# srinidhiPY/SSL_CR_Histo

Measured on AMD Instinct MI355X. Metric: images/sec (ResNet18 SSL_CR step, 256x256 bf16 synthetic patches; whole job), higher is better.
Workload: dtype bf16

## Files before the change

### include/sslcr.h

```cpp
#ifndef SSLCR_H_
#define SSLCR_H_
#include <stddef.h>
#include <stdint.h>

#ifdef __cplusplus
extern "C" {
#endif
#if defined(__GNUC__) || defined(__clang__)
#pragma GCC visibility push(default)
#endif

#define SSLCR_F32 0
#define SSLCR_BF16 1
#define SSLCR_FP8 2

int sslcr_version(void);
const char* sslcr_last_error(void);

typedef struct sslcr_conv_desc {
  const void* x;
  const void* w;
  void* y;
  const float* in_scale;
  const float* in_shift;
  const float* bias;
  const void* residual;
  float* stats;
  int N, H, W, C, K, R, S, stride, pad;
  int PH, PW;
  int OH, OW, osh;
  int transposed;
  int in_relu, relu, accumulate;
  int pix_mul, pix_off_h, pix_off_w;
  unsigned tap_mask;
  const void* mask_x; const float* mask_scale; const float* mask_shift; const float* mask_mean;
  int par4;
  int seg_images, seg_stride;
  const float* out_scale;
} sslcr_conv_desc;
int sslcr_conv2d(int dtype, const sslcr_conv_desc* d, void* stream);
int sslcr_conv2d_partial_rows(const sslcr_conv_desc* d);
int sslcr_conv2d_segments_ok(int dtype, const sslcr_conv_desc* d);
const char* sslcr_conv2d_kernel_name(int dtype, const sslcr_conv_desc* d);
int sslcr_conv2d_s2_pair(int dtype, const sslcr_conv_desc* c1, const sslcr_conv_desc* ds, void* stream);
int sslcr_conv2d_s2_pair_ok(int dtype, const sslcr_conv_desc* c1, const sslcr_conv_desc* ds);

typedef struct sslcr_fp8_desc {
  const uint8_t* w8;
  const float* w_dequant;
  float x_scale;
  const float* x_scale_dev;
  float* amax_out;
} sslcr_fp8_desc;
int sslcr_conv2d_fp8(const sslcr_conv_desc* d, const sslcr_fp8_desc* q, void* stream);
int sslcr_conv2d_fp8_partial_rows(const sslcr_conv_desc* d);
typedef struct sslcr_pack_fp8_desc {
  const float* w;
  uint8_t* w8;
  float* w_dequant;
  const float* gamma; const float* beta; const float* rmean; const float* rvar; float eps; float* bias_out;
  int K, C;
} sslcr_pack_fp8_desc;
int sslcr_pack_conv_fp8(const sslcr_pack_fp8_desc* d, void* stream);

typedef struct sslcr_wgrad_desc {
  const void* x;
  const void* dy;
  float* dw;
  const float* in_scale;
  const float* in_shift;
  int in_relu;
  int N, H, W, C, K, R, S, stride, pad, OH, OW;
  int seg_images;
  int seg_stride;
} sslcr_wgrad_desc;
int sslcr_conv2d_wgrad(int dtype, const sslcr_wgrad_desc* d, void* stream);
const char* sslcr_conv2d_wgrad_kernel_name(int dtype, const sslcr_wgrad_desc* d);

int sslcr_probe_tr16(const uint16_t* in, const int* byte_addr, uint16_t* out, void* stream);

typedef struct sslcr_stem_desc {
  const void* x;
  const void* w;
  void* y;
  const float* bias;
  float* stats;
  int N, H, W, OH, OW, in_f32, relu;
  const void* x2;
  int n_split;
  const float* out_scale;
} sslcr_stem_desc;
int sslcr_stem_conv(int dtype, const sslcr_stem_desc* d, void* stream);
int sslcr_stem_partial_rows(const sslcr_stem_desc* d);
int sslcr_stem_conv_pool(int dtype, const sslcr_stem_desc* d, int POH, int POW, void* stream);
typedef struct sslcr_stem_wgrad_desc {
  const void* x; const void* dy;
  float* dw;
  int N, H, W, OH, OW, in_f32;
  const void* x2; int n_split;
} sslcr_stem_wgrad_desc;
int sslcr_stem_wgrad(int dtype, const sslcr_stem_wgrad_desc* d, void* stream);

typedef struct sslcr_bn_finalize_desc {
  const float* partials;
  int rows, C;
  double count;
  const float* gamma; const float* beta;
  float* scale; float* shift; float* mean; float* invstd;
  float* running_mean; float* running_var; int64_t* num_batches_tracked;
  float momentum, eps; int replay;
  double* sums_out;
  const double* sums_in;
  double* stage;
  int nseg, seg_stride;
  int* tickets;
} sslcr_bn_finalize_desc;
int sslcr_bn_finalize(const sslcr_bn_finalize_desc* d, void* stream);

typedef struct sslcr_bn_act_desc {
  const void* x; const float* scale; const float* shift;
  const void* res; const float* rscale; const float* rshift;
  void* y; size_t pixels; int C; int relu;
  int nseg, seg_stride;
  uint8_t* ybits;
} sslcr_bn_act_desc;
int sslcr_bn_act(int dtype, const sslcr_bn_act_desc* d, void* stream);

typedef struct sslcr_pool_fwd_desc {
  const void* x; const float* scale; const float* shift; void* y; uint8_t* argmax; int N, H, W, C, OH, OW;
} sslcr_pool_fwd_desc;
int sslcr_bn_relu_maxpool(int dtype, const sslcr_pool_fwd_desc* d, void* stream);
typedef struct sslcr_pool_bwd_desc {
  const void* dy; const uint8_t* argmax; const void* x; const float* scale; const float* shift; void* dx; int N, H, W, C, OH, OW;
} sslcr_pool_bwd_desc;
int sslcr_maxpool_relu_bwd(int dtype, const sslcr_pool_bwd_desc* d, void* stream);

int sslcr_avgpool_fwd(int dtype, const void* x, float* y, int N, int HW, int C, void* stream);
int sslcr_avgpool_bwd(int dtype, const float* dy, void* dx, int N, int HW, int C, void* stream);

typedef struct sslcr_bn_bwd_desc {
  const void* dy; const void* x; const void* yact;
  const float* scale; const float* shift; const float* mean; const float* invstd;
  double* sums;
  void* dx; void* gout;
  size_t pixels; int C; int relu_from_x; double count;
  const void* pool_dy;
  const uint8_t* pool_argmax;
  int pH, pW, pOH, pOW;
  const void* pool_y;
  int g_in_reduce;
  float* dgamma; float* dbeta;
  float pg_scale;
  int nseg, seg_stride, sums_stride;
  const uint8_t* yact_bits;
} sslcr_bn_bwd_desc;
int sslcr_bn_bwd_reduce(int dtype, const sslcr_bn_bwd_desc* d, void* stream);
int sslcr_bn_bwd_apply(int dtype, const sslcr_bn_bwd_desc* d, void* stream);
int sslcr_bn_param_grads(const double* sums, const float* invstd, float* dgamma, float* dbeta, int C, void* stream);
int sslcr_stem_wgrad_pool(int dtype, const sslcr_stem_wgrad_desc* w, const sslcr_bn_bwd_desc* bn, void* stream);

int sslcr_linear_fwd(const float* x, const float* w, const float* b, float* y, int M, int N, int K, int relu, void* stream);
int sslcr_linear_bwd(const float* x, const float* w, const float* dy, const float* yact, float* dx, float* dw, float* db,
                     int M, int N, int K, int dx_accumulate, float* scratch, void* stream);
typedef struct sslcr_loss_desc {
  int kind;
  const float* logits; const float* logits_t;
  const float* target_f; const int64_t* target_i;
  float* dlogits;
  float* out;
  int nx, nu, C; float lambda_u;
  float inv_nx_global, inv_nu_global;
} sslcr_loss_desc;
int sslcr_loss(const sslcr_loss_desc* d, void* stream);
typedef struct sslcr_loss_opts {
  const float* class_weight;
  float label_smoothing;
  int ignore_index;
  float threshold;
  float temperature;
  const float* denominator;
  float* stats;
} sslcr_loss_opts;
int sslcr_loss_ex(const sslcr_loss_desc* d, const sslcr_loss_opts* opts, void* stream);
int sslcr_ce_denominator(const int64_t* target_i, int n, int C, const float* class_weight, int ignore_index, float* out2, void* stream);
int sslcr_softmax_col(const float* logits, float* out, int n, int C, int col, void* stream);
typedef struct sslcr_predict_desc {
  const float* logits;
  int n, C;
  const int64_t* target;
  float* scores;
  int64_t* pred;
  int64_t* confusion;
  int col;
  float* map;
  const int64_t* map_index;
  int64_t map_size;
} sslcr_predict_desc;
int sslcr_predict(const sslcr_predict_desc* d, void* stream);

typedef struct sslcr_tensor_desc {
  float* p; float* g; float* s1; float* s2;
  int n;
  int K, C, RS;
  void* w_fwd;
  void* w_dgrad;
  int pack_dtype;
  int dgrad_flip;
  int group;
} sslcr_tensor_desc;
typedef struct sslcr_opt_desc {
  int kind;
  float lr, beta1, beta2, eps, wd, momentum;
  float bc1, bc2;
  int first_step;
  float grad_scale;
} sslcr_opt_desc;
int sslcr_optimizer_step(const sslcr_tensor_desc* device_descs, int ntensors, int max_n, const sslcr_opt_desc* o, void* stream);
#define SSLCR_MAX_OPT_GROUPS 8
int sslcr_optimizer_step_groups(const sslcr_tensor_desc* device_descs, int ntensors, int max_n, const sslcr_opt_desc* groups, int ngroups,
                                const float* coef_dev, void* stream);
int sslcr_grad_norm(const float* g, size_t n, float max_norm, double* partials, float* out2, void* stream);
int sslcr_grad_norm_partials(void);
int sslcr_grad_accumulate(float* dst, const float* src, size_t n, void* stream);
int sslcr_axpby(float* p, float* q, size_t n, float alpha, int copy_back, void* stream);
int sslcr_fill(float* p, size_t n, float v, void* stream);

typedef struct sslcr_pack_desc {
  const float* w; void* w_fwd; void* w_dgrad;
  const float* gamma; const float* beta; const float* rmean; const float* rvar; float eps; float* bias_out;
  int K, C, R, S;
  int dgrad_flip;
  float* scale_out;
} sslcr_pack_desc;
int sslcr_pack_conv(int dtype, const sslcr_pack_desc* d, void* stream);
int sslcr_pack_stem(int dtype, const sslcr_pack_desc* d, void* stream);

typedef struct sslcr_weak_aug_desc {
  const uint8_t* src;
  uint8_t* dst;
  const int32_t* params;
  int N, SH, SW, OH, OW, src_hwc;
} sslcr_weak_aug_desc;
int sslcr_weak_augment(const sslcr_weak_aug_desc* d, void* stream);

typedef struct sslcr_wsi_gather_desc {
  const uint8_t* src;
  const int32_t* xy;
  uint8_t* dst;
  int origin_x, origin_y;
  int N, RH, RW, S, fill;
} sslcr_wsi_gather_desc;
int sslcr_wsi_gather(const sslcr_wsi_gather_desc* d, void* stream);

typedef struct sslcr_colour_aug_desc {
  const uint8_t* src;
  uint8_t* dst;
  const double* shift;
  const uint8_t* apply;
  double hed_from_rgb[9];
  double rgb_from_hed[9];
  int N, H, W, hwc;
} sslcr_colour_aug_desc;
int sslcr_hed_colour_augment(const sslcr_colour_aug_desc* d, void* stream);
typedef struct sslcr_brightness_contrast_desc {
  const uint8_t* src; uint8_t* dst;
  const double* alpha_beta;
  const uint8_t* apply;
  unsigned long long* stats;
  int N, H, W;
} sslcr_brightness_contrast_desc;
int sslcr_brightness_contrast(const sslcr_brightness_contrast_desc* d, void* stream);

#define SSLCR_AUGV2_COPY 0
#define SSLCR_AUGV2_BRIGHTNESS 1
#define SSLCR_AUGV2_CONTRAST 2
#define SSLCR_AUGV2_COLOR 3
#define SSLCR_AUGV2_AUTOCONTRAST 4
#define SSLCR_AUGV2_EQUALIZE 5
#define SSLCR_AUGV2_SHARPNESS 6
#define SSLCR_AUGV2_NEAREST_FIXED 7
#define SSLCR_AUGV2_NEAREST_TABLE 8
#define SSLCR_AUGV2_BICUBIC 9
typedef struct sslcr_augv2_desc {
  const uint8_t* src;
  uint8_t* dst;
  const int32_t* op;
  const float* factor;
  const int32_t* fixed;
  const double* shift;
  const double* affine;
  uint32_t* hist;
  unsigned long long* lsum;
  uint8_t* lut;
  int32_t* tab;
  unsigned ops_mask;
  int N, H, W, src_hwc, dst_hwc;
} sslcr_augv2_desc;
int sslcr_randaug_v2_slot(const sslcr_augv2_desc* d, void* stream);

#define SSLCR_AUGV2C_COPY 0
#define SSLCR_AUGV2C_HED 1
#define SSLCR_AUGV2C_HSV 2
typedef struct sslcr_augv2_colour_desc {
  uint8_t* img;
  const int32_t* op;
  const double* param;
  unsigned long long* bsum;
  double cutoff_lo, cutoff_hi;
  float hed_from_rgb[9];
  float rgb_from_hed[9];
  unsigned ops_mask;
  int N, H, W, hwc;
// ... 97 lines not shown
```

### ssl_cr_histo_amd/_lib.py

```python
import ctypes as C
import os

import torch

HERE = os.path.dirname(os.path.abspath(__file__))
LIB_PATH = os.path.join(HERE, "libsslcr.so")

vp, i32, f32, f64, sz = C.c_void_p, C.c_int, C.c_float, C.c_double, C.c_size_t


class SslcrError(RuntimeError):
    pass


def _S(name, fields):
    return type(name, (C.Structure,), {"_fields_": fields})


ConvDesc = _S("ConvDesc", [("x", vp), ("w", vp), ("y", vp), ("in_scale", vp), ("in_shift", vp), ("bias", vp),
                           ("residual", vp), ("stats", vp)] +
              [(k, i32) for k in ("N", "H", "W", "C", "K", "R", "S", "stride", "pad", "PH", "PW", "OH", "OW", "osh",
                                  "transposed", "in_relu", "relu", "accumulate", "pix_mul", "pix_off_h", "pix_off_w")] +
              [("tap_mask", C.c_uint), ("mask_x", vp), ("mask_scale", vp), ("mask_shift", vp), ("mask_mean", vp),
               ("par4", i32), ("seg_images", i32), ("seg_stride", i32), ("out_scale", vp)])
WgradDesc = _S("WgradDesc", [("x", vp), ("dy", vp), ("dw", vp), ("in_scale", vp), ("in_shift", vp), ("in_relu", i32)] +
               [(k, i32) for k in ("N", "H", "W", "C", "K", "R", "S", "stride", "pad", "OH", "OW", "seg_images", "seg_stride")])
StemDesc = _S("StemDesc", [("x", vp), ("w", vp), ("y", vp), ("bias", vp), ("stats", vp)] +
              [(k, i32) for k in ("N", "H", "W", "OH", "OW", "in_f32", "relu")] + [("x2", vp), ("n_split", i32), ("out_scale", vp)])
StemWgradDesc = _S("StemWgradDesc", [("x", vp), ("dy", vp), ("dw", vp)] +
                   [(k, i32) for k in ("N", "H", "W", "OH", "OW", "in_f32")] + [("x2", vp), ("n_split", i32)])
BnFinalizeDesc = _S("BnFinalizeDesc", [("partials", vp), ("rows", i32), ("C", i32), ("count", f64), ("gamma", vp),
                                       ("beta", vp), ("scale", vp), ("shift", vp), ("mean", vp), ("invstd", vp),
                                       ("running_mean", vp), ("running_var", vp), ("num_batches_tracked", vp),
                                       ("momentum", f32), ("eps", f32), ("replay", i32), ("sums_out", vp),
                                       ("sums_in", vp), ("stage", vp), ("nseg", i32), ("seg_stride", i32), ("tickets", vp)])
BnActDesc = _S("BnActDesc", [("x", vp), ("scale", vp), ("shift", vp), ("res", vp), ("rscale", vp), ("rshift", vp),
                             ("y", vp), ("pixels", sz), ("C", i32), ("relu", i32), ("nseg", i32), ("seg_stride", i32), ("ybits", vp)])
PoolFwdDesc = _S("PoolFwdDesc", [("x", vp), ("scale", vp), ("shift", vp), ("y", vp), ("argmax", vp)] +
                 [(k, i32) for k in ("N", "H", "W", "C", "OH", "OW")])
PoolBwdDesc = _S("PoolBwdDesc", [("dy", vp), ("argmax", vp), ("x", vp), ("scale", vp), ("shift", vp), ("dx", vp)] +
                 [(k, i32) for k in ("N", "H", "W", "C", "OH", "OW")])
BnBwdDesc = _S("BnBwdDesc", [("dy", vp), ("x", vp), ("yact", vp), ("scale", vp), ("shift", vp), ("mean", vp),
                             ("invstd", vp), ("sums", vp), ("dx", vp), ("gout", vp), ("pixels", sz), ("C", i32),
                             ("relu_from_x", i32), ("count", f64), ("pool_dy", vp), ("pool_argmax", vp), ("pH", i32),
                             ("pW", i32), ("pOH", i32), ("pOW", i32), ("pool_y", vp), ("g_in_reduce", i32), ("dgamma", vp), ("dbeta", vp),
                             ("pg_scale", f32), ("nseg", i32), ("seg_stride", i32), ("sums_stride", i32), ("yact_bits", vp)])
LossDesc = _S("LossDesc", [("kind", i32), ("logits", vp), ("logits_t", vp), ("target_f", vp), ("target_i", vp),
                           ("dlogits", vp), ("out", vp), ("nx", i32), ("nu", i32), ("C", i32), ("lambda_u", f32),
                           ("inv_nx_global", f32), ("inv_nu_global", f32)])
LossOpts = _S("LossOpts", [("class_weight", vp), ("label_smoothing", f32), ("ignore_index", i32), ("threshold", f32),
                           ("temperature", f32), ("denominator", vp), ("stats", vp)])
TensorDesc = _S("TensorDesc", [("p", vp), ("g", vp), ("s1", vp), ("s2", vp), ("n", i32), ("K", i32), ("C", i32),
                               ("RS", i32), ("w_fwd", vp), ("w_dgrad", vp), ("pack_dtype", i32), ("dgrad_flip", i32),
                               ("group", i32)])
OptDesc = _S("OptDesc", [("kind", i32), ("lr", f32), ("beta1", f32), ("beta2", f32), ("eps", f32), ("wd", f32),
                         ("momentum", f32), ("bc1", f32), ("bc2", f32), ("first_step", i32), ("grad_scale", f32)])
ClipDesc = _S("ClipDesc", [("max_norm", f32), ("out2", vp)])
MAX_OPT_GROUPS = 8
WeakAugDesc = _S("WeakAugDesc", [("src", vp), ("dst", vp), ("params", vp)] +
                 [(k, i32) for k in ("N", "SH", "SW", "OH", "OW", "src_hwc")])
ColourAugDesc = _S("ColourAugDesc", [("src", vp), ("dst", vp), ("shift", vp), ("apply", vp), ("hed_from_rgb", f64 * 9),
                                     ("rgb_from_hed", f64 * 9), ("N", i32), ("H", i32), ("W", i32), ("hwc", i32)])
BrightnessContrastDesc = _S("BrightnessContrastDesc", [("src", vp), ("dst", vp), ("alpha_beta", vp), ("apply", vp), ("stats", vp),
                                                       ("N", i32), ("H", i32), ("W", i32)])
AugV2Desc = _S("AugV2Desc", [(k, vp) for k in ("src", "dst", "op", "factor", "fixed", "shift", "affine", "hist", "lsum", "lut", "tab")] +
                [("ops_mask", C.c_uint)] + [(k, i32) for k in ("N", "H", "W", "src_hwc", "dst_hwc")])
AugV2ColourDesc = _S("AugV2ColourDesc", [("img", vp), ("op", vp), ("param", vp), ("bsum", vp), ("cutoff_lo", f64), ("cutoff_hi", f64),
                                         ("hed_from_rgb", f32 * 9), ("rgb_from_hed", f32 * 9), ("ops_mask", C.c_uint)] +
                      [(k, i32) for k in ("N", "H", "W", "hwc")])
WsiGatherDesc = _S("WsiGatherDesc", [("src", vp), ("xy", vp), ("dst", vp)] +
                   [(k, i32) for k in ("origin_x", "origin_y", "N", "RH", "RW", "S", "fill")])
PredictDesc = _S("PredictDesc", [("logits", vp), ("n", i32), ("C", i32), ("target", vp), ("scores", vp), ("pred", vp), ("confusion", vp),
                                 ("col", i32), ("map", vp), ("map_index", vp), ("map_size", C.c_int64)])
PackDesc = _S("PackDesc", [("w", vp), ("w_fwd", vp), ("w_dgrad", vp), ("gamma", vp), ("beta", vp), ("rmean", vp),
                           ("rvar", vp), ("eps", f32), ("bias_out", vp)] + [(k, i32) for k in ("K", "C", "R", "S", "dgrad_flip")] + [("scale_out", vp)])

Fp8Desc = _S("Fp8Desc", [("w8", vp), ("w_dequant", vp), ("x_scale", f32), ("x_scale_dev", vp), ("amax_out", vp)])
PackFp8Desc = _S("PackFp8Desc", [("w", vp), ("w8", vp), ("w_dequant", vp), ("gamma", vp), ("beta", vp), ("rmean", vp), ("rvar", vp),
                                 ("eps", f32), ("bias_out", vp), ("K", i32), ("C", i32)])

P = C.POINTER
SIGNATURES = {
    "sslcr_version": (i32, []),
    "sslcr_last_error": (C.c_char_p, []),
    "sslcr_conv2d": (i32, [i32, P(ConvDesc), vp]),
    "sslcr_conv2d_partial_rows": (i32, [P(ConvDesc)]),
    "sslcr_conv2d_segments_ok": (i32, [i32, P(ConvDesc)]),
    "sslcr_conv2d_kernel_name": (C.c_char_p, [i32, P(ConvDesc)]),
    "sslcr_conv2d_s2_pair": (i32, [i32, P(ConvDesc), P(ConvDesc), vp]),
    "sslcr_conv2d_s2_pair_ok": (i32, [i32, P(ConvDesc), P(ConvDesc)]),
    "sslcr_conv2d_fp8": (i32, [P(ConvDesc), P(Fp8Desc), vp]),
    "sslcr_conv2d_fp8_partial_rows": (i32, [P(ConvDesc)]),
    "sslcr_pack_conv_fp8": (i32, [P(PackFp8Desc), vp]),
    "sslcr_conv2d_wgrad": (i32, [i32, P(WgradDesc), vp]),
    "sslcr_conv2d_wgrad_kernel_name": (C.c_char_p, [i32, P(WgradDesc)]),
    "sslcr_probe_tr16": (i32, [vp, vp, vp, vp]),
    "sslcr_stem_conv": (i32, [i32, P(StemDesc), vp]),
    "sslcr_stem_partial_rows": (i32, [P(StemDesc)]),
    "sslcr_stem_conv_pool": (i32, [i32, P(StemDesc), i32, i32, vp]),
    "sslcr_stem_wgrad": (i32, [i32, P(StemWgradDesc), vp]),
    "sslcr_stem_wgrad_pool": (i32, [i32, P(StemWgradDesc), P(BnBwdDesc), vp]),
    "sslcr_bn_finalize": (i32, [P(BnFinalizeDesc), vp]),
    "sslcr_bn_act": (i32, [i32, P(BnActDesc), vp]),
    "sslcr_bn_relu_maxpool": (i32, [i32, P(PoolFwdDesc), vp]),
    "sslcr_maxpool_relu_bwd": (i32, [i32, P(PoolBwdDesc), vp]),
    "sslcr_avgpool_fwd": (i32, [i32, vp, vp, i32, i32, i32, vp]),
    "sslcr_avgpool_bwd": (i32, [i32, vp, vp, i32, i32, i32, vp]),
    "sslcr_bn_bwd_reduce": (i32, [i32, P(BnBwdDesc), vp]),
    "sslcr_bn_bwd_apply": (i32, [i32, P(BnBwdDesc), vp]),
    "sslcr_bn_param_grads": (i32, [vp, vp, vp, vp, i32, vp]),
    "sslcr_linear_fwd": (i32, [vp, vp, vp, vp, i32, i32, i32, i32, vp]),
    "sslcr_linear_bwd": (i32, [vp, vp, vp, vp, vp, vp, vp, i32, i32, i32, i32, vp, vp]),
    "sslcr_loss": (i32, [P(LossDesc), vp]),
    "sslcr_loss_ex": (i32, [P(LossDesc), P(LossOpts), vp]),
    "sslcr_ce_denominator": (i32, [vp, i32, i32, vp, i32, vp, vp]),
    "sslcr_softmax_col": (i32, [vp, vp, i32, i32, i32, vp]),
    "sslcr_predict": (i32, [P(PredictDesc), vp]),
    "sslcr_wsi_gather": (i32, [P(WsiGatherDesc), vp]),
    "sslcr_optimizer_step": (i32, [vp, i32, i32, P(OptDesc), vp]),
    "sslcr_optimizer_step_groups": (i32, [vp, i32, i32, P(OptDesc), i32, vp, vp]),
    "sslcr_grad_norm": (i32, [vp, sz, f32, vp, vp, vp]),
    "sslcr_grad_norm_partials": (i32, []),
    "sslcr_grad_accumulate": (i32, [vp, vp, sz, vp]),
    "sslcr_axpby": (i32, [vp, vp, sz, f32, i32, vp]),
    "sslcr_fill": (i32, [vp, sz, f32, vp]),
    "sslcr_pack_conv": (i32, [i32, P(PackDesc), vp]),
    "sslcr_pack_stem": (i32, [i32, P(PackDesc), vp]),
    "sslcr_weak_augment": (i32, [P(WeakAugDesc), vp]),
    "sslcr_hed_colour_augment": (i32, [P(ColourAugDesc), vp]),
    "sslcr_brightness_contrast": (i32, [P(BrightnessContrastDesc), vp]),
    "sslcr_randaug_v2_slot": (i32, [P(AugV2Desc), vp]),
    "sslcr_randaug_v2_colour": (i32, [P(AugV2ColourDesc), vp]),
}

_lib = None


def lib():
    global _lib
    if _lib is None:
        if not os.path.exists(LIB_PATH):
            raise SslcrError(f"{LIB_PATH} not built: run `python -m ssl_cr_histo_amd.build` "
                             "(or __graft_entry__.build()); there is no CPU/PyTorch fallback")
        L = C.CDLL(LIB_PATH, mode=C.RTLD_GLOBAL)
        for name, (res, args) in SIGNATURES.items():
            fn = getattr(L, name)
            fn.restype = res
            fn.argtypes = args
        _lib = L
    return _lib


def check(rc):
    if rc != 0:
        raise SslcrError(lib().sslcr_last_error().decode())


def stream_ptr():
    return C.c_void_p(torch.cuda.current_stream().cuda_stream)


def ptr(t):
    return None if t is None else C.c_void_p(t.data_ptr())
```

### ssl_cr_histo_amd/csrc/capi.cpp

```cpp
#include <stdarg.h>
#include <stdio.h>
#include <string.h>

#include "kernels.hpp"

namespace sslcr {
thread_local char g_err[512] = "";
int fail(const char* fmt, ...) {
  va_list ap;
  va_start(ap, fmt);
  vsnprintf(g_err, sizeof(g_err), fmt, ap);
  va_end(ap);
  return -1;
}
int check(hipError_t e, const char* what) {
  if (e == hipSuccess) return 0;
  return fail("%s: %s", what, hipGetErrorString(e));
}
}

using namespace sslcr;

#define NEED(cond, what) \
  do {                   \
    if (!(cond)) return fail("%s: invalid argument (%s)", __func__, what); \
  } while (0)
#define DT_OK(dt) NEED((dt) == SSLCR_F32 || (dt) == SSLCR_BF16, "dtype")

extern "C" {

int sslcr_version(void) { return 12; }
const char* sslcr_last_error(void) { return g_err; }

int sslcr_conv2d(int dtype, const sslcr_conv_desc* d, void* stream) {
  DT_OK(dtype);
  NEED(d && d->x && d->w && d->y, "null tensor");
  NEED(d->N > 0 && d->C > 0 && d->K > 0 && d->R > 0 && d->S > 0 && d->stride > 0, "shape");
  NEED(d->C % (dtype == SSLCR_BF16 ? 64 : 32) == 0, "C must be a multiple of the 128-byte channel slab");
  NEED(d->K % 64 == 0, "K % 64");
  NEED(d->osh >= 1 && d->PH > 0 && d->PW > 0, "pixel space");
  const ConvPlan p = conv_plan(dtype, *d);
  NEED(p.seg_ok, "seg_images: no segment form for this shape / dtype (sslcr_conv2d_segments_ok)");
  return check(launch_conv(dtype, *d, p, (hipStream_t)stream), "conv2d");
}
int sslcr_conv2d_partial_rows(const sslcr_conv_desc* d) { return d ? conv_partials_rows(*d) : -1; }
int sslcr_conv2d_segments_ok(int dtype, const sslcr_conv_desc* d) { return (d && (dtype == DT_F32 || dtype == DT_BF16) && conv_segments_ok(dtype, *d)) ? 1 : 0; }
const char* sslcr_conv2d_kernel_name(int dtype, const sslcr_conv_desc* d) { return d ? conv_kernel_name(dtype, *d) : ""; }
int sslcr_conv2d_s2_pair_ok(int dtype, const sslcr_conv_desc* c1, const sslcr_conv_desc* ds) {
  return (c1 && ds && conv_s2_pair_ok(dtype, *c1, *ds)) ? 1 : 0;
}
int sslcr_conv2d_s2_pair(int dtype, const sslcr_conv_desc* c1, const sslcr_conv_desc* ds, void* stream) {
  DT_OK(dtype);
  NEED(c1 && ds && c1->x && c1->w && c1->y && ds->w && ds->y, "null tensor");
  NEED(conv_s2_pair_ok(dtype, *c1, *ds), "pair not served (sslcr_conv2d_s2_pair_ok)");
  return check(launch_conv_s2(*c1, ds, (hipStream_t)stream), "conv2d_s2_pair");
}

int sslcr_conv2d_fp8(const sslcr_conv_desc* d, const sslcr_fp8_desc* q, void* stream) {
  NEED(d && q && d->x && d->y && q->w8 && q->w_dequant, "null tensor");
  NEED(q->x_scale > 0.f, "x_scale must be positive");
  NEED(conv_fp8_mode(*d) != 0, "shape not served by the fp8 kernel (3x3/1, C % 128, K % 128, 16x16-tileable or 8x8 with N % 4)");
  return check(launch_conv_fp8(*d, *q, (hipStream_t)stream), "conv2d_fp8");
}
int sslcr_conv2d_fp8_partial_rows(const sslcr_conv_desc* d) { return (d && conv_fp8_mode(*d)) ? conv_fp8_rows(*d) : 0; }
int sslcr_pack_conv_fp8(const sslcr_pack_fp8_desc* d, void* stream) {
  NEED(d && d->w && d->w8 && d->w_dequant && d->K > 0 && d->C > 0, "args");
  NEED(!d->gamma || (d->beta && d->rmean && d->rvar), "BatchNorm fold needs gamma, beta, running mean and var");
  return check(launch_pack_fp8(*d, (hipStream_t)stream), "pack_conv_fp8");
}

const char* sslcr_conv2d_wgrad_kernel_name(int dtype, const sslcr_wgrad_desc* d) { return d ? wgrad_kernel_name(dtype, *d) : ""; }
int sslcr_conv2d_wgrad(int dtype, const sslcr_wgrad_desc* d, void* stream) {
  DT_OK(dtype);
  NEED(d && d->x && d->dy && d->dw, "null tensor");
  NEED(d->C % 64 == 0 && d->K % 64 == 0, "C,K % 64");
  NEED((d->R == 3 && d->S == 3) || (d->R == 1 && d->S == 1), "3x3 or 1x1");
  return check(launch_wgrad(dtype, *d, (hipStream_t)stream), "conv2d_wgrad");
}

int sslcr_probe_tr16(const uint16_t* in, const int* byte_addr, uint16_t* out, void* stream) {
  NEED(in && byte_addr && out, "null");
  return check(launch_probe_tr16(in, byte_addr, out, (hipStream_t)stream), "probe_tr16");
}

int sslcr_stem_conv(int dtype, const sslcr_stem_desc* d, void* stream) {
  DT_OK(dtype);
  NEED(d && d->x && d->w && d->y, "null tensor");
  NEED(d->OH == (d->H + 6 - 7) / 2 + 1 && d->OW == (d->W + 6 - 7) / 2 + 1, "7x7/2 pad 3 output dims");
  NEED(!d->x2 || (d->n_split >= 0 && d->n_split <= d->N), "n_split outside the batch");
  return check(launch_stem(dtype, *d, (hipStream_t)stream), "stem_conv");
}
int sslcr_stem_conv_pool(int dtype, const sslcr_stem_desc* d, int POH, int POW, void* stream) {
  DT_OK(dtype);
  NEED(d && d->x && d->w && d->y, "null");
  NEED(stem_pool_ok(dtype, *d, POH, POW), "shape / mode not served by the fused stem + max-pool kernel");
  return check(launch_stem_pool(dtype, *d, POH, POW, (hipStream_t)stream), "stem_conv_pool");
}
int sslcr_stem_partial_rows(const sslcr_stem_desc* d) { return d ? stem_partials_rows(*d) : -1; }
int sslcr_stem_wgrad(int dtype, const sslcr_stem_wgrad_desc* d, void* stream) {
  DT_OK(dtype);
  NEED(d && d->x && d->dy && d->dw, "null tensor");
  NEED(!d->x2 || (d->n_split >= 0 && d->n_split <= d->N), "n_split outside the batch");
  return check(launch_stem_wgrad(dtype, *d, (hipStream_t)stream), "stem_wgrad");
}
int sslcr_stem_wgrad_pool(int dtype, const sslcr_stem_wgrad_desc* w, const sslcr_bn_bwd_desc* bn, void* stream) {
  DT_OK(dtype);
  NEED(w && w->x && w->dw && bn && bn->pool_dy && bn->pool_argmax && bn->x && bn->sums && bn->mean && bn->invstd && bn->scale && bn->shift, "null tensor");
  NEED(!w->x2 || (w->n_split >= 0 && w->n_split <= w->N), "n_split outside the batch");
  NEED(bn->C == 64 && bn->pH == w->OH && bn->pW == w->OW && bn->pixels == (size_t)w->N * w->OH * w->OW, "bn descriptor is not this stem's");
  NEED(!bn->g_in_reduce && !bn->gout, "pool form has no g output");
  return check(launch_stem_wgrad_pool(dtype, *w, *bn, (hipStream_t)stream), "stem_wgrad_pool");
}

int sslcr_bn_finalize(const sslcr_bn_finalize_desc* d, void* stream) {
  NEED(d && d->C > 0, "desc");
  NEED(d->sums_in || (d->partials && d->stage && d->rows > 0), "partials/stage");
  NEED(d->sums_out || (d->gamma && d->beta && d->scale && d->shift && d->count > 0), "finalize outputs");
  return check(launch_bn_finalize(*d, (hipStream_t)stream), "bn_finalize");
}
int sslcr_bn_act(int dtype, const sslcr_bn_act_desc* d, void* stream) {
  DT_OK(dtype);
  NEED(d && d->x && d->y && d->scale && d->shift, "null");
  NEED(d->C % 8 == 0, "C % 8");
  return check(launch_bn_act(dtype, *d, (hipStream_t)stream), "bn_act");
}
int sslcr_bn_relu_maxpool(int dtype, const sslcr_pool_fwd_desc* d, void* stream) {
  DT_OK(dtype);
  NEED(d && d->x && d->y, "null");
  if (!d->scale || !d->shift) {
    const int cols = d->C / (dtype == SSLCR_BF16 ? 8 : 4);
    NEED(!d->scale && !d->shift && !d->argmax, "plain max-pool (scale = shift = NULL) records no argmax");
    NEED(cols >= 1 && cols <= 256 && 256 % cols == 0 && d->C % (dtype == SSLCR_BF16 ? 8 : 4) == 0, "plain max-pool: unsupported channel count");
  }
  return check(launch_bn_relu_maxpool(dtype, *d, (hipStream_t)stream), "bn_relu_maxpool");
}
int sslcr_maxpool_relu_bwd(int dtype, const sslcr_pool_bwd_desc* d, void* stream) {
  DT_OK(dtype);
  NEED(d && d->x && d->dy && d->dx && d->argmax, "null");
  return check(launch_maxpool_relu_bwd(dtype, *d, (hipStream_t)stream), "maxpool_relu_bwd");
}
int sslcr_avgpool_fwd(int dtype, const void* x, float* y, int N, int HW, int C, void* stream) {
  DT_OK(dtype);
  NEED(x && y && N > 0 && HW > 0 && C % 8 == 0, "args");
  return check(launch_avgpool_fwd(dtype, x, y, N, HW, C, (hipStream_t)stream), "avgpool_fwd");
}
int sslcr_avgpool_bwd(int dtype, const float* dy, void* dx, int N, int HW, int C, void* stream) {
  DT_OK(dtype);
  NEED(dy && dx && N > 0 && HW > 0 && C % 8 == 0, "args");
  return check(launch_avgpool_bwd(dtype, dy, dx, N, HW, C, (hipStream_t)stream), "avgpool_bwd");
}
int sslcr_bn_bwd_reduce(int dtype, const sslcr_bn_bwd_desc* d, void* stream) {
  DT_OK(dtype);
  NEED(d && (d->dy || (d->pool_dy && d->pool_argmax)) && d->x && d->sums && d->mean, "null");
  NEED(!d->g_in_reduce || (d->yact && d->gout && d->dy && !d->pool_dy), "g_in_reduce needs dy, yact and gout");
  return check(launch_bn_bwd_reduce(dtype, *d, (hipStream_t)stream), "bn_bwd_reduce");
}
int sslcr_bn_bwd_apply(int dtype, const sslcr_bn_bwd_desc* d, void* stream) {
  DT_OK(dtype);
  NEED(d && (d->dy || (d->pool_dy && d->pool_argmax)) && d->x && d->sums && d->dx && d->mean && d->invstd && d->scale, "null");
  NEED(!d->g_in_reduce || (d->yact && d->gout && d->dy && !d->pool_dy), "g_in_reduce needs dy, yact and gout");
  return check(launch_bn_bwd_apply(dtype, *d, (hipStream_t)stream), "bn_bwd_apply");
}
int sslcr_bn_param_grads(const double* sums, const float* invstd, float* dgamma, float* dbeta, int C, void* stream) {
  NEED(sums && invstd && dgamma && dbeta, "null");
  return check(launch_bn_param_grads(sums, invstd, dgamma, dbeta, C, (hipStream_t)stream), "bn_param_grads");
}

int sslcr_linear_fwd(const float* x, const float* w, const float* b, float* y, int M, int N, int K, int relu, void* stream) {
  NEED(x && w && y && M > 0 && N > 0 && K > 0, "args");
  return check(launch_linear_fwd(x, w, b, y, M, N, K, relu, (hipStream_t)stream), "linear_fwd");
}
int sslcr_linear_bwd(const float* x, const float* w, const float* dy, const float* yact, float* dx, float* dw, float* db,
                     int M, int N, int K, int dx_accumulate, float* scratch, void* stream) {
  NEED(x && w && dy && scratch && M > 0 && N > 0 && K > 0, "args");
  return check(launch_linear_bwd(x, w, dy, yact, dx, dw, db, M, N, K, dx_accumulate, scratch, (hipStream_t)stream), "linear_bwd");
}
int sslcr_loss(const sslcr_loss_desc* d, void* stream) {
  NEED(d && d->logits && d->out && d->nx > 0 && d->C > 0 && d->C <= 64, "args");
  return check(launch_loss(*d, (hipStream_t)stream), "loss");
}

int sslcr_loss_ex(const sslcr_loss_desc* d, const sslcr_loss_opts* o, void* stream) {
  if (!o) return sslcr_loss(d, stream);
  NEED(d && d->logits && d->out && d->nx > 0 && d->C > 0 && d->C <= 64, "args");
  const char* why = loss_opts_error(d->kind, d->C, *o);
  if (why) return fail("sslcr_loss_ex: invalid argument (%s)", why);
  if (d->kind != 1 && d->kind != 2) return check(launch_loss(*d, (hipStream_t)stream), "loss");
  NEED(d->target_i && (d->kind == 2 || d->nu == 0 || d->logits_t), "cross-entropy needs target_i (and logits_t for the consistency rows)");
  NEED(d->nu >= 0, "nu");
  return check(launch_loss_ex(*d, *o, (hipStream_t)stream), "loss_ex");
}
int sslcr_ce_denominator(const int64_t* target_i, int n, int C, const float* class_weight, int ignore_index, float* out2, void* stream) {
  NEED(out2 && (target_i || n == 0) && n >= 0 && C > 0 && C <= 64, "args");
  return check(launch_ce_denominator(target_i, n, C, class_weight, ignore_index, out2, (hipStream_t)stream), "ce_denominator");
}

int sslcr_softmax_col(const float* logits, float* out, int n, int C, int col, void* stream) {
  NEED(logits && out && n > 0 && C > 0 && C <= 64 && col >= 0 && col < C, "args");
  return check(launch_softmax_col(logits, out, n, C, col, (hipStream_t)stream), "softmax_col");
}

int sslcr_predict(const sslcr_predict_desc* d, void* stream) {
  NEED(d, "null descriptor");
  NEED(d->n >= 0 && d->C >= 1 && d->C <= 64, "n >= 0 and 1 <= C <= 64");
  if (d->n == 0) return 0;
  NEED(d->logits, "null logits");
  NEED(!d->confusion || d->target, "confusion needs target");
  NEED((reinterpret_cast<uintptr_t>(d->confusion) & 7) == 0, "confusion alignment");
  NEED(!d->map || (d->map_index && d->map_size >= 0), "map needs map_index and map_size >= 0");
  NEED(!d->map || (d->col >= 0 && d->col < d->C), "col outside [0, C)");
  return check(launch_predict(*d, (hipStream_t)stream), "predict");
}
int sslcr_wsi_gather(const sslcr_wsi_gather_desc* d, void* stream) {
  NEED(d, "null descriptor");
  NEED(d->S >= 1 && d->N >= 0, "S >= 1 and N >= 0");
  NEED(d->RH >= 1 && d->RW >= 1, "empty region");
  NEED(d->fill >= 0 && d->fill <= 255, "fill outside [0, 255]");
  if (d->N == 0) return 0;
  NEED(d->src && d->xy && d->dst, "null tensor");
  NEED((reinterpret_cast<uintptr_t>(d->xy) & 3) == 0, "xy alignment");
  return check(launch_wsi_gather(*d, (hipStream_t)stream), "wsi_gather");
}

int sslcr_optimizer_step(const sslcr_tensor_desc* device_descs, int ntensors, int max_n, const sslcr_opt_desc* o, void* stream) {
  return sslcr_optimizer_step_groups(device_descs, ntensors, max_n, o, 1, nullptr, stream);
}
int sslcr_optimizer_step_groups(const sslcr_tensor_desc* device_descs, int ntensors, int max_n, const sslcr_opt_desc* groups, int ngroups,
                                const float* coef_dev, void* stream) {
  NEED(device_descs && groups && ntensors > 0 && max_n > 0, "args");
  NEED(ngroups >= 1 && ngroups <= SSLCR_MAX_OPT_GROUPS, "ngroups must be 1..8");
// ... 82 lines not shown
```

### ssl_cr_histo_amd/csrc/common.hpp

```cpp
#pragma once
#include <hip/hip_runtime.h>
#include <stdint.h>

namespace sslcr {

typedef uint16_t bf16_t;
typedef __bf16 bf16x8_t __attribute__((ext_vector_type(8)));
typedef float f32x4_t __attribute__((ext_vector_type(4)));
typedef uint32_t u32x4_t __attribute__((ext_vector_type(4)));
typedef uint32_t u32x2_t __attribute__((ext_vector_type(2)));

enum { DT_F32 = 0, DT_BF16 = 1 };

__device__ __forceinline__ float bf2f(uint16_t v) { return __uint_as_float(((uint32_t)v) << 16); }
__device__ __forceinline__ uint16_t f2bf(float f) {
  uint32_t u = __float_as_uint(f);
  u += 0x7fffu + ((u >> 16) & 1u);
  return (uint16_t)(u >> 16);
}
__device__ __forceinline__ uint32_t pack_bf2(float lo, float hi) {
  return (uint32_t)f2bf(lo) | ((uint32_t)f2bf(hi) << 16);
}
__device__ __forceinline__ float bf_lo(uint32_t w) { return __uint_as_float(w << 16); }
__device__ __forceinline__ float bf_hi(uint32_t w) { return __uint_as_float(w & 0xffff0000u); }

template <typename T> struct Elem;
template <> struct Elem<float> {
  static constexpr int EPC = 4;
  static constexpr int DT = DT_F32;
  __device__ static __forceinline__ void unpack(const u32x4_t& v, float* f) {
#pragma unroll
    for (int i = 0; i < 4; ++i) f[i] = __uint_as_float(v[i]);
  }
  __device__ static __forceinline__ u32x4_t pack(const float* f) {
    u32x4_t v;
#pragma unroll
    for (int i = 0; i < 4; ++i) v[i] = __float_as_uint(f[i]);
    return v;
  }
  __device__ static __forceinline__ float ld(const float* p) { return *p; }
  __device__ static __forceinline__ void st(float* p, float v) { *p = v; }
};
template <> struct Elem<bf16_t> {
  static constexpr int EPC = 8;
  static constexpr int DT = DT_BF16;
  __device__ static __forceinline__ void unpack(const u32x4_t& v, float* f) {
#pragma unroll
    for (int i = 0; i < 4; ++i) { f[2 * i] = bf_lo(v[i]); f[2 * i + 1] = bf_hi(v[i]); }
  }
  __device__ static __forceinline__ u32x4_t pack(const float* f) {
    u32x4_t v;
#pragma unroll
    for (int i = 0; i < 4; ++i) v[i] = pack_bf2(f[2 * i], f[2 * i + 1]);
    return v;
  }
  __device__ static __forceinline__ float ld(const bf16_t* p) { return bf2f(*p); }
  __device__ static __forceinline__ void st(bf16_t* p, float v) { *p = f2bf(v); }
};

template <typename T> struct PackH {
  __device__ static __forceinline__ u32x4_t run(const float* f) { return Elem<T>::pack(f); }
};
template <> struct PackH<bf16_t> {
  typedef __bf16 bf16x2_t __attribute__((ext_vector_type(2)));
  typedef float f32x2_t __attribute__((ext_vector_type(2)));
  __device__ static __forceinline__ u32x4_t run(const float* f) {
    u32x4_t v;
#pragma unroll
    for (int i = 0; i < 4; ++i)
      v[i] = __builtin_bit_cast(uint32_t, __builtin_convertvector(f32x2_t{f[2 * i], f[2 * i + 1]}, bf16x2_t));
    return v;
  }
};

__device__ __forceinline__ float row16_sum(float v) {
  v += __int_as_float(__builtin_amdgcn_update_dpp(0, __float_as_int(v), 0xB1, 0xf, 0xf, true));
  v += __int_as_float(__builtin_amdgcn_update_dpp(0, __float_as_int(v), 0x4E, 0xf, 0xf, true));
  v += __int_as_float(__builtin_amdgcn_update_dpp(0, __float_as_int(v), 0x141, 0xf, 0xf, true));
  v += __int_as_float(__builtin_amdgcn_update_dpp(0, __float_as_int(v), 0x140, 0xf, 0xf, true));
  return v;
}
__device__ __forceinline__ void row16_sum4(float& a, float& b, float& c, float& d) {
  asm volatile(
      "s_nop 1\n\t"
      "v_add_f32_dpp %0, %0, %0 quad_perm:[1,0,3,2] row_mask:0xf bank_mask:0xf\n\t"
      "v_add_f32_dpp %1, %1, %1 quad_perm:[1,0,3,2] row_mask:0xf bank_mask:0xf\n\t"
      "v_add_f32_dpp %2, %2, %2 quad_perm:[1,0,3,2] row_mask:0xf bank_mask:0xf\n\t"
      "v_add_f32_dpp %3, %3, %3 quad_perm:[1,0,3,2] row_mask:0xf bank_mask:0xf\n\t"
      "v_add_f32_dpp %0, %0, %0 quad_perm:[2,3,0,1] row_mask:0xf bank_mask:0xf\n\t"
      "v_add_f32_dpp %1, %1, %1 quad_perm:[2,3,0,1] row_mask:0xf bank_mask:0xf\n\t"
      "v_add_f32_dpp %2, %2, %2 quad_perm:[2,3,0,1] row_mask:0xf bank_mask:0xf\n\t"
      "v_add_f32_dpp %3, %3, %3 quad_perm:[2,3,0,1] row_mask:0xf bank_mask:0xf\n\t"
      "v_add_f32_dpp %0, %0, %0 row_half_mirror row_mask:0xf bank_mask:0xf\n\t"
      "v_add_f32_dpp %1, %1, %1 row_half_mirror row_mask:0xf bank_mask:0xf\n\t"
      "v_add_f32_dpp %2, %2, %2 row_half_mirror row_mask:0xf bank_mask:0xf\n\t"
      "v_add_f32_dpp %3, %3, %3 row_half_mirror row_mask:0xf bank_mask:0xf\n\t"
      "v_add_f32_dpp %0, %0, %0 row_mirror row_mask:0xf bank_mask:0xf\n\t"
      "v_add_f32_dpp %1, %1, %1 row_mirror row_mask:0xf bank_mask:0xf\n\t"
      "v_add_f32_dpp %2, %2, %2 row_mirror row_mask:0xf bank_mask:0xf\n\t"
      "v_add_f32_dpp %3, %3, %3 row_mirror row_mask:0xf bank_mask:0xf"
      : "+v"(a), "+v"(b), "+v"(c), "+v"(d));
}
__device__ __forceinline__ void row16_fold16(float (&v)[16]) {
  asm volatile(
      "s_nop 1\n\t"
      "v_add_f32_dpp %0, %0, %0 row_ror:8 row_mask:0xf bank_mask:0x3\n\t"
      "v_add_f32_dpp %0, %8, %8 row_ror:8 row_mask:0xf bank_mask:0xc\n\t"
      "v_add_f32_dpp %1, %1, %1 row_ror:8 row_mask:0xf bank_mask:0x3\n\t"
      "v_add_f32_dpp %1, %9, %9 row_ror:8 row_mask:0xf bank_mask:0xc\n\t"
      "v_add_f32_dpp %2, %2, %2 row_ror:8 row_mask:0xf bank_mask:0x3\n\t"
      "v_add_f32_dpp %2, %10, %10 row_ror:8 row_mask:0xf bank_mask:0xc\n\t"
      "v_add_f32_dpp %3, %3, %3 row_ror:8 row_mask:0xf bank_mask:0x3\n\t"
      "v_add_f32_dpp %3, %11, %11 row_ror:8 row_mask:0xf bank_mask:0xc\n\t"
      "v_add_f32_dpp %4, %4, %4 row_ror:8 row_mask:0xf bank_mask:0x3\n\t"
      "v_add_f32_dpp %4, %12, %12 row_ror:8 row_mask:0xf bank_mask:0xc\n\t"
      "v_add_f32_dpp %5, %5, %5 row_ror:8 row_mask:0xf bank_mask:0x3\n\t"
      "v_add_f32_dpp %5, %13, %13 row_ror:8 row_mask:0xf bank_mask:0xc\n\t"
      "v_add_f32_dpp %6, %6, %6 row_ror:8 row_mask:0xf bank_mask:0x3\n\t"
      "v_add_f32_dpp %6, %14, %14 row_ror:8 row_mask:0xf bank_mask:0xc\n\t"
      "v_add_f32_dpp %7, %7, %7 row_ror:8 row_mask:0xf bank_mask:0x3\n\t"
      "v_add_f32_dpp %7, %15, %15 row_ror:8 row_mask:0xf bank_mask:0xc\n\t"
      "v_add_f32_dpp %0, %0, %0 row_half_mirror row_mask:0xf bank_mask:0x5\n\t"
      "v_add_f32_dpp %0, %4, %4 row_half_mirror row_mask:0xf bank_mask:0xa\n\t"
      "v_add_f32_dpp %1, %1, %1 row_half_mirror row_mask:0xf bank_mask:0x5\n\t"
      "v_add_f32_dpp %1, %5, %5 row_half_mirror row_mask:0xf bank_mask:0xa\n\t"
      "v_add_f32_dpp %2, %2, %2 row_half_mirror row_mask:0xf bank_mask:0x5\n\t"
      "v_add_f32_dpp %2, %6, %6 row_half_mirror row_mask:0xf bank_mask:0xa\n\t"
      "v_add_f32_dpp %3, %3, %3 row_half_mirror row_mask:0xf bank_mask:0x5\n\t"
      "v_add_f32_dpp %3, %7, %7 row_half_mirror row_mask:0xf bank_mask:0xa\n\t"
      "v_add_f32_dpp %0, %0, %0 quad_perm:[1,0,3,2] row_mask:0xf bank_mask:0xf\n\t"
      "v_add_f32_dpp %1, %1, %1 quad_perm:[1,0,3,2] row_mask:0xf bank_mask:0xf\n\t"
      "v_add_f32_dpp %2, %2, %2 quad_perm:[1,0,3,2] row_mask:0xf bank_mask:0xf\n\t"
      "v_add_f32_dpp %3, %3, %3 quad_perm:[1,0,3,2] row_mask:0xf bank_mask:0xf\n\t"
      "v_add_f32_dpp %0, %0, %0 quad_perm:[2,3,0,1] row_mask:0xf bank_mask:0xf\n\t"
      "v_add_f32_dpp %1, %1, %1 quad_perm:[2,3,0,1] row_mask:0xf bank_mask:0xf\n\t"
      "v_add_f32_dpp %2, %2, %2 quad_perm:[2,3,0,1] row_mask:0xf bank_mask:0xf\n\t"
      "v_add_f32_dpp %3, %3, %3 quad_perm:[2,3,0,1] row_mask:0xf bank_mask:0xf"
      : "+&v"(v[0]), "+&v"(v[1]), "+&v"(v[2]), "+&v"(v[3]), "+&v"(v[4]), "+&v"(v[5]), "+&v"(v[6]), "+&v"(v[7])
      : "v"(v[8]), "v"(v[9]), "v"(v[10]), "v"(v[11]), "v"(v[12]), "v"(v[13]), "v"(v[14]), "v"(v[15]));
}
__device__ __forceinline__ float wave_sum(float v) {
  v = row16_sum(v);
  v += __shfl_xor(v, 16);
  v += __shfl_xor(v, 32);
  return v;
}

__device__ __forceinline__ float clamp_lo(float x, float lo) { return __builtin_amdgcn_fmed3f(x, lo, __builtin_inff()); }
__device__ __forceinline__ float relu0(float x) { return __builtin_amdgcn_fmed3f(x, 0.f, __builtin_inff()); }

__device__ __forceinline__ u32x4_t ld16(const void* p) { return *reinterpret_cast<const u32x4_t*>(p); }
__device__ __forceinline__ void st16(void* p, const u32x4_t& v) { *reinterpret_cast<u32x4_t*>(p) = v; }
__device__ __forceinline__ u32x4_t ld16_nt(const void* p) { return __builtin_nontemporal_load(reinterpret_cast<const u32x4_t*>(p)); }
__device__ __forceinline__ void st16_nt(void* p, const u32x4_t& v) { __builtin_nontemporal_store(v, reinterpret_cast<u32x4_t*>(p)); }

struct LdsDma {
#if defined(__HIP_DEVICE_COMPILE__)
  __amdgpu_buffer_rsrc_t r;
#endif
  __device__ __forceinline__ void init(const void* base, unsigned bytes) {
#if defined(__HIP_DEVICE_COMPILE__)
    r = __builtin_amdgcn_make_buffer_rsrc(const_cast<void*>(base), 0, (int)bytes, 0x00020000);
#endif
  }
  __device__ __forceinline__ void load16(void* dst, int voff, int soff) const {
#if defined(__HIP_DEVICE_COMPILE__)
    __builtin_amdgcn_raw_ptr_buffer_load_lds(r, (__attribute__((address_space(3))) void*)dst, 16, voff, soff, 0, 0);
#endif
  }
};


template <typename T> struct Mma;
template <> struct Mma<bf16_t> {
  __device__ static __forceinline__ void run(const u32x4_t& a, const u32x4_t& b, f32x4_t& c) {
    c = __builtin_amdgcn_mfma_f32_16x16x32_bf16(__builtin_bit_cast(bf16x8_t, a), __builtin_bit_cast(bf16x8_t, b), c, 0, 0, 0);
  }
};
template <> struct Mma<float> {
  __device__ static __forceinline__ void run(const u32x4_t& a, const u32x4_t& b, f32x4_t& c) {
#pragma unroll
    for (int e = 0; e < 4; ++e)
      c = __builtin_amdgcn_mfma_f32_16x16x4f32(__uint_as_float(a[e]), __uint_as_float(b[e]), c, 0, 0, 0);
  }
};

template <typename B>
__device__ __forceinline__ int xcd_run_start(B b, int G) { return (G & 7) ? (int)b : (int)(b & 7) * (G >> 3) + (int)(b >> 3); }
struct OuterInner { int outer, inner; };
__device__ __forceinline__ OuterInner xcd_outer_inner(int w, int n_outer, int n_inner, bool inner_slow) {
  int outer, inner;
  if ((n_outer & 7) == 0) {
    const int grp = w / (8 * n_inner), r = w - grp * 8 * n_inner;
    outer = grp * 8 + (r & 7); inner = r >> 3;
  } else if (inner_slow) {
    inner = w / n_outer; outer = w - inner * n_outer;
  } else {
    outer = w / n_inner; inner = w - outer * n_inner;
  }
  return {outer, inner};
}

typedef short s16x4_t __attribute__((ext_vector_type(4)));
typedef short s16x8_t __attribute__((ext_vector_type(8)));
__device__ __forceinline__ bf16x8_t tr_pair(const char* p0, const char* p1) {
  s16x4_t lo = __builtin_amdgcn_ds_read_tr16_b64_v4i16((__attribute__((address_space(3))) s16x4_t*)(p0));
  s16x4_t hi = __builtin_amdgcn_ds_read_tr16_b64_v4i16((__attribute__((address_space(3))) s16x4_t*)(p1));
  s16x8_t v = __builtin_shufflevector(lo, hi, 0, 1, 2, 3, 4, 5, 6, 7);
  return __builtin_bit_cast(bf16x8_t, v);
}
template <int OFF>
__device__ __forceinline__ u32x2_t lds_tr16(uint32_t addr) {
  u32x2_t v;
  asm volatile("ds_read_b64_tr_b16 %0, %1 offset:%2" : "=v"(v) : "v"(addr), "n"(OFF));
  return v;
}
__device__ __forceinline__ uint32_t lds_addr(const void* p) { return (uint32_t)(size_t)(__attribute__((address_space(3))) const char*)(const char*)p; }
__device__ __forceinline__ bf16x8_t frag_join(const u32x2_t& lo, const u32x2_t& hi) {
  return __builtin_bit_cast(bf16x8_t, u32x4_t{lo[0], lo[1], hi[0], hi[1]});
}

__device__ __forceinline__ void barrier_lds() { asm volatile("s_waitcnt lgkmcnt(0)\n\ts_barrier" ::: "memory"); }
__device__ __forceinline__ void barrier_bare() { asm volatile("s_barrier" ::: "memory"); }
// ... 91 lines not shown
```

### ssl_cr_histo_amd/csrc/conv_route.cpp

```cpp
#include "kernels.hpp"

namespace sslcr {

ConvPlan conv_plan(int dtype, const ConvArgs& a) {
  auto both = [&](int (*tiling)(int, const ConvArgs&)) {
    const int t = tiling(dtype, a);
    return t == tiling(DT_BF16, a) ? t : 0;
  };
  const bool segs = a.seg_images > 0;
  const bool seg_common = segs && dtype == DT_BF16 && a.N % a.seg_images == 0 && !a.transposed && !a.par4 && a.N / a.seg_images <= 8;
  bool seg_form = false;
  bool ok = !(a.out_scale && (!a.bias || a.stats || a.mask_x));
  ConvPlan p{};
  const int q = both(conv_halo256_mode);
  if (const int mode = conv_h16_mode(a, q)) {
    const bool pp = conv_pp64_ok(dtype, a);
    p.route = pp ? ConvRoute::PP64 : ConvRoute::H16;
    p.param = mode;
    p.rows = segs && a.N < a.seg_images ? -1 : (pp ? conv_pp64_rows(a) : conv_h16_rows(a));
    p.name = pp ? conv_pp64_name(a) : conv_h16_name(dtype, a, mode);
    seg_form = true;
  } else if (q) {
    p.route = ConvRoute::HALO256;
    p.param = q;
    p.rows = conv_halo256_tiles(a, q) * 4;
    p.name = conv_halo256_name(dtype, a, q);
    seg_form = q == 16 || a.seg_images % 4 == 0;
  } else if (const int tw = both(conv_halo_tw)) {
    p.route = ConvRoute::HALO;
    p.param = tw;
    p.rows = conv_halo_tiles(a, tw) * 2;
    p.name = conv_halo_name(dtype, a, tw);
  } else if (conv_s2_ok(dtype, a)) {
    p.route = ConvRoute::S2;
    p.rows = conv_s2_rows(a);
    p.name = conv_s2_name(a, false);
    seg_form = true;
  } else if (conv_s2d_ok(dtype, a)) {
    p.route = ConvRoute::S2D;
    const int bp = both(conv_dma_bp);
    p.rows = bp ? conv_dma_rows(a, bp) : conv_igemm_rows(a);
    p.name = conv_s2d_name();
    p.par4_one_launch = bp != 0;
  } else if (const int bp = both(conv_dma_bp)) {
    p.route = ConvRoute::DMA;
    p.param = bp;
    p.rows = conv_dma_rows(a, bp);
    p.name = conv_dma_name(dtype, bp);
    p.par4_one_launch = a.par4 != 0;
    seg_form = !a.in_scale && ((long)a.seg_images * a.PH * a.PW) % bp == 0;
  } else {
    p.route = ConvRoute::IGEMM;
    p.rows = conv_igemm_rows(a);
    p.name = conv_igemm_name(dtype, a);
    if (a.par4) ok = false;
  }
  if (a.mask_x && p.route != ConvRoute::H16 && p.route != ConvRoute::PP64) ok = seg_form = false;
  p.seg_ok = !segs || (seg_common && seg_form);
  p.ok = ok && p.seg_ok;
  return p;
}

hipError_t launch_conv(int dtype, const ConvArgs& a, const ConvPlan& p, hipStream_t st) {
  if (!p.ok) return hipErrorInvalidValue;
  switch (p.route) {
    case ConvRoute::H16: return launch_conv_h16(dtype, a, p.param, st);
    case ConvRoute::PP64: return launch_conv_pp64(a, st);
    case ConvRoute::HALO256: return launch_conv_halo256(dtype, a, p.param, st);
    case ConvRoute::HALO: return launch_conv_halo(dtype, a, p.param, st);
    case ConvRoute::S2: return launch_conv_s2(a, nullptr, st);
    case ConvRoute::S2D: return launch_conv_s2d(a, st);
    case ConvRoute::DMA: return launch_conv_dma(dtype, a, p.param, st);
    case ConvRoute::IGEMM: return launch_igemm(dtype, a, st);
  }
  return hipErrorInvalidValue;
}

WgradPlan wgrad_plan(int dtype, const WgradArgs& a) {
  if (const int tw = wgrad_halo_tw(a)) {
    const int kh = dtype == DT_BF16 && a.K % 128 == 0 ? 2 : 1;
    if (kh == 2 && wgrad_dma_ok(dtype, a, wgrad_halo_splits(a, tw, 2))) return {WgradRoute::HALO_DMA, tw, 2, true, wgrad_dma_name(a, tw)};
    return {WgradRoute::HALO, tw, kh, true, wgrad_halo_name(dtype, tw, kh)};
  }
  if (wgrad_s2_ok(dtype, a)) return {WgradRoute::S2, 0, 0, true, wgrad_s2_name(a)};
  const bool segs = a.seg_images > 0 && a.seg_images < a.N;
  return {WgradRoute::GENERIC, 0, 0, !segs, wgrad_generic_name(dtype, a)};
}

hipError_t launch_wgrad(int dtype, const WgradArgs& a, const WgradPlan& p, hipStream_t st) {
  if (!p.ok) return hipErrorInvalidValue;
  switch (p.route) {
    case WgradRoute::HALO:
    case WgradRoute::HALO_DMA: return launch_wgrad_halo(dtype, a, p, st);
    case WgradRoute::S2: return launch_wgrad_s2(a, st);
    case WgradRoute::GENERIC: return launch_wgrad_generic(dtype, a, st);
  }
  return hipErrorInvalidValue;
}

}
```

### ssl_cr_histo_amd/csrc/engine.cpp

```cpp
#include <rccl/rccl.h>
#include <stdio.h>
#include <stdlib.h>
#include <string.h>

#include <atomic>
#include <chrono>
#include <condition_variable>
#include <mutex>
#include <vector>

#include "kernels.hpp"

using namespace sslcr;

#define TRY(expr)                                   \
  do {                                              \
    hipError_t _e = (expr);                         \
    if (_e != hipSuccess) return check(_e, #expr);  \
  } while (0)
#define TRYI(expr)            \
  do {                        \
    int _r = (expr);          \
    if (_r != 0) return _r;   \
  } while (0)
// ... 181 lines not shown
  float *cat[3], *hact[3], *fi[3], *feats = nullptr, *hid = nullptr, *logits = nullptr, *dE[3], *dfeats = nullptr, *dhid = nullptr,
        *dtmp256 = nullptr, *dtmp512 = nullptr, *dcat = nullptr, *scratch = nullptr, *dlogits = nullptr, *logits_t = nullptr;
  int last_N = 0, last_npass = 0;
  bool last_segments = false;
  bool packed_train = false, packed_eval = false;
  bool tap = false;
  DevBuf tapbuf[8][6];
  int tapdims[8][6][4] = {};
  int tap_flags[8] = {};
  std::vector<sslcr_tensor_desc> host_descs;
  std::vector<float*> st1, st2;
  std::vector<int> group_of;
  int ndesc = 0, max_n = 0;
};

namespace {

struct VSrc { const void* p[VW_MAX]; };
template <typename T>
__global__ void vsum_kernel(T* dst, VSrc src, int W, size_t n) {
  for (size_t i = (size_t)blockIdx.x * blockDim.x + threadIdx.x; i < n; i += (size_t)gridDim.x * blockDim.x) {
    T s = static_cast<const T*>(src.p[0])[i];
    for (int q = 1; q < W; ++q) s += static_cast<const T*>(src.p[q])[i];
    dst[i] = s;
  }
}

std::atomic<int> g_live_ctx{0};

inline bool sharded(const sslcr_ctx* c) { return c->comm != nullptr || c->vcomm != nullptr; }

int vcomm_all_reduce(sslcr_ctx* c, int chan, void* buf, size_t count, bool f64, hipStream_t st) {
  sslcr_vcomm* v = c->vcomm;
  VChan& ch = v->ch[chan];
  const int r = c->rank, W = v->world;
  const size_t bytes = count * (f64 ? 8 : 4);
  if (v->poisoned) return fail("virtual all-reduce: the communicator was poisoned by an earlier timeout");
  const int ph = (int)(ch.calls[r]++ & 1);
  for (int q = 0; q < W; ++q)
    if (q != r && ch.out_set[ph][q]) TRY(hipStreamWaitEvent(st, ch.ev_out[ph][q], 0));
  if (ch.cap[ph][r] < bytes) {
    if (ch.slot[ph][r]) TRY(hipFree(ch.slot[ph][r]));
    ch.slot[ph][r] = nullptr; ch.cap[ph][r] = 0;
    TRY(hipMalloc(&ch.slot[ph][r], (bytes + 255) & ~(size_t)255));
    ch.cap[ph][r] = (bytes + 255) & ~(size_t)255;
  }
  if (!ch.ev_in[ph][r]) {
    TRY(hipEventCreateWithFlags(&ch.ev_in[ph][r], hipEventDisableTiming));
    TRY(hipEventCreateWithFlags(&ch.ev_out[ph][r], hipEventDisableTiming));
  }
  TRY(hipMemcpyAsync(ch.slot[ph][r], buf, bytes, hipMemcpyDeviceToDevice, st));
  TRY(hipEventRecord(ch.ev_in[ph][r], st));
  {
    std::unique_lock<std::mutex> lk(ch.m);
    const long g = ch.gen;
    if (++ch.arrived == W) {
      ch.arrived = 0; ++ch.gen;
      ch.cv.notify_all();
    } else if (!ch.cv.wait_for(lk, std::chrono::seconds(120), [&] { return ch.gen != g; })) {
      --ch.arrived;
      c->vcomm->poisoned = true;
      ch.cv.notify_all();
      return fail("virtual all-reduce: rank %d waited 120 s for its peers (channel %d); the communicator is now unusable", r, chan);
    }
  }
  VSrc src;
  for (int q = 0; q < W; ++q) {
    src.p[q] = ch.slot[ph][q];
    if (q != r) TRY(hipStreamWaitEvent(st, ch.ev_in[ph][q], 0));
  }
  const int blocks = (int)((count + 255) / 256 < 1024 ? (count + 255) / 256 : 1024);
  if (f64) hipLaunchKernelGGL(vsum_kernel<double>, dim3(blocks), dim3(256), 0, st, (double*)buf, src, W, count);
  else hipLaunchKernelGGL(vsum_kernel<float>, dim3(blocks), dim3(256), 0, st, (float*)buf, src, W, count);
  TRY(hipGetLastError());
  TRY(hipEventRecord(ch.ev_out[ph][r], st));
  ch.out_set[ph][r] = true;
  return 0;
}

int all_reduce(sslcr_ctx* c, int chan, void* buf, size_t count, bool f64, hipStream_t st) {
  if (c->vcomm) return vcomm_all_reduce(c, chan, buf, count, f64, st);
  TRYN(ncclAllReduce(buf, buf, count, f64 ? ncclDouble : ncclFloat, ncclSum, chan == 0 ? c->comm : c->comm_g, st));
  return 0;
}

template <class Book, class Launch>
hipError_t profiled(sslcr_ctx* c, int slot, hipStream_t st, Book&& book, Launch&& launch) {
  if (!c->prof.on) return launch();
  ProfRec r;
  r.e0 = c->prof.get(); r.e1 = c->prof.get();
  book(r);
  (void)hipEventRecord(r.e0, st);
  hipError_t e = launch();
  (void)hipEventRecord(r.e1, st);
  c->prof.rec[slot].push_back(r);
  return e;
}
hipError_t prof_conv(sslcr_ctx* c, int dt, const ConvArgs& a, hipStream_t st) {
  const ConvPlan plan = conv_plan(dt, a);
  auto book = [&](ProfRec& r) {
    const double es = c->esz();
    const double rs = a.tap_mask ? (double)__builtin_popcount(a.tap_mask) : (double)a.R * a.S;
    const double M = (double)a.N * a.PH * a.PW, src = (double)a.N * a.H * a.W;
    r.flops = a.transposed ? 2.0 * src * a.C * a.K * rs : 2.0 * M * a.K * a.C * rs;
    r.bytes = (src * a.C + (double)a.K * rs * a.C + M * a.K * (a.residual ? 2.0 : 1.0) * (a.accumulate ? 2.0 : 1.0)) * es;
    r.name = plan.name;
  };
  return profiled(c, 0, st, book, [&] { return launch_conv(dt, a, plan, st); });
}
hipError_t prof_conv_pair(sslcr_ctx* c, const ConvArgs& a, const ConvArgs& d, hipStream_t st) {
  auto book = [&](ProfRec& r) {
    const double es = c->esz();
    const double M = (double)a.N * a.PH * a.PW, src = (double)a.N * a.H * a.W;
    r.flops = 2.0 * M * a.K * a.C * 10.0;
    r.bytes = (src * a.C + (double)a.K * 10.0 * a.C + 2.0 * M * a.K) * es;
    r.name = conv_s2_name(a, true);
  };
  return profiled(c, 0, st, book, [&] { return launch_conv_s2(a, &d, st); });
}
inline bool fp8_layer(const sslcr_ctx* c, const ConvL& L) {
  return c->fp8 && L.k == 3 && L.stride == 1 && L.cin % 128 == 0 && L.cout % 128 == 0;
}
inline bool use_fp8(const sslcr_ctx* c, const ConvL& L, const ConvArgs& a) { return fp8_layer(c, L) && L.w8_fwd && conv_fp8_mode(a) != 0; }
hipError_t prof_conv_fwd(sslcr_ctx* c, int dt, const ConvArgs& a_in, const ConvL& L, bool folded, hipStream_t st) {
  ConvArgs a = a_in;
  a.out_scale = nullptr;
  if (!use_fp8(c, L, a)) return prof_conv(c, dt, a_in, st);
  Fp8Args q;
  q.w8 = folded ? L.w8_fold : L.w8_fwd;
  q.w_dequant = folded ? L.dq_fold : L.dq_fwd;
  q.x_scale = 1.0f;
  q.x_scale_dev = L.f8s ? L.f8s + (folded ? 2 : 0) : nullptr;
  q.amax_out = L.f8s ? L.f8s + (folded ? 3 : 1) : nullptr;
  auto book = [&](ProfRec& r) {
    const double M = (double)a.N * a.PH * a.PW;
    r.flops = 2.0 * M * a.K * a.C * 9.0;
    r.bytes = ((double)a.N * a.H * a.W * a.C + M * a.K * (a.residual ? 2.0 : 1.0)) * 2.0 + (double)a.K * 9.0 * a.C;
    r.name = conv_fp8_name(a);
  };
  return profiled(c, 0, st, book, [&] { return launch_conv_fp8(a, q, st); });
}
hipError_t prof_wgrad(sslcr_ctx* c, int dt, const WgradArgs& a, hipStream_t st) {
  const WgradPlan plan = wgrad_plan(dt, a);
  auto book = [&](ProfRec& r) {
    const double es = c->esz();
    const double M = (double)a.N * a.OH * a.OW;
    r.flops = 2.0 * M * a.K * a.C * a.R * a.S;
    r.bytes = ((double)a.N * a.H * a.W * a.C + M * a.K) * es + (double)a.K * a.R * a.S * a.C * 4.0;
    r.name = plan.name;
  };
  return profiled(c, 1, st, book, [&] { return launch_wgrad(dt, a, plan, st); });
}

inline bool tile16(const ConvPlan& p) { return p.route == ConvRoute::H16 || p.route == ConvRoute::PP64; }

constexpr int kMaxSeg = 3;
const int kBlockCfg[8][3] ={{64, 64, 1}, {64, 64, 1}, {64, 128, 2}, {128, 128, 1}, {128, 256, 2}, {256, 256, 1}, {256, 512, 2}, {512, 512, 1}};

inline int out_dim(int h, int k, int stride, int pad) { return (h + 2 * pad - k) / stride + 1; }

void build_topology(sslcr_net* n) {
  int p = 0, b = 0;
  n->stem = ConvL{3, 64, 7, 2, 3, p++};
  n->bn0 = BnL{64, p, p + 1, b++};
  p += 2;
  for (int i = 0; i < 8; ++i) {
    BlockL& B = n->blocks[i];
    const int cin = kBlockCfg[i][0], cout = kBlockCfg[i][1], s = kBlockCfg[i][2];
    B.pstart = p;
    B.c1 = ConvL{cin, cout, 3, s, 1, p++};
    B.b1 = BnL{cout, p, p + 1, b++};
    p += 2;
    B.c2 = ConvL{cout, cout, 3, 1, 1, p++};
    B.b2 = BnL{cout, p, p + 1, b++};
    p += 2;
    B.has_ds = (s != 1 || cin != cout);
    if (B.has_ds) {
      B.ds = ConvL{cin, cout, 1, s, 0, p++};
      B.bd = BnL{cout, p, p + 1, b++};
      p += 2;
    }
  }
  n->psize.assign(n->nparams, 0);
  auto conv_sz = [](const ConvL& c) { return c.cout * c.cin * c.k * c.k; };
  n->psize[n->stem.pidx] = conv_sz(n->stem);
  n->psize[n->bn0.pg] = n->psize[n->bn0.pb] = 64;
  for (int i = 0; i < 8; ++i) {
    BlockL& B = n->blocks[i];
    n->psize[B.c1.pidx] = conv_sz(B.c1);
    n->psize[B.c2.pidx] = conv_sz(B.c2);
    n->psize[B.b1.pg] = n->psize[B.b1.pb] = B.b1.C;
    n->psize[B.b2.pg] = n->psize[B.b2.pb] = B.b2.C;
    if (B.has_ds) {
      n->psize[B.ds.pidx] = conv_sz(B.ds);
      n->psize[B.bd.pg] = n->psize[B.bd.pb] = B.bd.C;
    }
  }
  n->psize[60] = 512 * 1024;
  n->psize[61] = 512;
  n->psize[62] = 256 * 512;
  n->psize[63] = 256;
  if (n->head_kind == 0) {
    n->psize[64] = n->ncls * 768;
    n->psize[65] = n->ncls;
  } else {
    n->psize[64] = 128 * 768;
    n->psize[65] = 128;
    n->psize[66] = n->ncls * 128;
    n->psize[67] = n->ncls;
  }
  n->goff.assign(n->nparams + 1, 0);
  for (int i = 0; i < n->nparams; ++i) n->goff[i + 1] = n->goff[i] + ((n->psize[i] + 63) & ~63);
  n->grad_count = n->goff[n->nparams];
}

bool unfold_eval(const sslcr_ctx* c) {
  static const bool on = [] { const char* e = getenv("SSLCR_UNFOLD_EVAL"); return !e || atoi(e) != 0; }();
  return on && c->dtype == DT_BF16;
}

int alloc_shadow(sslcr_net* n) {
  const size_t es = n->ctx->esz();
  Carver c;
  std::vector<std::pair<ConvL*, size_t>> offs;
  auto add = [&](ConvL& L) {
    const size_t wbytes = (L.pidx == 0 ? (size_t)64 * 224 : (size_t)L.cout * L.cin * L.k * L.k) * es;
    size_t o = c.take(wbytes);
    c.take(wbytes);
    c.take(wbytes);
    c.take(L.cout * sizeof(float));
    c.take(L.cout * sizeof(float));
    if (L.pidx == 0) c.take(wbytes);
    if (fp8_layer(n->ctx, L)) {
      c.take((size_t)L.cout * 9 * L.cin); c.take((size_t)L.cout * 9 * L.cin);
      c.take(L.cout * sizeof(float)); c.take(L.cout * sizeof(float));
    }
    offs.push_back({&L, o});
  };
  add(n->stem);
  for (int i = 0; i < 8; ++i) {
    add(n->blocks[i].c1);
    add(n->blocks[i].c2);
    if (n->blocks[i].has_ds) add(n->blocks[i].ds);
  }
  TRYI(n->shadow.ensure(c.off));
  for (auto& pr : offs) {
    ConvL& L = *pr.first;
    const size_t wbytes = ((L.pidx == 0 ? (size_t)64 * 224 : (size_t)L.cout * L.cin * L.k * L.k) * es + 255) & ~(size_t)255;
    char* base = (char*)n->shadow.p + pr.second;
    L.w_fwd = base;
    L.w_dg = base + wbytes;
    L.w_fold = base + 2 * wbytes;
    L.b_fold = (float*)(base + 3 * wbytes);
    {
      const size_t bb = (L.cout * sizeof(float) + 255) & ~(size_t)255;
      L.s_fold = unfold_eval(n->ctx) ? (float*)(base + 3 * wbytes + bb) : nullptr;
      if (L.pidx == 0) L.w_foldf = base + 3 * wbytes + 2 * bb;
    }
    if (fp8_layer(n->ctx, L)) {
      const size_t bb = (L.cout * sizeof(float) + 255) & ~(size_t)255, w8 = ((size_t)L.cout * 9 * L.cin + 255) & ~(size_t)255;
      char* q = base + 3 * wbytes + 2 * bb;
      L.w8_fwd = (uint8_t*)q; L.w8_fold = (uint8_t*)(q + w8);
      L.dq_fwd = (float*)(q + 2 * w8); L.dq_fold = (float*)(q + 2 * w8 + bb);
    }
  }
  if (n->ctx->fp8) {
    n->n8 = 0;
    for (auto& pr : offs) if (pr.first->w8_fwd) n->n8 += 2;
    TRYI(n->f8buf.ensure((size_t)n->n8 * 2 * sizeof(float)));
    n->f8slots = (float*)n->f8buf.p;
    std::vector<float> init((size_t)n->n8 * 2);
    for (int i = 0; i < n->n8; ++i) { init[2 * i] = 1.f; init[2 * i + 1] = 0.f; }
    TRY(hipMemcpy(n->f8slots, init.data(), init.size() * sizeof(float), hipMemcpyHostToDevice));
    int k = 0;
    for (auto& pr : offs) if (pr.first->w8_fwd) { pr.first->f8s = n->f8slots + 4 * k; ++k; }
  }
  return 0;
}

int pack_conv_layer(sslcr_net* n, ConvL& L, const BnL& bn, int mode, hipStream_t st) {
  const int dt = n->ctx->dtype;
  PackArgs a;
  memset(&a, 0, sizeof(a));
  a.w = n->params[L.pidx];
  a.K = L.cout; a.C = L.cin; a.R = L.k; a.S = L.k;
  a.eps = 1e-5f;
  const bool stem = (L.pidx == 0);
  if (mode & 1) {
    a.w_fwd = L.w_fwd;
    a.w_dgrad = stem ? nullptr : L.w_dg;
    a.dgrad_flip = (L.k == 3 && L.stride == 1);
    TRY(stem ? launch_pack_stem(dt, a, st) : launch_pack_conv(dt, a, st));
  }
  if (mode & 2) {
    a.w_fwd = L.w_fold;
    a.w_dgrad = nullptr;
    a.gamma = n->params[bn.pg]; a.beta = n->params[bn.pb];
    a.rmean = n->bn_rm[bn.bidx]; a.rvar = n->bn_rv[bn.bidx];
    a.bias_out = L.b_fold;
    a.scale_out = L.s_fold;
    TRY(stem ? launch_pack_stem(dt, a, st) : launch_pack_conv(dt, a, st));
    if (stem && L.s_fold && L.w_foldf) {
      a.w_fwd = L.w_foldf; a.scale_out = nullptr;
      TRY(launch_pack_stem(dt, a, st));
    }
  }
// ... 398 lines not shown
  n->feats = (float*)(b + o_feats); n->hid = (float*)(b + o_hid); n->logits = (float*)(b + o_log);
  n->dfeats = (float*)(b + o_dfeats); n->dhid = (float*)(b + o_dhid);
  n->dtmp256 = (float*)(b + o_d256); n->dtmp512 = (float*)(b + o_d512); n->dcat = (float*)(b + o_dcat);
  n->scratch = (float*)(b + o_scr); n->dlogits = (float*)(b + o_dl); n->logits_t = (float*)(b + o_lt);
  n->hN = N;
  return 0;
}

const int kPairs[3][2] = {{0, 1}, {1, 2}, {0, 2}};

int heads_forward(sslcr_net* n, float* const* E, int npass, int N, hipStream_t st) {
  const float *w0 = n->params[60], *b0 = n->params[61], *w2 = n->params[62], *b2 = n->params[63];
  const int nh = (npass == 3) ? 3 : 1;
  for (int i = 0; i < nh; ++i) {
    const float* Ea = E[npass == 3 ? kPairs[i][0] : 0];
    const float* Eb = E[npass == 3 ? kPairs[i][1] : 0];
    if (Ea == Eb) {
      TRY(launch_copy2d_multi(n->cat[i], 1024, 2, 512, Ea, 512, 1, 0, N, 512, st));
    } else {
      TRY(launch_copy2d(n->cat[i], 1024, Ea, 512, N, 512, 0, st));
      TRY(launch_copy2d(n->cat[i] + 512, 1024, Eb, 512, N, 512, 0, st));
    }
    TRY(launch_linear_fwd(n->cat[i], w0, b0, n->hact[i], N, 512, 1024, 1, st));
    TRY(launch_linear_fwd(n->hact[i], w2, b2, n->fi[i], N, 256, 512, 0, st));
  }
  if (nh == 1) {
    TRY(launch_copy2d_multi(n->feats, 768, 3, 256, n->fi[0], 256, 1, 0, N, 256, st));
  } else {
    for (int i = 0; i < 3; ++i) TRY(launch_copy2d(n->feats + 256 * i, 768, n->fi[i], 256, N, 256, 0, st));
  }
  if (n->head_kind == 0) {
    TRY(launch_linear_fwd(n->feats, n->params[64], n->params[65], n->logits, N, n->ncls, 768, 0, st));
  } else {
    TRY(launch_linear_fwd(n->feats, n->params[64], n->params[65], n->hid, N, 128, 768, 1, st));
    TRY(launch_linear_fwd(n->hid, n->params[66], n->params[67], n->logits, N, n->ncls, 128, 0, st));
  }
  return 0;
}

inline float* gptr(sslcr_net* n, int pidx) { return n->rg[pidx] ? n->gw + n->goff[pidx] : nullptr; }

int heads_backward(sslcr_net* n, const float* dlogits, int npass, int N, bool need_dE, hipStream_t st) {
  const float *w0 = n->params[60], *w2 = n->params[62];
  const bool any_fc = n->rg[60] || n->rg[61] || n->rg[62] || n->rg[63];
  if (n->head_kind == 0) {
    TRY(launch_linear_bwd(n->feats, n->params[64], dlogits, nullptr, (any_fc || need_dE) ? n->dfeats : nullptr, gptr(n, 64), gptr(n, 65),
                          N, n->ncls, 768, 0, n->scratch, st));
  } else {
    TRY(launch_linear_bwd(n->hid, n->params[66], dlogits, nullptr, n->dhid, gptr(n, 66), gptr(n, 67), N, n->ncls, 128, 0, n->scratch, st));
    TRY(launch_linear_bwd(n->feats, n->params[64], n->dhid, n->hid, (any_fc || need_dE) ? n->dfeats : nullptr, gptr(n, 64), gptr(n, 65),
                          N, 128, 768, 0, n->scratch, st));
  }
  if (!any_fc && !need_dE) return 0;
  const int nh = (npass == 3) ? 3 : 1;
  if (need_dE && nh == 3)
    for (int i = 0; i < npass; ++i) TRY(hipMemsetAsync(n->dE[i], 0, (size_t)N * 512 * 4, st));
  for (int i = 0; i < nh; ++i) {
    if (nh == 3) {
      TRY(launch_copy2d(n->dtmp256, 256, n->dfeats + 256 * i, 768, N, 256, 0, st));
    } else {
      TRY(launch_copy2d_multi(n->dtmp256, 256, 1, 0, n->dfeats, 768, 3, 256, N, 256, st));
    }
    TRY(launch_linear_bwd(n->hact[i], w2, n->dtmp256, nullptr, n->dtmp512, gptr(n, 62), gptr(n, 63), N, 256, 512, 0, n->scratch, st));
    TRY(launch_linear_bwd(n->cat[i], w0, n->dtmp512, n->hact[i], need_dE ? n->dcat : nullptr, gptr(n, 60), gptr(n, 61), N, 512, 1024, 0,
                          n->scratch, st));
    if (need_dE && nh == 1) {
      TRY(launch_copy2d_multi(n->dE[0], 512, 1, 0, n->dcat, 1024, 2, 512, N, 512, st));
    } else if (need_dE) {
      const int a = nh == 3 ? kPairs[i][0] : 0, b = nh == 3 ? kPairs[i][1] : 0;
      TRY(launch_copy2d(n->dE[a], 512, n->dcat, 1024, N, 512, 1, st));
      TRY(launch_copy2d(n->dE[b], 512, n->dcat + 512, 1024, N, 512, 1, st));
    }
  }
  return 0;
}

struct PoolSrc {
  const void* dy; const uint8_t* argmax; int H, W, OH, OW; const void* y;
};

struct BnBwdReq {
  const void *dy = nullptr, *x = nullptr, *yact = nullptr;
  void *dx = nullptr, *gout = nullptr;
  int relu_from_x = 0;
  size_t pixels = 0;
  double count = 0.0;
  const PoolSrc* pool = nullptr;
  int g_in_reduce = 0;
  const float* sum_rows = nullptr;
  int n_sum_rows = 0, nseg = 0, seg_stride = 0;
  bool defer = false;
};

double* take_sums_n(sslcr_ctx* c, int nseg) {
  if (!c->bn_ring.p || c->bn_ring_i + nseg > sslcr_ctx::kBnRing) return nullptr;
  double* p = (double*)c->bn_ring.p + (size_t)c->bn_ring_i * sslcr_ctx::kBnSlot;
  c->bn_ring_i += nseg;
  return p;
}
double* take_sums(sslcr_ctx* c) { return take_sums_n(c, 1); }
double* take_sums_or_fixed(sslcr_ctx* c) {
  double* ring = take_sums(c);
  return ring ? ring : c->bn_sums;
}

int bn_bwd_begin(sslcr_net* n, const BnL& bn, const BnSaved& sv, const BnBwdReq& q, hipStream_t st, double* sums, BnBwdArgs* out) {
  sslcr_ctx* c = n->ctx;
  BnBwdArgs a;
  memset(&a, 0, sizeof(a));
  a.dy = q.dy; a.x = q.x; a.yact = q.yact; a.scale = sv.scale; a.shift = sv.shift; a.mean = sv.mean; a.invstd = sv.invstd;
  a.sums = sums; a.dx = q.dx; a.gout = q.gout; a.pixels = q.pixels; a.C = bn.C; a.relu_from_x = q.relu_from_x;
  if (q.nseg > 1) { a.nseg = q.nseg; a.seg_stride = q.seg_stride; a.sums_stride = sslcr_ctx::kBnSlot; }
  a.g_in_reduce = (q.g_in_reduce && q.yact && q.gout) ? 1 : 0;
  a.yact_bits = ybits_of(n, q.yact);
  const bool synced = sharded(c) && c->bn_sync;
  if (n->rg[bn.pg] || n->rg[bn.pb]) {
    a.dgamma = gptr(n, bn.pg); a.dbeta = gptr(n, bn.pb);
    a.pg_scale = synced ? 1.0f / c->world : 1.0f;
    if (!a.dgamma || !a.dbeta) { a.dgamma = nullptr; a.dbeta = nullptr; }
  }
  if (const PoolSrc* s = q.pool) { a.pool_dy = s->dy; a.pool_argmax = s->argmax; a.pH = s->H; a.pW = s->W; a.pOH = s->OH; a.pOW = s->OW; a.pool_y = s->y; }
  a.count = synced ? q.count * c->world : q.count;
  if (q.sum_rows) {
    BnFinalizeArgs r;
    memset(&r, 0, sizeof(r));
    r.partials = q.sum_rows; r.rows = q.n_sum_rows; r.C = bn.C; r.stage = c->bn_stage; r.sums_out = sums; r.tickets = c->bn_tickets;
    if (q.nseg > 1) { r.nseg = q.nseg; r.seg_stride = sslcr_ctx::kBnSlot; }
    TRY(launch_bn_finalize(r, st));
  } else if (!q.defer) {
    TRY(launch_bn_bwd_reduce(c->dtype, a, st));
  }
  *out = a;
  return 0;
}

int bn_bwd_sync(sslcr_ctx* c, double* sums, size_t count, hipStream_t st) {
  if (sharded(c) && c->bn_sync) TRYI(all_reduce(c, 0, sums, count, true, st));
  return 0;
}

int bn_bwd_end(sslcr_ctx* c, const BnBwdArgs& a, hipStream_t st) {
  auto book = [&](ProfRec& r) {
    const bool pool = a.pool_dy != nullptr;
    if (pool) r.name = c->dtype == DT_BF16 ? "sslcr::bn_bwd_apply_pool_kernel<unsigned short>" : "sslcr::bn_bwd_apply_pool_kernel<float>";
    else r.name = c->dtype == DT_BF16 ? "sslcr::bn_bwd_apply_kernel<unsigned short>" : "sslcr::bn_bwd_apply_kernel<float>";
    r.flops = 0.0;
    const double t = (double)a.pixels * a.C * c->esz();
    const double rd = (pool ? 0.25 * t + 0.25 * (double)a.pixels * a.C : t) + t + ((a.yact && !a.g_in_reduce) ? t : 0.0);
    r.bytes = rd + t + ((a.gout && !a.g_in_reduce) ? t : 0.0);
  };
  return check(profiled(c, 2, st, book, [&] { return launch_bn_bwd_apply(c->dtype, a, st); }), "launch_bn_bwd_apply");
}

int bn_backward(sslcr_net* n, const BnL& bn, const BnSaved& sv, const BnBwdReq& q, hipStream_t st) {
  sslcr_ctx* c = n->ctx;
  const bool segs = q.nseg > 1;
  double* sums = segs ? take_sums_n(c, q.nseg) : q.sum_rows ? c->bn_sums : take_sums_or_fixed(c);
  if (!sums) return fail("bn_backward: no ring slots for the segments");
  BnBwdArgs a;
  TRYI(bn_bwd_begin(n, bn, sv, q, st, sums, &a));
  if (!segs) TRYI(bn_bwd_sync(c, sums, 2 * (size_t)bn.C, st));
  return bn_bwd_end(c, a, st);
}

int wg_wait(sslcr_ctx* c, int kind, hipStream_t st) {
  if (c->wg_pending[kind]) {
    TRY(hipStreamWaitEvent(st, c->ev_wg_done[kind], 0));
    c->wg_pending[kind] = false;
  }
  return 0;
}
int wg_join(sslcr_ctx* c, hipStream_t waiter) {
  if (!c->wg_any) return 0;
  TRY(hipEventRecord(c->ev_wg_join, c->wg_stream));
  TRY(hipStreamWaitEvent(waiter, c->ev_wg_join, 0));
  return 0;
}

int wgrad_call(sslcr_net* n, const ConvL& L, const void* x, const void* dy, const BnSaved* pro, int N, int H, int W, int OH, int OW, hipStream_t st,
               int kind, int seg_images = 0, int seg_stride = 0) {
  if (!n->rg[L.pidx]) return 0;
  sslcr_ctx* c = n->ctx;
  WgradArgs a;
  memset(&a, 0, sizeof(a));
  a.x = x; a.dy = dy; a.dw = n->gw + n->goff[L.pidx];
  if (pro) { a.in_scale = pro->scale; a.in_shift = pro->shift; a.in_relu = 1; }
  a.N = N; a.H = H; a.W = W; a.C = L.cin; a.K = L.cout; a.R = L.k; a.S = L.k; a.stride = L.stride; a.pad = L.pad; a.OH = OH; a.OW = OW;
  a.seg_images = seg_images; a.seg_stride = seg_stride;
  if (kind < 0 || !c->use_wg || c->prof.on) {
    TRY(prof_wgrad(c, c->dtype, a, st));
    return 0;
  }
  if (!c->wg_stream) {
    TRY(hipStreamCreateWithFlags(&c->wg_stream, hipStreamNonBlocking));
    for (int k = 0; k < 3; ++k) {
      TRY(hipEventCreateWithFlags(&c->ev_wg_in[k], hipEventDisableTiming));
      TRY(hipEventCreateWithFlags(&c->ev_wg_done[k], hipEventDisableTiming));
    }
    TRY(hipEventCreateWithFlags(&c->ev_wg_join, hipEventDisableTiming));
  }
  TRY(hipEventRecord(c->ev_wg_in[kind], st));
  TRY(hipStreamWaitEvent(c->wg_stream, c->ev_wg_in[kind], 0));
  TRY(prof_wgrad(c, c->dtype, a, c->wg_stream));
  TRY(hipEventRecord(c->ev_wg_done[kind], c->wg_stream));
  c->wg_pending[kind] = true;
  c->wg_any = true;
  return 0;
}

int launch_bucket_allreduce(sslcr_net* n, int bucket, size_t lo, size_t hi, hipStream_t st) {
  sslcr_ctx* c = n->ctx;
  if (!sharded(c) || hi <= lo) return 0;
  TRY(hipEventRecord(c->ev_ready[bucket], st));
  TRY(hipStreamWaitEvent(c->comm_stream, c->ev_ready[bucket], 0));
  TRYI(wg_join(c, c->comm_stream));
  float* g = n->gw + lo;
  TRYI(all_reduce(c, 1, g, hi - lo, false, c->comm_stream));
  return 0;
}

int lowest_trainable(const sslcr_net* n) {
  for (int i = 0; i < 60; ++i)
    if (n->rg[i]) return i;
  return 60;
}

ConvArgs dgrad3x3_s1_args(const ConvL& L, const void* dy, void* dx, int N, int oh, int ow) {
  ConvArgs a = conv_args(L, dy, L.w_dg, dx, N, oh, ow);
  a.C = L.cout; a.K = L.cin; a.transposed = 0; a.PH = oh; a.PW = ow; a.OH = oh; a.OW = ow;
  return a;
}
ConvArgs with_bn1_mask(ConvArgs a, const void* raw, const BnSaved& s) {
  a.mask_x = raw; a.mask_scale = s.scale; a.mask_shift = s.shift; a.mask_mean = s.mean;
  return a;
}
unsigned parity_tap_mask(int ph, int pw) {
  unsigned m = 0;
  for (int r = 0; r < 3; ++r)
    for (int s = 0; s < 3; ++s)
      if (((ph + 1 - r) & 1) == 0 && ((pw + 1 - s) & 1) == 0) m |= 1u << (r * 3 + s);
  return m;
}

enum { kG = 1, kRaw2 = 2, kAct1 = 3, kRaw1 = 4, kRawD = 6, kKinds = 7 };
struct Backward {
  sslcr_net* n; sslcr_ctx* c; hipStream_t st;
  int dt, npass, N; size_t es; PassState* P; Dims d;
  int bn_stride;
  char* S; size_t unit;
  int kOut = 0, kXin = 5;
  int i; const BlockL* B;
  int oh, ow, xh, xw;
  size_t opix, so, si;
  bool c2_batched, seg_dg, seg_bn;

  char* buf(int kind, int p, size_t bytes) const { return S + (size_t)kind * npass * unit + (size_t)p * bytes; }
  char* dRaw0() const { return S + (size_t)kKinds * npass * unit; }
  int tap(int slot, const void* src, int h_, int w_, int c_) {
    if (!n->tap) return 0;
    const size_t bytes = (size_t)N * h_ * w_ * c_ * es;
    TRYI(n->tapbuf[i][slot].ensure(bytes));
    TRY(hipMemcpyAsync(n->tapbuf[i][slot].p, src, bytes, hipMemcpyDeviceToDevice, st));
    int* d4 = n->tapdims[i][slot];
    d4[0] = N; d4[1] = h_; d4[2] = w_; d4[3] = c_;
    return 0;
  }

  ConvArgs conv2_dgrad_segments_args(const void* dy, void* dx) const {
    ConvArgs m = with_bn1_mask(dgrad3x3_s1_args(B->c2, dy, dx, N * npass, oh, ow), P[0].blk[i].raw1, P[0].bn[B->b1.bidx]);
    m.seg_images = N; m.seg_stride = bn_stride;
    return m;
  }

  void enter(int blk) {
    i = blk; B = &n->blocks[i];
    oh = d.lh[i]; ow = d.lw[i];
    xh = i == 0 ? d.ph : d.lh[i - 1]; xw = i == 0 ? d.pw : d.lw[i - 1];
    opix = (size_t)N * oh * ow;
    so = opix * B->c2.cout * es; si = (size_t)N * xh * xw * B->c1.cin * es;
    c2_batched = false;
    if (npass > 1) {
      WgradArgs q;
      memset(&q, 0, sizeof(q));
      q.N = N * npass; q.H = oh; q.W = ow; q.C = B->c2.cin; q.K = B->c2.cout; q.R = 3; q.S = 3; q.stride = 1; q.pad = 1; q.OH = oh; q.OW = ow;
      c2_batched = wgrad_halo_tw(q) != 0 && (wgrad_halo_tw(q) == 16 || N % 2 == 0);
    }
    seg_dg = false;
    if (npass > 1 && segments_on() && !c->prof.on) {
      const ConvArgs m = conv2_dgrad_segments_args(nullptr, nullptr);
      const ConvPlan p = conv_plan(dt, m);
      seg_dg = tile16(p) && p.seg_ok && p.rows % npass == 0;
    }
    seg_bn = npass > 1 && segments_on() && !c->prof.on && !(sharded(c) && c->bn_sync) && c->bn_ring.p &&
             c->bn_ring_i + 2 * npass <= sslcr_ctx::kBnRing;
  }

  int bn2(int p, int nseg) {
    const PassState& ps = P[p];
    char *G = buf(kG, p, so), *dRaw2 = buf(kRaw2, p, so), *dRawD = buf(kRawD, p, so);
    TRYI(wg_wait(c, 0, st));
    if (B->has_ds) TRYI(wg_wait(c, 2, st));
    BnBwdReq q2, qd;
    q2.dy = buf(kOut, p, so); q2.x = ps.blk[i].raw2; q2.yact = ps.blk[i].y; q2.dx = dRaw2; q2.gout = G; q2.g_in_reduce = 1;
    qd.dy = G; qd.x = ps.blk[i].rawd; qd.dx = dRawD;
    q2.pixels = qd.pixels = opix * nseg; q2.count = qd.count = (double)opix;
    if (nseg > 1) { q2.nseg = qd.nseg = nseg; q2.seg_stride = qd.seg_stride = bn_stride; }
    if (!B->has_ds) TRYI(bn_backward(n, B->b2, ps.bn[B->b2.bidx], q2, st));
    else TRYI(nseg > 1 ? bn2_and_shortcut_segments(q2, qd) : bn2_and_shortcut(ps, q2, qd));
    if (p != 0) return 0;
    TRYI(tap(0, G, oh, ow, B->c2.cout));
    TRYI(tap(1, dRaw2, oh, ow, B->c2.cout));
    return B->has_ds ? tap(4, dRawD, oh, ow, B->ds.cout) : 0;
  }
  int bn2_and_shortcut_segments(const BnBwdReq& q2, const BnBwdReq& qd) {
    BnBwdArgs a2, ad;
    double* sums_2 = take_sums_n(c, npass);
    if (!sums_2) return fail("backbone_backward: ring slots");
    TRYI(bn_bwd_begin(n, B->b2, P[0].bn[B->b2.bidx], q2, st, sums_2, &a2));
    TRYI(bn_bwd_begin(n, B->bd, P[0].bn[B->bd.bidx], qd, st, sums_2 + 2 * B->b2.C, &ad));
    TRYI(bn_bwd_end(c, a2, st));
    return bn_bwd_end(c, ad, st);
  }
  int bn2_and_shortcut(const PassState& ps, BnBwdReq q2, BnBwdReq qd) {
    BnBwdArgs a2, ad;
    double* sums_2 = take_sums_or_fixed(c);
    q2.defer = qd.defer = true;
    TRYI(bn_bwd_begin(n, B->b2, ps.bn[B->b2.bidx], q2, st, sums_2, &a2));
    TRYI(bn_bwd_begin(n, B->bd, ps.bn[B->bd.bidx], qd, st, sums_2 + 2 * B->b2.C, &ad));
    const bool pair = bn_bwd_pair_ok(a2, ad);
    static const bool g_free = [] { const char* e = getenv("SSLCR_BN_PAIR_G"); return e && atoi(e) == 0; }();
    const int keep_g = (n->tap || !a2.yact_bits || !g_free) ? 1 : 0;
    if (pair) {
      TRY(launch_bn_bwd_reduce_pair(dt, a2, ad, keep_g, st));
    } else {
      TRY(launch_bn_bwd_reduce(dt, a2, st));
      TRY(launch_bn_bwd_reduce(dt, ad, st));
    }
    TRYI(bn_bwd_sync(c, sums_2, 4 * (size_t)B->b2.C, st));
    if (!pair) {
      TRYI(bn_bwd_end(c, a2, st));
      return bn_bwd_end(c, ad, st);
    }
    auto book = [&](ProfRec& r) {
      r.name = dt == DT_BF16 ? "sslcr::bn_bwd_apply_pair_kernel<unsigned short>" : "sslcr::bn_bwd_apply_pair_kernel<float>";
      r.flops = 0.0;
      r.bytes = (keep_g ? 5.0 : 5.0625) * (double)opix * B->b2.C * c->esz();
    };
    return check(profiled(c, 2, st, book, [&] { return launch_bn_bwd_apply_pair(dt, a2, ad, keep_g, st); }), "launch_bn_bwd_apply_pair");
  }

  int bn1(int p, int nseg, const float* rows, int nrows) {
    TRYI(wg_wait(c, 1, st));
    BnBwdReq q;
    q.dy = buf(kAct1, p, so); q.x = P[p].blk[i].raw1; q.relu_from_x = rows ? 0 : 1; q.dx = buf(kRaw1, p, so);
    q.pixels = opix * nseg; q.count = (double)opix; q.sum_rows = rows; q.n_sum_rows = nrows;
    if (nseg > 1) { q.nseg = nseg; q.seg_stride = bn_stride; }
    TRYI(bn_backward(n, B->b1, P[p].bn[B->b1.bidx], q, st));
    return p == 0 ? tap(3, q.dx, oh, ow, B->c1.cout) : 0;
  }
  int conv2_dgrad_bn1(int p) {
    ConvArgs a = dgrad3x3_s1_args(B->c2, buf(kRaw2, p, so), buf(kAct1, p, so), N, oh, ow);
    const ConvArgs m = with_bn1_mask(a, P[p].blk[i].raw1, P[p].bn[B->b1.bidx]);
    float* rows = nullptr; int nrows = 0;
    const ConvPlan pm = conv_plan(dt, m);
    if (tile16(pm)) {
      nrows = pm.rows;
      TRYI(partials_rows(c, nrows, m.K, &rows));
      a = m;
      a.stats = rows;
    }
    TRY(prof_conv(c, dt, a, st));
    if (p == 0) {
      TRYI(tap(2, a.y, oh, ow, B->c2.cin));
      n->tap_flags[i] = rows ? 1 : 0;
    }
    return bn1(p, 1, rows, nrows);
  }
  int conv2_dgrad_bn1_segments() {
    ConvArgs m = conv2_dgrad_segments_args(buf(kRaw2, 0, so), buf(kAct1, 0, so));
    float* rows = nullptr; int nrows = 0;
    TRYI(ensure_partials(c, m, &rows, &nrows));
    m.stats = rows;
    TRY(prof_conv(c, dt, m, st));
    TRYI(tap(2, m.y, oh, ow, B->c2.cin));
    n->tap_flags[i] = 1;
    if (seg_bn) return bn1(0, npass, rows, nrows);
    const int per = nrows / npass;
    for (int p = 0; p < npass; ++p) TRYI(bn1(p, 1, rows + (size_t)p * per * 2 * B->b1.C, per));
    return 0;
  }

  int conv2_wgrad(int p) { return wgrad_call(n, B->c2, P[p].blk[i].raw1, buf(kRaw2, p, so), &P[p].bn[B->b1.bidx], N, oh, ow, oh, ow, st, 0); }
  int wgrads() {
    if (c2_batched)
      TRYI(wgrad_call(n, B->c2, P[0].blk[i].raw1, buf(kRaw2, 0, so), &P[0].bn[B->b1.bidx], N * npass, oh, ow, oh, ow, st, 0, N, bn_stride));
    const char* X0 = i == 0 ? P[0].pooled : P[0].blk[i - 1].y;
    TRYI(wgrad_call(n, B->c1, X0, buf(kRaw1, 0, so), nullptr, N * npass, xh, xw, oh, ow, st, 1));
    if (B->has_ds) TRYI(wgrad_call(n, B->ds, X0, buf(kRawD, 0, so), nullptr, N * npass, xh, xw, oh, ow, st, 2));
    return 0;
  }

  int input_grad() {
    const int NB = N * npass;
    char* dXin = buf(kXin, 0, si);
    ConvArgs a = conv_args(B->c1, buf(kRaw1, 0, so), B->c1.w_dg, dXin, NB, oh, ow);
    a.C = B->c1.cout; a.K = B->c1.cin; a.transposed = (B->c1.stride == 1) ? 0 : 1; a.PH = xh; a.PW = xw; a.OH = xh; a.OW = xw;
    if (!B->has_ds) a.residual = buf(kG, 0, so);
    if (B->c1.stride == 1) {
      TRY(prof_conv(c, dt, a, st));
    } else {
      ConvArgs q4 = a;
      q4.pix_mul = 2; q4.PH = xh / 2; q4.PW = xw / 2; q4.par4 = 1;
      const bool one = xh % 2 == 0 && xw % 2 == 0 && conv_plan(dt, q4).par4_one_launch;
      if (one) TRY(prof_conv(c, dt, q4, st));
      for (int par = 0; par < (one ? 0 : 4); ++par) {
        ConvArgs q = a;
        const int ph = par >> 1, pw = par & 1;
        q.pix_mul = 2; q.pix_off_h = ph; q.pix_off_w = pw;
        q.PH = (xh - ph + 1) / 2; q.PW = (xw - pw + 1) / 2;
        if (q.PH <= 0 || q.PW <= 0) continue;
        q.tap_mask = parity_tap_mask(ph, pw);
        TRY(prof_conv(c, dt, q, st));
      }
    }
    if (B->has_ds) {
      ConvArgs s = conv_args(B->ds, buf(kRawD, 0, so), B->ds.w_dg, dXin, NB, oh, ow);
      s.C = B->ds.cout; s.K = B->ds.cin; s.stride = 1; s.pad = 0; s.PH = oh; s.PW = ow; s.OH = xh; s.OW = xw; s.osh = B->ds.stride;
      s.accumulate = 1;
      TRY(prof_conv(c, dt, s, st));
    }
    return tap(5, dXin, xh, xw, B->c1.cin);
  }

  int block() {
    if (seg_bn) TRYI(bn2(0, npass));
    for (int p = 0; p < npass; ++p) {
      if (!seg_bn) TRYI(bn2(p, 1));
      if (!c2_batched) TRYI(conv2_wgrad(p));
      if (!seg_dg) TRYI(conv2_dgrad_bn1(p));
    }
    if (seg_dg) TRYI(conv2_dgrad_bn1_segments());
    return wgrads();
  }

  int stem(int p) {
    const PassState& ps = P[p];
    const PoolSrc pool{buf(kOut, p, (size_t)N * d.ph * d.pw * 64 * es), ps.argmax, d.oh0, d.ow0, d.ph, d.pw, ps.pooled};
    const size_t spix = (size_t)N * d.oh0 * d.ow0;
    BnBwdReq q;
    q.x = ps.raw0; q.relu_from_x = 1; q.pixels = spix; q.count = (double)spix; q.pool = &pool;
    StemWgradArgs w;
    memset(&w, 0, sizeof(w));
    w.x = ps.x; w.x2 = ps.x2; w.n_split = ps.n_split; w.dy = dRaw0(); w.dw = n->gw + n->goff[0];
    w.N = N; w.H = ps.H; w.W = ps.W; w.OH = d.oh0; w.OW = d.ow0; w.in_f32 = ps.in_f32;
    if (!(n->rg[0] && c->fuse_stem_bwd)) {
      q.dx = dRaw0();
      TRYI(bn_backward(n, n->bn0, ps.bn[0], q, st));
      if (n->rg[0]) TRY(launch_stem_wgrad(dt, w, st));
      return 0;
    }
    BnBwdArgs a;
    double* sums0 = take_sums_or_fixed(c);
    TRYI(bn_bwd_begin(n, n->bn0, ps.bn[0], q, st, sums0, &a));
    TRYI(bn_bwd_sync(c, sums0, 2 * 64, st));
    w.dy = nullptr;
    auto book = [&](ProfRec& r) {
      r.name = dt == DT_BF16 ? "sslcr::stem_wgrad_kernel<unsigned short, pool>" : "sslcr::stem_wgrad_kernel<float, pool>";
      r.flops = 0.0;
      const double t = (double)spix * 64 * c->esz();
      r.bytes = 0.25 * t + 0.25 * (double)spix * 64 + t + (double)N * 3 * ps.H * ps.W * (ps.in_f32 ? 4 : 1);
    };
    return check(profiled(c, 2, st, book, [&] { return launch_stem_wgrad_pool(dt, w, a, st); }), "launch_stem_wgrad_pool");
  }
};

int backbone_backward(sslcr_net* n, int npass, hipStream_t st) {
  sslcr_ctx* c = n->ctx;
  const int low = lowest_trainable(n);
  if (low >= 60) return 0;
  Backward b;
  b.n = n; b.c = c; b.st = st; b.dt = c->dtype; b.es = c->esz();
  b.P = n->pass; b.npass = npass; b.N = n->pass[0].N;
  b.d = make_dims(n->pass[0].H, n->pass[0].W);
  b.bn_stride = npass > 1 ? (int)(n->pass[1].bn[0].scale - n->pass[0].bn[0].scale) : 0;
  const Dims& d = b.d; const int N = b.N;
  b.unit = (((size_t)N * d.ph * d.pw * 64 * b.es) + 255) & ~(size_t)255;
  const size_t stem_sz = (((size_t)N * d.oh0 * d.ow0 * 64 * b.es) + 255) & ~(size_t)255;
  TRYI(c->scratch.ensure(kKinds * npass * b.unit + stem_sz));
  b.S = (char*)c->scratch.p;
  size_t hi_pending = n->goff[60];
  int bucket = 1;
  for (int p = 0; p < npass; ++p)
    TRY(launch_avgpool_bwd(b.dt, n->dE[p], b.buf(b.kOut, p, (size_t)N * d.lh[7] * d.lw[7] * 512 * b.es), N, d.lh[7] * d.lw[7], 512, st));
  for (int i = 7; i >= 0; --i) {
    b.enter(i);
    TRYI(b.block());
    const bool need_dx = low < b.B->pstart;
    if (need_dx) {
      TRYI(b.input_grad());
      const int t = b.kOut; b.kOut = b.kXin; b.kXin = t;
    }
    if (i == 6 || i == 4 || i == 2) {
      TRYI(launch_bucket_allreduce(n, bucket++, n->goff[b.B->pstart], hi_pending, st));
      hi_pending = n->goff[b.B->pstart];
    }
    if (!need_dx) break;
  }
  if (low < 3)
    for (int p = 0; p < npass; ++p) TRYI(b.stem(p));
  TRYI(launch_bucket_allreduce(n, bucket, 0, hi_pending, st));
  return 0;
}

int net_forward(sslcr_net* n, int train, const void* const* xs, int in_f32, int N, int H, int W, float* feats, float* logits, hipStream_t st) {
  if (!(train ? n->packed_train : n->packed_eval)) TRYI(sslcr_net_pack(n, train ? 1 : 2, st));
  const int npass_ = n->triplet ? 3 : 1;
  if (n->n8 > 0 && !n->f8_cal[train ? 0 : 1]) {
    n->f8_calib_pass = true;
    TRYI(alloc_heads(n, N));
    int rc = 0;
    for (int i = 0; i < npass_ && rc == 0 && train; ++i)
      rc = backbone_forward_train(n, n->pass[i], xs[i], in_f32, N, H, W, n->triplet ? 1 : 3, st);
    if (!train) rc = backbone_forward_eval(n, xs, npass_, in_f32, N, H, W, n->dE, st);
    n->f8_calib_pass = false;
    if (rc) return rc;
    n->f8_cal[train ? 0 : 1] = true;
  }
  if (n->n8 > 0) TRY(launch_fp8_scale_update(n->f8slots, n->n8, st));
  if (train) n->packed_eval = false;
  const int npass = n->triplet ? 3 : 1;
  TRYI(alloc_heads(n, N));
  float* E[3] = {nullptr, nullptr, nullptr};
  const bool segs = train && npass == 3 && segments_servable(n, N, H, W);
  if (train) n->last_segments = segs;
  if (segs) {
    TRYI(backbone_forward_train_segments(n, xs, in_f32, N, H, W, st));
    for (int i = 0; i < npass; ++i) E[i] = n->pass[i].E;
  }
  for (int i = 0; i < npass && !segs && train; ++i) {
    TRYI(backbone_forward_train(n, n->pass[i], xs[i], in_f32, N, H, W, n->triplet ? 1 : 3, st));
    E[i] = n->pass[i].E;
  }
  if (!train) {
    for (int i = 0; i < npass; ++i) E[i] = n->dE[i];
    TRYI(backbone_forward_eval(n, xs, npass, in_f32, N, H, W, E, st));
  }
  TRYI(heads_forward(n, E, npass, N, st));
  if (feats) TRY(hipMemcpyAsync(feats, n->feats, (size_t)N * 768 * 4, hipMemcpyDeviceToDevice, st));
  if (logits) TRY(hipMemcpyAsync(logits, n->logits, (size_t)N * n->ncls * 4, hipMemcpyDeviceToDevice, st));
  n->last_N = N; n->last_npass = train ? npass : 0;
// ... 609 lines not shown
```

### ssl_cr_histo_amd/csrc/kernels.hpp

```cpp
#pragma once
#include <string>

#include "common.hpp"
#include "launch.hpp"
#include "../../include/sslcr.h"

namespace sslcr {

using ConvArgs = sslcr_conv_desc;
using WgradArgs = sslcr_wgrad_desc;
using StemArgs = sslcr_stem_desc;
using StemWgradArgs = sslcr_stem_wgrad_desc;
using BnFinalizeArgs = sslcr_bn_finalize_desc;
using BnActArgs = sslcr_bn_act_desc;
using PoolFwdArgs = sslcr_pool_fwd_desc;
using PoolBwdArgs = sslcr_pool_bwd_desc;
using BnBwdArgs = sslcr_bn_bwd_desc;
using LossArgs = sslcr_loss_desc;
using LossOpts = sslcr_loss_opts;
using TensorDesc = sslcr_tensor_desc;
using OptArgs = sslcr_opt_desc;
using PackArgs = sslcr_pack_desc;
using Fp8Args = sslcr_fp8_desc;
using PackFp8Args = sslcr_pack_fp8_desc;

inline std::string karg(const char* s) { return s; }
inline std::string karg(bool v) { return v ? "true" : "false"; }
inline std::string karg(int v) { return std::to_string(v); }
template <class... A>
std::string kname(const char* kernel, A... args) {
  std::string s = std::string("sslcr::") + kernel;
  const char* sep = "<";
  ((s += sep + karg(args), sep = ", "), ...);
  return sizeof...(A) ? s + ">" : s;
}
template <typename T> constexpr const char* ktype() { return sizeof(T) == 2 ? "unsigned short" : "float"; }
struct InstName {
  template <class I> const char* operator()(I) const {
    static const std::string s = I::spell();
    return s.c_str();
  }
};

enum class ConvRoute { H16, PP64, HALO256, HALO, S2, S2D, DMA, IGEMM };
struct ConvPlan {
  ConvRoute route;
  int param;
  int rows;
  bool seg_ok;
  bool ok;
  bool par4_one_launch;
  const char* name;
};
ConvPlan conv_plan(int dtype, const ConvArgs& a);
hipError_t launch_conv(int dtype, const ConvArgs& a, const ConvPlan& p, hipStream_t st);
inline hipError_t launch_conv(int dtype, const ConvArgs& a, hipStream_t st) { return launch_conv(dtype, a, conv_plan(dtype, a), st); }
inline const char* conv_kernel_name(int dtype, const ConvArgs& a) { return conv_plan(dtype, a).name; }
inline int conv_partials_rows(const ConvArgs& a) { return conv_plan(DT_BF16, a).rows; }
inline bool conv_segments_ok(int dtype, const ConvArgs& a) { return conv_plan(dtype, a).seg_ok; }
enum class WgradRoute { HALO, HALO_DMA, S2, GENERIC };
struct WgradPlan {
  WgradRoute route;
  int tw, KH;
  bool ok;
  const char* name;
};
WgradPlan wgrad_plan(int dtype, const WgradArgs& a);
hipError_t launch_wgrad(int dtype, const WgradArgs& a, const WgradPlan& p, hipStream_t st);
inline hipError_t launch_wgrad(int dtype, const WgradArgs& a, hipStream_t st) { return launch_wgrad(dtype, a, wgrad_plan(dtype, a), st); }
inline const char* wgrad_kernel_name(int dtype, const WgradArgs& a) { return wgrad_plan(dtype, a).name; }
inline bool wgrad_dma_used(int dtype, const WgradArgs& a) { return wgrad_plan(dtype, a).route == WgradRoute::HALO_DMA; }
int conv_igemm_rows(const ConvArgs& a);
hipError_t launch_igemm(int dtype, const ConvArgs& a, hipStream_t st);
const char* conv_igemm_name(int dtype, const ConvArgs& a);
int conv_halo_tw(int dtype, const ConvArgs& a);
int conv_halo_tiles(const ConvArgs& a, int tw);
hipError_t launch_conv_halo(int dtype, const ConvArgs& a, int tw, hipStream_t st);
const char* conv_halo_name(int dtype, const ConvArgs& a, int tw);
int conv_halo256_mode(int dtype, const ConvArgs& a);
int conv_halo256_tiles(const ConvArgs& a, int mode);
hipError_t launch_conv_halo256(int dtype, const ConvArgs& a, int mode, hipStream_t st);
const char* conv_halo256_name(int dtype, const ConvArgs& a, int mode);
int conv_h16_mode(const ConvArgs& a, int q);
int conv_h16_rows(const ConvArgs& a);
hipError_t launch_conv_h16(int dtype, const ConvArgs& a, int mode, hipStream_t st);
const char* conv_h16_name(int dtype, const ConvArgs& a, int mode);
bool conv_pp64_ok(int dtype, const ConvArgs& a);
hipError_t launch_conv_pp64(const ConvArgs& a, hipStream_t st);
const char* conv_pp64_name(const ConvArgs& a);
int conv_pp64_rows(const ConvArgs& a);
int conv_dma_bp(int dtype, const ConvArgs& a);
int conv_dma_rows(const ConvArgs& a, int bp);
hipError_t launch_conv_dma(int dtype, const ConvArgs& a, int bp, hipStream_t st);
const char* conv_dma_name(int dtype, int bp);
bool conv_s2_ok(int dtype, const ConvArgs& a);
bool conv_s2_pair_ok(int dtype, const ConvArgs& a, const ConvArgs& d);
int conv_s2_rows(const ConvArgs& a);
hipError_t launch_conv_s2(const ConvArgs& a, const ConvArgs* d, hipStream_t st);
const char* conv_s2_name(const ConvArgs& a, bool pair);
bool conv_s2d_ok(int dtype, const ConvArgs& a);
hipError_t launch_conv_s2d(const ConvArgs& a, hipStream_t st);
const char* conv_s2d_name();
int conv_fp8_mode(const ConvArgs& a);
int conv_fp8_rows(const ConvArgs& a);
const char* conv_fp8_name(const ConvArgs& a);
hipError_t launch_conv_fp8(const ConvArgs& a, const Fp8Args& q, hipStream_t st);
hipError_t launch_pack_fp8(const PackFp8Args& a, hipStream_t st);
hipError_t launch_fp8_scale_update(float* slots, int n, hipStream_t st);
hipError_t launch_wgrad_generic(int dtype, const WgradArgs& a, hipStream_t st);
const char* wgrad_generic_name(int dtype, const WgradArgs& a);
int wgrad_halo_tw(const WgradArgs& a);
int wgrad_halo_splits(const WgradArgs& a, int tw, int kh);
hipError_t launch_wgrad_halo(int dtype, const WgradArgs& a, const WgradPlan& p, hipStream_t st);
const char* wgrad_halo_name(int dtype, int tw, int kh);
bool wgrad_dma_ok(int dtype, const WgradArgs& a, int splits);
const char* wgrad_dma_name(const WgradArgs& a, int tw);
hipError_t launch_wgrad_dma(const WgradArgs& a, int tw, int tps, int ntiles, int splits, void* slabs, hipStream_t st);
hipError_t launch_probe_tr16(const uint16_t* in, const int* byte_addr, uint16_t* out, hipStream_t st);
bool wgrad_s2_ok(int dtype, const WgradArgs& a);
hipError_t launch_wgrad_s2(const WgradArgs& a, hipStream_t st);
const char* wgrad_s2_name(const WgradArgs& a);
hipError_t launch_stem(int dtype, const StemArgs& a, hipStream_t st);
int stem_partials_rows(const StemArgs& a);
hipError_t launch_stem_wgrad(int dtype, const StemWgradArgs& a, hipStream_t st);
hipError_t launch_stem_wgrad_pool(int dtype, const StemWgradArgs& a, const sslcr_bn_bwd_desc& b, hipStream_t st);
bool stem_pool_ok(int dtype, const StemArgs& a, int POH, int POW);
hipError_t launch_stem_pool(int dtype, const StemArgs& a, int POH, int POW, hipStream_t st);
hipError_t launch_bn_finalize(const BnFinalizeArgs& a, hipStream_t st);
hipError_t launch_bn_act(int dtype, const BnActArgs& a, hipStream_t st);
hipError_t launch_bn_relu_maxpool(int dtype, const PoolFwdArgs& a, hipStream_t st);
hipError_t launch_maxpool_relu_bwd(int dtype, const PoolBwdArgs& a, hipStream_t st);
hipError_t launch_avgpool_fwd(int dtype, const void* x, float* y, int N, int HW, int C, hipStream_t st);
hipError_t launch_avgpool_bwd(int dtype, const float* dy, void* dx, int N, int HW, int C, hipStream_t st);
hipError_t launch_bn_bwd_reduce(int dtype, const BnBwdArgs& a, hipStream_t st);
hipError_t launch_bn_bwd_apply(int dtype, const BnBwdArgs& a, hipStream_t st);
bool bn_bwd_pair_ok(const BnBwdArgs& a, const BnBwdArgs& b);
hipError_t launch_bn_bwd_reduce_pair(int dtype, const BnBwdArgs& a, const BnBwdArgs& b, int keep_g, hipStream_t st);
hipError_t launch_bn_bwd_apply_pair(int dtype, const BnBwdArgs& a, const BnBwdArgs& b, int from_g, hipStream_t st);
hipError_t launch_bn_param_grads(const double* sums, const float* invstd, float* dgamma, float* dbeta, int C, hipStream_t st);
hipError_t launch_bn_param_grads_scaled(const double* sums, const float* invstd, float* dgamma, float* dbeta, int C, float scale, hipStream_t st);
hipError_t launch_linear_fwd(const float* x, const float* w, const float* b, float* y, int M, int N, int K, int relu, hipStream_t st);
hipError_t launch_linear_bwd(const float* x, const float* w, const float* dy, const float* yact, float* dx, float* dw, float* db,
                             int M, int N, int K, int dx_accumulate, float* scratch, hipStream_t st);
hipError_t launch_loss(const LossArgs& a, hipStream_t st);
hipError_t launch_loss_ex(const LossArgs& a, const LossOpts& o, hipStream_t st);
hipError_t launch_ce_denominator(const int64_t* y, int n, int C, const float* w, int ignore_index, float* out2, hipStream_t st);
inline LossOpts loss_opts_default() {
  LossOpts o;
  o.class_weight = nullptr; o.label_smoothing = 0.f; o.ignore_index = -100; o.threshold = 0.f; o.temperature = 0.f;
  o.denominator = nullptr; o.stats = nullptr;
  return o;
}
inline bool loss_opts_is_default(const LossOpts& o) {
  return !o.class_weight && o.label_smoothing == 0.f && o.ignore_index == -100 && o.threshold == 0.f && o.temperature == 0.f &&
         !o.denominator && !o.stats;
}
inline const char* loss_opts_error(int kind, int C, const LossOpts& o) {
  if (loss_opts_is_default(o)) return nullptr;
  if (kind != 1 && kind != 2) return "loss options apply to the cross-entropy kinds (1, 2) only, not to the MSE kinds (0, 3)";
  if (C > 64) return "C > 64";
  if (!(o.label_smoothing >= 0.f && o.label_smoothing < 1.f)) return "label_smoothing outside [0, 1)";
  if (!(o.threshold >= 0.f && o.threshold <= 1.f)) return "threshold outside [0, 1]";
  if (!(o.temperature >= 0.f)) return "temperature < 0";
  if (kind == 2 && (o.threshold != 0.f || o.temperature != 0.f)) return "threshold / temperature need the consistency term (kind 1)";
  return nullptr;
}
hipError_t launch_softmax_col(const float* logits, float* out, int n, int C, int col, hipStream_t st);
hipError_t launch_predict(const sslcr_predict_desc& a, hipStream_t st);
hipError_t launch_wsi_gather(const sslcr_wsi_gather_desc& a, hipStream_t st);
hipError_t launch_weak_augment(const sslcr_weak_aug_desc& a, hipStream_t st);
hipError_t launch_hed_colour(const sslcr_colour_aug_desc& a, hipStream_t st);
hipError_t launch_brightness_contrast(const sslcr_brightness_contrast_desc& a, hipStream_t st);
hipError_t launch_augv2(const sslcr_augv2_desc& a, hipStream_t st);
hipError_t launch_augv2_colour(const sslcr_augv2_colour_desc& a, hipStream_t st);
struct OptTable { OptArgs row[SSLCR_MAX_OPT_GROUPS]; };
inline OptTable opt_table_noop() {
  OptTable t;
  for (OptArgs& o : t.row) { o.kind = 1; o.lr = 0.f; o.beta1 = 0.f; o.beta2 = 0.f; o.eps = 0.f; o.wd = 0.f; o.momentum = 1.f; o.bc1 = 1.f; o.bc2 = 1.f; o.first_step = 0; o.grad_scale = 0.f; }
  return t;
}
hipError_t launch_optimizer(const TensorDesc* d_descs, int ntensors, int max_n, const OptTable& tab, const float* coef, hipStream_t st);
constexpr int OPT_CHUNK = 2048;
constexpr int OPT_TILE = 16 * 16 * 9;
constexpr int OPT_CHUNK_GROUP_SHIFT = 24;
hipError_t launch_optimizer_chunks(const TensorDesc* d_descs, const void* d_chunks , int nchunks,
                                   const OptTable& tab, const float* coef, hipStream_t st);
constexpr int GRAD_NORM_BLOCKS = 1024;
hipError_t launch_grad_norm(const float* g, size_t n, float max_norm, double* partials , float* out2, hipStream_t st);
hipError_t launch_grad_accumulate(float* dst, const float* src, size_t n, hipStream_t st);
hipError_t launch_axpby(float* p, float* q, size_t n, float alpha, int copy_back, hipStream_t st);
hipError_t launch_fill(float* p, size_t n, float v, hipStream_t st);
hipError_t launch_pack_conv(int dtype, const PackArgs& a, hipStream_t st);
hipError_t launch_pack_stem(int dtype, const PackArgs& a, hipStream_t st);
hipError_t launch_copy2d(float* dst, long ldd, const float* src, long lds, int rows, int w, int accumulate, hipStream_t st);
hipError_t launch_copy2d_multi(float* dst, long ldd, int ndst, long dstep, const float* src, long lds, int nsrc, long sstep, int rows, int w,
                               hipStream_t st);
hipError_t launch_unpack_grad(const float* g, float* out, int K, int C, int RS, hipStream_t st);
int fail(const char* fmt, ...);
int check(hipError_t e, const char* what);

}
```

### ssl_cr_histo_amd/csrc/wgrad_halo.hip

```cpp

#include "kernels.hpp"

namespace sslcr {

template <typename T, int TW, int KH>
__global__ __launch_bounds__(256 * KH, 2) void wgrad3x3_halo_kernel(const WgradArgs a, int tiles_per_split, int ntiles, f32x4_t* partials) {
  constexpr int EPC = Elem<T>::EPC;
  constexpr bool BF = Elem<T>::DT == DT_BF16;
  constexpr int RB = 64 * sizeof(T);
  constexpr int CPR = RB / 16;
  constexpr int TH = 8;
  constexpr int NI = 128 / (TH * TW);
  constexpr int HH = TH + 2, HWD = TW + 2;
  constexpr int HP = NI * HH * HWD;
  constexpr int NT = 256 * KH;
  constexpr int YL = 128 * CPR / 256;
  constexpr int HL = (HP * CPR + NT - 1) / NT;
  constexpr int YROWS = 256 / CPR, HROWS = NT / CPR;
  constexpr int PITCH = BF ? (TW == 16 ? 24 : 16) : HWD;
  constexpr int YH = 128 * RB;
  constexpr int YBUF = KH * YH, HBUF = NI * HH * PITCH * RB;
  constexpr int BUF = YBUF + HBUF;
  constexpr int NBUF = KH;
  extern __shared__ __attribute__((aligned(16))) char smem[];

  const int tid = threadIdx.x, lane = tid & 63;
  const int wave = (tid >> 6) & 3, kh = tid >> 8;
  const int li = lane & 15, g = lane >> 4;
  const int gx = a.K / (64 * KH), gy = a.C / 64, GT = gx * gy, splits = (int)gridDim.x / GT;
  const OuterInner oi = xcd_outer_inner(blockIdx.x, splits, GT, false);
  const int bz = oi.outer, bt = oi.inner;
  const int by = bt / gx, bx = bt - by * gx;
  const int k0 = bx * (64 * KH), c0 = by * 64;
  const int chunk = tid % CPR, prow = tid / CPR;
  const int chunky = tid % (CPR * KH), prowy = tid / (CPR * KH);
  const bool xform = a.in_scale != nullptr;
  float* s_aff = reinterpret_cast<float*>(smem + NBUF * BUF);
  const int nseg = a.seg_images > 0 ? a.N / a.seg_images : 1;
  for (int i = tid; i < nseg * 64; i += NT) {
    const int sg = i >> 6, ch = i & 63;
    s_aff[sg * 128 + ch] = xform ? a.in_scale[(size_t)sg * a.seg_stride + c0 + ch] : 1.f;
    s_aff[sg * 128 + 64 + ch] = xform ? a.in_shift[(size_t)sg * a.seg_stride + c0 + ch] : 0.f;
  }
  const int tiles_w = a.W / TW, tiles_h = a.H / TH;
  const int t_begin = bz * tiles_per_split;
  int t_end = t_begin + tiles_per_split;
  if (t_end > ntiles) t_end = ntiles;
  if (t_begin >= t_end) {
    if (partials) {
      const size_t wg = ((size_t)bz * gy + by) * gx + bx;
      for (int e = 0; e < 36; ++e) partials[(wg * 36 + e) * NT + tid] = f32x4_t{0.f, 0.f, 0.f, 0.f};
    }
    return;
  }
  const char* xg = reinterpret_cast<const char*>(a.x);
  const char* dyg = reinterpret_cast<const char*>(a.dy);

  int rel_y[YL], rel_h[HL];
  static_assert(HL <= 16, "edge mask holds 16 halo entries");
  unsigned long long edge = 0;
  unsigned hvalid = 0;
#pragma unroll
  for (int i = 0; i < YL; ++i) {
    const int p = prowy + YROWS * i;
    const int ni = p / (TH * TW), rem = p - ni * (TH * TW);
    const int ph = rem / TW, pw = rem - ph * TW;
    rel_y[i] = (ni * a.H + ph) * a.W + pw;
  }
#pragma unroll
  for (int i = 0; i < HL; ++i) {
    const int hp = prow + HROWS * i;
    rel_h[i] = 0;
    if (hp < HP) {
      const int ni = hp / (HH * HWD), rem = hp - ni * (HH * HWD);
      const int hr = rem / HWD, hc = rem - hr * HWD;
      rel_h[i] = (ni * a.H + hr - 1) * a.W + hc - 1;
      hvalid |= 1u << i;
      edge |= (unsigned long long)((hr == 0) | ((hr == HH - 1) << 1) | ((hc == 0) << 2) | ((hc == HWD - 1) << 3)) << (4 * i);
    }
  }
  const size_t ybase = ((size_t)k0 + chunky * EPC) * sizeof(T), xbase = ((size_t)c0 + chunk * EPC) * sizeof(T);

  u32x4_t yreg[YL], hreg[HL];
  unsigned hin = 0;
  int seg_ld = 0;
  auto load_regs = [&](int tile) {
    int t = tile;
    const int tw_i = t % tiles_w; t /= tiles_w;
    const int th_i = t % tiles_h;
    const int n0 = (t / tiles_h) * NI;
    const int h0 = th_i * TH, w0 = tw_i * TW;
    seg_ld = a.seg_images > 0 ? n0 / a.seg_images : 0;
    const int origin = (n0 * a.H + h0) * a.W + w0;
    const unsigned long long out =
        (unsigned long long)((h0 == 0) | ((h0 + TH >= a.H) << 1) | ((w0 == 0) << 2) | ((w0 + TW >= a.W) << 3)) * 0x1111111111111111ull;
#pragma unroll
    for (int i = 0; i < YL; ++i)
      yreg[i] = ld16(dyg + (size_t)(origin + rel_y[i]) * a.K * sizeof(T) + ybase);
    hin = hvalid;
    const unsigned long long bad = edge & out;
#pragma unroll
    for (int i = 0; i < HL; ++i) {
      const bool ok = ((hvalid >> i) & 1u) && !((bad >> (4 * i)) & 0xfull);
      hreg[i] = ld16(xg + (size_t)(origin + (ok ? rel_h[i] : 0)) * a.C * sizeof(T) + xbase);
      if (!ok) hin &= ~(1u << i);
    }
  };
  auto swz = [](int row) { return (row >> 1) & 3; };
  auto chunk_off_of = [&](int row, int ch) {
    if (!BF) return ch * 16;
    return (((ch >> 1) ^ swz(row)) << 5) | ((ch & 1) << 4);
  };
  auto chunk_off = [&](int row) { return chunk_off_of(row, chunk); };
  auto store_lds = [&](int buf) {
    char* yb = smem + buf * BUF;
    char* hb = yb + YBUF;
    float r_scale[EPC], r_shift[EPC];
    if (xform) {
#pragma unroll
      for (int e = 0; e < EPC; ++e) { r_scale[e] = s_aff[seg_ld * 128 + chunk * EPC + e]; r_shift[e] = s_aff[seg_ld * 128 + 64 + chunk * EPC + e]; }
    }
#pragma unroll
    for (int i = 0; i < YL; ++i) {
      const int p = prowy + YROWS * i;
      st16(yb + (chunky / CPR) * YH + p * RB + chunk_off_of(p, chunky % CPR), yreg[i]);
    }
#pragma unroll
    for (int i = 0; i < HL; ++i) {
      const int hp = prow + HROWS * i;
      if (hp >= HP) continue;
      const int hni = hp / (HH * HWD), hrem = hp - hni * (HH * HWD);
      const int hpl = (hni * HH + hrem / HWD) * PITCH + hrem % HWD;
      u32x4_t v = hreg[i];
      if (!((hin >> i) & 1u)) {
        v = u32x4_t{0u, 0u, 0u, 0u};
      } else if (xform) {
        float f[EPC];
        Elem<T>::unpack(v, f);
#pragma unroll
        for (int e = 0; e < EPC; ++e) {
          float q = fmaf(f[e], r_scale[e], r_shift[e]);
          f[e] = a.in_relu ? fmaxf(q, 0.f) : q;
        }
        v = Elem<T>::pack(f);
      }
      st16(hb + hpl * RB + chunk_off(hpl), v);
    }
  };

  f32x4_t acc[9][4];
#pragma unroll
  for (int t = 0; t < 9; ++t)
#pragma unroll
    for (int c = 0; c < 4; ++c) acc[t][c] = f32x4_t{0.f, 0.f, 0.f, 0.f};

  auto hpix = [&](int p) {
    if (TW == 16) return (p >> 4) * PITCH + (p & 15);
    return (p >> 6) * (HH * PITCH) + ((p >> 3) & 7) * PITCH + (p & 7);
  };

  load_regs(t_begin);
  __syncthreads();
  store_lds(0);
  __syncthreads();
  int buf = 0;
  for (int tile = t_begin; tile < t_end; ++tile) {
    const bool more = tile + 1 < t_end;
    if (more) load_regs(tile + 1);
    const char* yb = smem + buf * BUF;
    const char* hb = yb + YBUF;
    if constexpr (BF) {
      const int pl = 16 * (g >> 1) + 4 * (g & 1) + (li >> 2);
      constexpr int HI = (TW == 16 ? 8 : PITCH) * RB;
      int Aoff[4], Boff[3];
#pragma unroll
      for (int t4 = 0; t4 < 4; ++t4) Aoff[t4] = pl * RB + ((t4 ^ swz(pl)) << 5) + (li & 3) * 8;
#pragma unroll
      for (int sx = 0; sx < 3; ++sx) {
        const int hp = hpix(pl) + sx;
        Boff[sx] = hp * RB + ((wave ^ swz(hp)) << 5) + (li & 3) * 8;
      }
      bf16x8_t bfr[2];
      auto bfrag_of = [&](int q, int t) {
        const int qoff = (hpix(q * 32) + (t / 3) * PITCH) * RB;
        return tr_pair(hb + Boff[t % 3] + qoff, hb + Boff[t % 3] + qoff + HI);
      };
      auto qstep = [&](const int q, const int par) {
        bf16x8_t af[4];
#pragma unroll
        for (int t4 = 0; t4 < 4; ++t4) {
          const char* pa = yb + kh * YH + q * 32 * RB + Aoff[t4];
          af[t4] = tr_pair(pa, pa + 8 * RB);
        }
#pragma unroll
        for (int t = 0; t < 9; ++t) {
          bfr[(t + 1 + par) & 1] = t < 8 ? bfrag_of(q, t + 1) : bfrag_of(q < 3 ? q + 1 : 3, 0);
          __builtin_amdgcn_sched_barrier(0);
#pragma unroll
          for (int t4 = 0; t4 < 4; ++t4)
            acc[t][t4] = __builtin_amdgcn_mfma_f32_16x16x32_bf16(af[t4], bfr[(t + par) & 1], acc[t][t4], 0, 0, 0);
          __builtin_amdgcn_sched_barrier(0);
        }
      };
      bfr[0] = bfrag_of(0, 0);
#pragma unroll 1
      for (int q2 = 0; q2 < 2; ++q2) {
        qstep(2 * q2, 0);
        qstep(2 * q2 + 1, 1);
      }
    } else {
#pragma unroll 2
      for (int q = 0; q < 32; ++q) {
        const int p = 4 * q + g;
        float av[4];
#pragma unroll
        for (int t4 = 0; t4 < 4; ++t4) av[t4] = *reinterpret_cast<const float*>(yb + p * RB + (16 * t4 + li) * 4);
        const int hp0 = hpix(p);
#pragma unroll
        for (int t = 0; t < 9; ++t) {
          const int toff = (t / 3) * PITCH + (t % 3);
          const float bv = *reinterpret_cast<const float*>(hb + (hp0 + toff) * RB + (16 * wave + li) * 4);
#pragma unroll
          for (int t4 = 0; t4 < 4; ++t4) acc[t][t4] = __builtin_amdgcn_mfma_f32_16x16x4f32(av[t4], bv, acc[t][t4], 0, 0, 0);
        }
      }
    }
    if (NBUF == 1) {
      __syncthreads();
      if (more) store_lds(0);
    } else if (more) {
      store_lds(buf ^ 1);
    }
    __syncthreads();
    if (NBUF == 2) buf ^= 1;
  }

  if (partials) {
    const size_t wg = ((size_t)bz * gy + by) * gx + bx;
    f32x4_t* sp = partials + wg * 36 * NT + tid;
#pragma unroll
    for (int t = 0; t < 9; ++t)
#pragma unroll
      for (int t4 = 0; t4 < 4; ++t4) sp[(size_t)(t * 4 + t4) * NT] = acc[t][t4];
    return;
  }
#pragma unroll
  for (int t = 0; t < 9; ++t)
#pragma unroll
    for (int t4 = 0; t4 < 4; ++t4)
#pragma unroll
      for (int j = 0; j < 4; ++j) {
        const int k = k0 + 64 * kh + 16 * t4 + 4 * g + j;
        a.dw[((size_t)k * 9 + t) * a.C + c0 + 16 * wave + li] += acc[t][t4][j];
      }
}

__global__ __launch_bounds__(1024) void wgrad_fold_kernel(const f32x4_t* __restrict__ partials, float* dw, int C, int gx, int gy, int splits,
                                                         int ev, int kh_n, int mode) {
  __shared__ f32x4_t red[16][64];
  const int NT = 256 * kh_n, taps = ev >> 2;
  const size_t per_wg = (size_t)ev * NT;
  const size_t v = (size_t)blockIdx.x * blockDim.x + threadIdx.x;
  const int ZG = blockDim.y, zl = threadIdx.y;
  const int tid = (int)(v % NT);
  const int e = (int)((v / NT) % ev);
  const int bxy = (int)(v / per_wg);
  const int bx = bxy % gx, by = bxy / gx;
  f32x4_t sum = {0.f, 0.f, 0.f, 0.f};
  const size_t zstride = (size_t)gy * gx * per_wg;
  const f32x4_t* p = partials + (size_t)zl * zstride + ((size_t)by * gx + bx) * per_wg + (size_t)e * NT + tid;
  for (int z = zl; z < splits; z += ZG, p += (size_t)ZG * zstride) {
    const f32x4_t q = __builtin_nontemporal_load(p);
    sum[0] += q[0]; sum[1] += q[1]; sum[2] += q[2]; sum[3] += q[3];
  }
  if (ZG > 1) {
    red[zl][threadIdx.x] = sum;
    __syncthreads();
    if (zl != 0) return;
    for (int y = 1; y < ZG; ++y) {
      const f32x4_t q = red[y][threadIdx.x];
      sum[0] += q[0]; sum[1] += q[1]; sum[2] += q[2]; sum[3] += q[3];
    }
  }
  const int lane = tid & 63, wave = (tid >> 6) & 3, kh = tid >> 8;
  const int li = lane & 15, g = lane >> 4;
  if (mode == 1) {
    const int r = e >> 1, s = (e & 1) * 4 + (li >> 2), c = li & 3;
    if (s < 7 && c < 3) {
#pragma unroll
      for (int j = 0; j < 4; ++j) dw[(((16 * wave + 4 * g + j) * 3 + c) * 7 + r) * 7 + s] += sum[j];
    }
    return;
  }
  const int t = e >> 2, t4 = e & 3;
#pragma unroll
  for (int j = 0; j < 4; ++j) {
    const int k = bx * 64 * kh_n + 64 * kh + 16 * t4 + 4 * g + j;
    dw[((size_t)k * taps + t) * C + by * 64 + 16 * wave + li] += sum[j];
  }
}
static hipError_t fold_launch(const void* slabs, float* dw, int C, int gx, int gy, int splits, int ev, int kh_n, int mode, hipStream_t st) {
  const size_t nvec = (size_t)gx * gy * ev * 256 * kh_n;
  int zg = 1;
  while (zg < 16 && splits >= 8 * zg) zg *= 2;
  int vx = 64;
  while (vx > 16 && nvec / vx < (size_t)(2 * device_cus())) vx >>= 1;
  hipLaunchKernelGGL(wgrad_fold_kernel, dim3((unsigned)(nvec / vx)), dim3(vx, zg), 0, st, reinterpret_cast<const f32x4_t*>(slabs), dw, C, gx, gy,
                     splits, ev, kh_n, mode);
  return hipGetLastError();
}
hipError_t launch_wgrad_fold(const void* slabs, float* dw, int C, int gx, int gy, int splits, int taps, int kh_n, hipStream_t st) {
  return fold_launch(slabs, dw, C, gx, gy, splits, taps * 4, kh_n, 0, st);
}
hipError_t launch_stem_wgrad_fold(const void* slabs, float* dw, int nwg, hipStream_t st) {
  return fold_launch(slabs, dw, 0, 1, 1, nwg, 14, 1, 1, st);
}

int wgrad_halo_tw(const WgradArgs& a) {
  if (a.R != 3 || a.S != 3 || a.stride != 1 || a.pad != 1 || a.OH != a.H || a.OW != a.W) return 0;
  if (a.C % 64 != 0 || a.K % 64 != 0 || a.H % 8 != 0) return 0;
  if (a.W % 16 == 0) return 16;
  if (a.W % 8 == 0 && a.N % 2 == 0) return 8;
  return 0;
}

static int wh_splits(const WgradArgs& a, int TW, int KH, int* tps_out, int* ntiles_out) {
  const int NI = 128 / (8 * TW);
  const int ntiles = (a.N / NI) * (a.H / 8) * (a.W / TW);
  const int kc = (a.K / (64 * KH)) * (a.C / 64);
  int splits = cdiv((KH == 1 ? 2 : 1) * device_cus(), kc);
  const int max_splits = cdiv(ntiles, 16);
  if (splits > max_splits) splits = max_splits;
  if (splits < 1) splits = 1;
  const int tps = cdiv(ntiles, splits);
  if (tps_out) *tps_out = tps;
  if (ntiles_out) *ntiles_out = ntiles;
  return cdiv(ntiles, tps);
}
int wgrad_halo_splits(const WgradArgs& a, int tw, int kh) { return wh_splits(a, tw, kh, nullptr, nullptr); }

template <typename T, int TW, int KH>
struct WgradHaloInst { static std::string spell() { return kname("wgrad3x3_halo_kernel", ktype<T>(), TW, KH); } };

template <typename T, int TW, int KH>
static hipError_t launch_wh(WgradHaloInst<T, TW, KH>, const WgradArgs& a, bool dma, hipStream_t st) {
  constexpr bool BF = Elem<T>::DT == DT_BF16;
  constexpr int NI = 128 / (8 * TW);
  int tps, ntiles;
  const int splits = wh_splits(a, TW, KH, &tps, &ntiles);
  const int nseg = a.seg_images > 0 ? a.N / a.seg_images : 1;
  if (nseg > 8 || (a.seg_images > 0 && (a.N % a.seg_images != 0 || a.seg_images % NI != 0))) return hipErrorInvalidValue;
  const int gx = a.K / (64 * KH), gy = a.C / 64;
  const size_t slab_bytes = splits > 1 ? (size_t)gx * gy * splits * 36 * 256 * KH * sizeof(f32x4_t) : 0;
  return with_slabs(st, slab_bytes,
    [&](f32x4_t* slabs) {
      if (dma) return launch_wgrad_dma(a, TW, tps, ntiles, splits, slabs, st);
      const int pitch = BF ? (TW == 16 ? 24 : 16) : TW + 2;
      const size_t lds = (size_t)KH * (128 * KH + NI * 10 * pitch) * 64 * sizeof(T) + 512 * nseg;
      return launch_lds<wgrad3x3_halo_kernel<T, TW, KH>>(dim3(gx * gy * splits), dim3(256 * KH), lds, KH == 1 ? 96 * 1024 : 160 * 1024, st, a, tps,
                                                         ntiles, slabs);
    },
    [&](f32x4_t* slabs) { return launch_wgrad_fold(slabs, a.dw, a.C, gx, gy, splits, 9, KH, st); });
}

template <class F>
static auto wh_pick(int dtype, int tw, int kh, F&& f) {
  if (dtype == DT_BF16) {
    if (kh == 2) return tw == 16 ? f(WgradHaloInst<bf16_t, 16, 2>{}) : f(WgradHaloInst<bf16_t, 8, 2>{});
    return tw == 16 ? f(WgradHaloInst<bf16_t, 16, 1>{}) : f(WgradHaloInst<bf16_t, 8, 1>{});
  }
  return tw == 16 ? f(WgradHaloInst<float, 16, 1>{}) : f(WgradHaloInst<float, 8, 1>{});
}
hipError_t launch_wgrad_halo(int dtype, const WgradArgs& a, const WgradPlan& p, hipStream_t st) {
  return wh_pick(dtype, p.tw, p.KH, [&](auto inst) { return launch_wh(inst, a, p.route == WgradRoute::HALO_DMA, st); });
}
const char* wgrad_halo_name(int dtype, int tw, int kh) { return wh_pick(dtype, tw, kh, InstName{}); }

}
```

Measured before the change: 69580.

## Fuse BN backward apply into 3x3 halo weight-gradient kernel for 64-channel layers

Adds a fused kernel path that computes the BN backward apply (dx from dy and raw x with per-channel coefficients) while staging the output gradient tile for the 3x3 stride-1 weight-gradient halo kernel. It also writes dx to global memory in the same pass. The engine defers the BN apply for conv1/conv2 of basic blocks so the wgrad kernel can perform it, removing a separate elementwise pass and a re-read of dx. The path is limited to bf16, C=K=64 layers with a single pass and no segments, and is enabled by default through an environment flag. It adds register pressure and extra global stores inside the wgrad kernel.

```diff
diff --git a/include/sslcr.h b/include/sslcr.h
--- a/include/sslcr.h
+++ b/include/sslcr.h
@@ -158,6 +158,9 @@
 int sslcr_bn_bwd_apply(int dtype, const sslcr_bn_bwd_desc* d, void* stream);
 int sslcr_bn_param_grads(const double* sums, const float* invstd, float* dgamma, float* dbeta, int C, void* stream);
 int sslcr_stem_wgrad_pool(int dtype, const sslcr_stem_wgrad_desc* w, const sslcr_bn_bwd_desc* bn, void* stream);
+int sslcr_conv2d_wgrad_bn(int dtype, const sslcr_wgrad_desc* w, const sslcr_bn_bwd_desc* bn, void* stream);
+int sslcr_conv2d_wgrad_bn_ok(int dtype, const sslcr_wgrad_desc* w, const sslcr_bn_bwd_desc* bn);
+const char* sslcr_conv2d_wgrad_bn_kernel_name(int dtype, const sslcr_wgrad_desc* w, const sslcr_bn_bwd_desc* bn);
 
 int sslcr_linear_fwd(const float* x, const float* w, const float* b, float* y, int M, int N, int K, int relu, void* stream);
 int sslcr_linear_bwd(const float* x, const float* w, const float* dy, const float* yact, float* dx, float* dw, float* db,
diff --git a/ssl_cr_histo_amd/_lib.py b/ssl_cr_histo_amd/_lib.py
--- a/ssl_cr_histo_amd/_lib.py
+++ b/ssl_cr_histo_amd/_lib.py
@@ -94,6 +94,9 @@
     "sslcr_pack_conv_fp8": (i32, [P(PackFp8Desc), vp]),
     "sslcr_conv2d_wgrad": (i32, [i32, P(WgradDesc), vp]),
     "sslcr_conv2d_wgrad_kernel_name": (C.c_char_p, [i32, P(WgradDesc)]),
+    "sslcr_conv2d_wgrad_bn": (i32, [i32, P(WgradDesc), P(BnBwdDesc), vp]),
+    "sslcr_conv2d_wgrad_bn_ok": (i32, [i32, P(WgradDesc), P(BnBwdDesc)]),
+    "sslcr_conv2d_wgrad_bn_kernel_name": (C.c_char_p, [i32, P(WgradDesc), P(BnBwdDesc)]),
     "sslcr_probe_tr16": (i32, [vp, vp, vp, vp]),
     "sslcr_stem_conv": (i32, [i32, P(StemDesc), vp]),
     "sslcr_stem_partial_rows": (i32, [P(StemDesc)]),
diff --git a/ssl_cr_histo_amd/csrc/capi.cpp b/ssl_cr_histo_amd/csrc/capi.cpp
--- a/ssl_cr_histo_amd/csrc/capi.cpp
+++ b/ssl_cr_histo_amd/csrc/capi.cpp
@@ -29,7 +29,7 @@
 
 extern "C" {
 
-int sslcr_version(void) { return 12; }
+int sslcr_version(void) { return 13; }
 const char* sslcr_last_error(void) { return g_err; }
 
 int sslcr_conv2d(int dtype, const sslcr_conv_desc* d, void* stream) {
@@ -76,6 +76,22 @@
   NEED(d->C % 64 == 0 && d->K % 64 == 0, "C,K % 64");
   NEED((d->R == 3 && d->S == 3) || (d->R == 1 && d->S == 1), "3x3 or 1x1");
   return check(launch_wgrad(dtype, *d, (hipStream_t)stream), "conv2d_wgrad");
+}
+
+const char* sslcr_conv2d_wgrad_bn_kernel_name(int dtype, const sslcr_wgrad_desc* w, const sslcr_bn_bwd_desc* bn) {
+  return w && bn ? wgrad_bn_plan(dtype, *w, *bn).name : "";
+}
+int sslcr_conv2d_wgrad_bn_ok(int dtype, const sslcr_wgrad_desc* w, const sslcr_bn_bwd_desc* bn) {
+  return (w && bn && wgrad_bn_plan(dtype, *w, *bn).ok) ? 1 : 0;
+}
+int sslcr_conv2d_wgrad_bn(int dtype, const sslcr_wgrad_desc* w, const sslcr_bn_bwd_desc* bn, void* stream) {
+  DT_OK(dtype);
+  NEED(w && w->x && w->dw && bn && bn->x && bn->dx && bn->sums && bn->mean && bn->invstd && bn->scale, "null tensor");
+  NEED(bn->g_in_reduce ? bn->gout != nullptr : bn->dy != nullptr, "no gradient (dy, or gout with g_in_reduce)");
+  const WgradPlan p = wgrad_bn_plan(dtype, *w, *bn);
+  NEED(p.ok, "pair of descriptors not served by the fused kernel (sslcr_conv2d_wgrad_bn_ok): bf16, 3x3 / 1, C = K = 64, W % 16, H % 8, "
+             "no mask, no segments, no pool source");
+  return check(launch_wgrad_bn(dtype, *w, *bn, p, (hipStream_t)stream), "conv2d_wgrad_bn");
 }
 
 int sslcr_probe_tr16(const uint16_t* in, const int* byte_addr, uint16_t* out, void* stream) {
diff --git a/ssl_cr_histo_amd/csrc/common.hpp b/ssl_cr_histo_amd/csrc/common.hpp
--- a/ssl_cr_histo_amd/csrc/common.hpp
+++ b/ssl_cr_histo_amd/csrc/common.hpp
@@ -64,11 +64,13 @@
 template <> struct PackH<bf16_t> {
   typedef __bf16 bf16x2_t __attribute__((ext_vector_type(2)));
   typedef float f32x2_t __attribute__((ext_vector_type(2)));
+  __device__ static __forceinline__ uint32_t pair(float lo, float hi) {
+    return __builtin_bit_cast(uint32_t, __builtin_convertvector(f32x2_t{lo, hi}, bf16x2_t));
+  }
   __device__ static __forceinline__ u32x4_t run(const float* f) {
     u32x4_t v;
 #pragma unroll
-    for (int i = 0; i < 4; ++i)
-      v[i] = __builtin_bit_cast(uint32_t, __builtin_convertvector(f32x2_t{f[2 * i], f[2 * i + 1]}, bf16x2_t));
+    for (int i = 0; i < 4; ++i) v[i] = pair(f[2 * i], f[2 * i + 1]);
     return v;
   }
 };
diff --git a/ssl_cr_histo_amd/csrc/conv_route.cpp b/ssl_cr_histo_amd/csrc/conv_route.cpp
--- a/ssl_cr_histo_amd/csrc/conv_route.cpp
+++ b/ssl_cr_histo_amd/csrc/conv_route.cpp
@@ -94,8 +94,20 @@
     case WgradRoute::HALO_DMA: return launch_wgrad_halo(dtype, a, p, st);
     case WgradRoute::S2: return launch_wgrad_s2(a, st);
     case WgradRoute::GENERIC: return launch_wgrad_generic(dtype, a, st);
+    case WgradRoute::HALO_BN: break;
   }
   return hipErrorInvalidValue;
 }
 
+WgradPlan wgrad_bn_plan(int dtype, const WgradArgs& a, const BnBwdArgs& b) {
+  if (wgrad_halo_bn_ok(dtype, a, b)) return {WgradRoute::HALO_BN, 16, 1, true, wgrad_halo_bn_name()};
+  WgradPlan p = wgrad_plan(dtype, a);
+  p.ok = false;
+  return p;
 }
+hipError_t launch_wgrad_bn(int dtype, const WgradArgs& a, const BnBwdArgs& b, const WgradPlan& p, hipStream_t st) {
+  if (!p.ok || p.route != WgradRoute::HALO_BN || dtype != DT_BF16) return hipErrorInvalidValue;
+  return launch_wgrad_halo_bn(a, b, st);
+}
+
+}
diff --git a/ssl_cr_histo_amd/csrc/engine.cpp b/ssl_cr_histo_amd/csrc/engine.cpp
--- a/ssl_cr_histo_amd/csrc/engine.cpp
+++ b/ssl_cr_histo_amd/csrc/engine.cpp
@@ -357,6 +357,17 @@
   return profiled(c, 1, st, book, [&] { return launch_wgrad(dt, a, plan, st); });
 }
 
+hipError_t prof_wgrad_bn(sslcr_ctx* c, int dt, const WgradArgs& a, const BnBwdArgs& b, const WgradPlan& plan, hipStream_t st) {
+  auto book = [&](ProfRec& r) {
+    const double es = c->esz();
+    const double M = (double)a.N * a.OH * a.OW;
+    r.flops = 2.0 * M * a.K * a.C * a.R * a.S;
+    r.bytes = ((double)a.N * a.H * a.W * a.C + 3.0 * M * a.K) * es + (double)a.K * a.R * a.S * a.C * 4.0;
+    r.name = plan.name;
+  };
+  return profiled(c, 1, st, book, [&] { return launch_wgrad_bn(dt, a, b, plan, st); });
+}
+
 inline bool tile16(const ConvPlan& p) { return p.route == ConvRoute::H16 || p.route == ConvRoute::PP64; }
 
 constexpr int kMaxSeg = 3;
@@ -1061,7 +1072,7 @@
   return check(profiled(c, 2, st, book, [&] { return launch_bn_bwd_apply(c->dtype, a, st); }), "launch_bn_bwd_apply");
 }
 
-int bn_backward(sslcr_net* n, const BnL& bn, const BnSaved& sv, const BnBwdReq& q, hipStream_t st) {
+int bn_backward(sslcr_net* n, const BnL& bn, const BnSaved& sv, const BnBwdReq& q, hipStream_t st, BnBwdArgs* held = nullptr) {
   sslcr_ctx* c = n->ctx;
   const bool segs = q.nseg > 1;
   double* sums = segs ? take_sums_n(c, q.nseg) : q.sum_rows ? c->bn_sums : take_sums_or_fixed(c);
@@ -1069,6 +1080,7 @@
   BnBwdArgs a;
   TRYI(bn_bwd_begin(n, bn, sv, q, st, sums, &a));
   if (!segs) TRYI(bn_bwd_sync(c, sums, 2 * (size_t)bn.C, st));
+  if (held) { *held = a; return 0; }
   return bn_bwd_end(c, a, st);
 }
 
@@ -1086,16 +1098,21 @@
   return 0;
 }
 
-int wgrad_call(sslcr_net* n, const ConvL& L, const void* x, const void* dy, const BnSaved* pro, int N, int H, int W, int OH, int OW, hipStream_t st,
-               int kind, int seg_images = 0, int seg_stride = 0) {
-  if (!n->rg[L.pidx]) return 0;
-  sslcr_ctx* c = n->ctx;
+WgradArgs wgrad_args(sslcr_net* n, const ConvL& L, const void* x, const void* dy, const BnSaved* pro, int N, int H, int W, int OH, int OW,
+                     int seg_images = 0, int seg_stride = 0) {
   WgradArgs a;
   memset(&a, 0, sizeof(a));
   a.x = x; a.dy = dy; a.dw = n->gw + n->goff[L.pidx];
   if (pro) { a.in_scale = pro->scale; a.in_shift = pro->shift; a.in_relu = 1; }
   a.N = N; a.H = H; a.W = W; a.C = L.cin; a.K = L.cout; a.R = L.k; a.S = L.k; a.stride = L.stride; a.pad = L.pad; a.OH = OH; a.OW = OW;
   a.seg_images = seg_images; a.seg_stride = seg_stride;
+  return a;
+}
+int wgrad_call(sslcr_net* n, const ConvL& L, const void* x, const void* dy, const BnSaved* pro, int N, int H, int W, int OH, int OW, hipStream_t st,
+               int kind, int seg_images = 0, int seg_stride = 0) {
+  if (!n->rg[L.pidx]) return 0;
+  sslcr_ctx* c = n->ctx;
+  const WgradArgs a = wgrad_args(n, L, x, dy, pro, N, H, W, OH, OW, seg_images, seg_stride);
   if (kind < 0 || !c->use_wg || c->prof.on) {
     TRY(prof_wgrad(c, c->dtype, a, st));
     return 0;
@@ -1204,6 +1221,33 @@
              c->bn_ring_i + 2 * npass <= sslcr_ctx::kBnRing;
   }
 
+  struct HeldBn { bool on = false; BnBwdArgs a; WgradArgs w; WgradPlan plan; };
+  HeldBn held[2];
+  int bn_backward_before_wgrad(int k, const BnL& bn, const BnSaved& sv, const BnBwdReq& q, const ConvL& L, const WgradArgs& w) {
+    static const bool enabled = [] { const char* e = getenv("SSLCR_WGRAD_BN"); return !e || atoi(e) != 0; }();
+    held[k].on = false;
+    const bool launch_stream = !c->use_wg || c->prof.on;
+    if (!(enabled && dt == DT_BF16 && npass == 1 && q.nseg <= 1 && launch_stream && n->rg[L.pidx])) return bn_backward(n, bn, sv, q, st);
+    BnBwdArgs a;
+    TRYI(bn_backward(n, bn, sv, q, st, &a));
+    const WgradPlan plan = wgrad_bn_plan(dt, w, a);
+    if (!plan.ok) return bn_bwd_end(c, a, st);
+    held[k].on = true; held[k].a = a; held[k].w = w; held[k].plan = plan;
+    return 0;
+  }
+  int wgrad_fused(int k, int tap_slot) {
+    HeldBn& h = held[k];
+    h.on = false;
+    TRY(prof_wgrad_bn(c, dt, h.w, h.a, h.plan, st));
+    return tap(tap_slot, h.a.dx, oh, ow, h.w.K);
+  }
+  WgradArgs conv2_wgrad_args(int p) const {
+    return wgrad_args(n, B->c2, P[p].blk[i].raw1, buf(kRaw2, p, so), &P[p].bn[B->b1.bidx], N, oh, ow, oh, ow);
+  }
+  WgradArgs conv1_wgrad_args() const {
+    return wgrad_args(n, B->c1, i == 0 ? P[0].pooled : P[0].blk[i - 1].y, buf(kRaw1, 0, so), nullptr, N * npass, xh, xw, oh, ow);
+  }
+
   int bn2(int p, int nseg) {
     const PassState& ps = P[p];
     char *G = buf(kG, p, so), *dRaw2 = buf(kRaw2, p, so), *dRawD = buf(kRawD, p, so);
@@ -1214,11 +1258,11 @@
     qd.dy = G; qd.x = ps.blk[i].rawd; qd.dx = dRawD;
     q2.pixels = qd.pixels = opix * nseg; q2.count = qd.count = (double)opix;
     if (nseg > 1) { q2.nseg = qd.nseg = nseg; q2.seg_stride = qd.seg_stride = bn_stride; }
-    if (!B->has_ds) TRYI(bn_backward(n, B->b2, ps.bn[B->b2.bidx], q2, st));
+    if (!B->has_ds) TRYI(bn_backward_before_wgrad(0, B->b2, ps.bn[B->b2.bidx], q2, B->c2, conv2_wgrad_args(p)));
     else TRYI(nseg > 1 ? bn2_and_shortcut_segments(q2, qd) : bn2_and_shortcut(ps, q2, qd));
     if (p != 0) return 0;
     TRYI(tap(0, G, oh, ow, B->c2.cout));
-    TRYI(tap(1, dRaw2, oh, ow, B->c2.cout));
+    if (!held[0].on) TRYI(tap(1, dRaw2, oh, ow, B->c2.cout));
     return B->has_ds ? tap(4, dRawD, oh, ow, B->ds.cout) : 0;
   }
   int bn2_and_shortcut_segments(const BnBwdReq& q2, const BnBwdReq& qd) {
@@ -1264,8 +1308,8 @@
     q.dy = buf(kAct1, p, so); q.x = P[p].blk[i].raw1; q.relu_from_x = rows ? 0 : 1; q.dx = buf(kRaw1, p, so);
     q.pixels = opix * nseg; q.count = (double)opix; q.sum_rows = rows; q.n_sum_rows = nrows;
     if (nseg > 1) { q.nseg = nseg; q.seg_stride = bn_stride; }
-    TRYI(bn_backward(n, B->b1, P[p].bn[B->b1.bidx], q, st));
-    return p == 0 ? tap(3, q.dx, oh, ow, B->c1.cout) : 0;
+    TRYI(bn_backward_before_wgrad(1, B->b1, P[p].bn[B->b1.bidx], q, B->c1, conv1_wgrad_args()));
+    return p == 0 && !held[1].on ? tap(3, q.dx, oh, ow, B->c1.cout) : 0;
   }
   int conv2_dgrad_bn1(int p) {
     ConvArgs a = dgrad3x3_s1_args(B->c2, buf(kRaw2, p, so), buf(kAct1, p, so), N, oh, ow);
@@ -1299,12 +1343,16 @@
     return 0;
   }
 
-  int conv2_wgrad(int p) { return wgrad_call(n, B->c2, P[p].blk[i].raw1, buf(kRaw2, p, so), &P[p].bn[B->b1.bidx], N, oh, ow, oh, ow, st, 0); }
+  int conv2_wgrad(int p) {
+    if (held[0].on) return wgrad_fused(0, 1);
+    return wgrad_call(n, B->c2, P[p].blk[i].raw1, buf(kRaw2, p, so), &P[p].bn[B->b1.bidx], N, oh, ow, oh, ow, st, 0);
+  }
   int wgrads() {
     if (c2_batched)
       TRYI(wgrad_call(n, B->c2, P[0].blk[i].raw1, buf(kRaw2, 0, so), &P[0].bn[B->b1.bidx], N * npass, oh, ow, oh, ow, st, 0, N, bn_stride));
     const char* X0 = i == 0 ? P[0].pooled : P[0].blk[i - 1].y;
-    TRYI(wgrad_call(n, B->c1, X0, buf(kRaw1, 0, so), nullptr, N * npass, xh, xw, oh, ow, st, 1));
+    if (held[1].on) TRYI(wgrad_fused(1, 3));
+    else TRYI(wgrad_call(n, B->c1, X0, buf(kRaw1, 0, so), nullptr, N * npass, xh, xw, oh, ow, st, 1));
     if (B->has_ds) TRYI(wgrad_call(n, B->ds, X0, buf(kRawD, 0, so), nullptr, N * npass, xh, xw, oh, ow, st, 2));
     return 0;
   }
diff --git a/ssl_cr_histo_amd/csrc/kernels.hpp b/ssl_cr_histo_amd/csrc/kernels.hpp
--- a/ssl_cr_histo_amd/csrc/kernels.hpp
+++ b/ssl_cr_histo_amd/csrc/kernels.hpp
@@ -58,7 +58,7 @@
 inline const char* conv_kernel_name(int dtype, const ConvArgs& a) { return conv_plan(dtype, a).name; }
 inline int conv_partials_rows(const ConvArgs& a) { return conv_plan(DT_BF16, a).rows; }
 inline bool conv_segments_ok(int dtype, const ConvArgs& a) { return conv_plan(dtype, a).seg_ok; }
-enum class WgradRoute { HALO, HALO_DMA, S2, GENERIC };
+enum class WgradRoute { HALO, HALO_DMA, S2, GENERIC, HALO_BN };
 struct WgradPlan {
   WgradRoute route;
   int tw, KH;
@@ -69,6 +69,8 @@
 hipError_t launch_wgrad(int dtype, const WgradArgs& a, const WgradPlan& p, hipStream_t st);
 inline hipError_t launch_wgrad(int dtype, const WgradArgs& a, hipStream_t st) { return launch_wgrad(dtype, a, wgrad_plan(dtype, a), st); }
 inline const char* wgrad_kernel_name(int dtype, const WgradArgs& a) { return wgrad_plan(dtype, a).name; }
+WgradPlan wgrad_bn_plan(int dtype, const WgradArgs& a, const BnBwdArgs& b);
+hipError_t launch_wgrad_bn(int dtype, const WgradArgs& a, const BnBwdArgs& b, const WgradPlan& p, hipStream_t st);
 inline bool wgrad_dma_used(int dtype, const WgradArgs& a) { return wgrad_plan(dtype, a).route == WgradRoute::HALO_DMA; }
 int conv_igemm_rows(const ConvArgs& a);
 hipError_t launch_igemm(int dtype, const ConvArgs& a, hipStream_t st);
@@ -113,6 +115,9 @@
 int wgrad_halo_splits(const WgradArgs& a, int tw, int kh);
 hipError_t launch_wgrad_halo(int dtype, const WgradArgs& a, const WgradPlan& p, hipStream_t st);
 const char* wgrad_halo_name(int dtype, int tw, int kh);
+bool wgrad_halo_bn_ok(int dtype, const WgradArgs& a, const BnBwdArgs& b);
+hipError_t launch_wgrad_halo_bn(const WgradArgs& a, const BnBwdArgs& b, hipStream_t st);
+const char* wgrad_halo_bn_name();
 bool wgrad_dma_ok(int dtype, const WgradArgs& a, int splits);
 const char* wgrad_dma_name(const WgradArgs& a, int tw);
 hipError_t launch_wgrad_dma(const WgradArgs& a, int tw, int tps, int ntiles, int splits, void* slabs, hipStream_t st);
diff --git a/ssl_cr_histo_amd/csrc/wgrad_halo.hip b/ssl_cr_histo_amd/csrc/wgrad_halo.hip
--- a/ssl_cr_histo_amd/csrc/wgrad_halo.hip
+++ b/ssl_cr_histo_amd/csrc/wgrad_halo.hip
@@ -1,3 +1,5 @@
+
+#include <stdlib.h>
 
 #include "kernels.hpp"
 
@@ -5,254 +7,17 @@
 
 template <typename T, int TW, int KH>
 __global__ __launch_bounds__(256 * KH, 2) void wgrad3x3_halo_kernel(const WgradArgs a, int tiles_per_split, int ntiles, f32x4_t* partials) {
-  constexpr int EPC = Elem<T>::EPC;
-  constexpr bool BF = Elem<T>::DT == DT_BF16;
-  constexpr int RB = 64 * sizeof(T);
-  constexpr int CPR = RB / 16;
-  constexpr int TH = 8;
-  constexpr int NI = 128 / (TH * TW);
-  constexpr int HH = TH + 2, HWD = TW + 2;
-  constexpr int HP = NI * HH * HWD;
-  constexpr int NT = 256 * KH;
-  constexpr int YL = 128 * CPR / 256;
-  constexpr int HL = (HP * CPR + NT - 1) / NT;
-  constexpr int YROWS = 256 / CPR, HROWS = NT / CPR;
-  constexpr int PITCH = BF ? (TW == 16 ? 24 : 16) : HWD;
-  constexpr int YH = 128 * RB;
-  constexpr int YBUF = KH * YH, HBUF = NI * HH * PITCH * RB;
-  constexpr int BUF = YBUF + HBUF;
-  constexpr int NBUF = KH;
-  extern __shared__ __attribute__((aligned(16))) char smem[];
-
-  const int tid = threadIdx.x, lane = tid & 63;
-  const int wave = (tid >> 6) & 3, kh = tid >> 8;
-  const int li = lane & 15, g = lane >> 4;
-  const int gx = a.K / (64 * KH), gy = a.C / 64, GT = gx * gy, splits = (int)gridDim.x / GT;
-  const OuterInner oi = xcd_outer_inner(blockIdx.x, splits, GT, false);
-  const int bz = oi.outer, bt = oi.inner;
-  const int by = bt / gx, bx = bt - by * gx;
-  const int k0 = bx * (64 * KH), c0 = by * 64;
-  const int chunk = tid % CPR, prow = tid / CPR;
-  const int chunky = tid % (CPR * KH), prowy = tid / (CPR * KH);
-  const bool xform = a.in_scale != nullptr;
-  float* s_aff = reinterpret_cast<float*>(smem + NBUF * BUF);
-  const int nseg = a.seg_images > 0 ? a.N / a.seg_images : 1;
-  for (int i = tid; i < nseg * 64; i += NT) {
-    const int sg = i >> 6, ch = i & 63;
-    s_aff[sg * 128 + ch] = xform ? a.in_scale[(size_t)sg * a.seg_stride + c0 + ch] : 1.f;
-    s_aff[sg * 128 + 64 + ch] = xform ? a.in_shift[(size_t)sg * a.seg_stride + c0 + ch] : 0.f;
-  }
-  const int tiles_w = a.W / TW, tiles_h = a.H / TH;
-  const int t_begin = bz * tiles_per_split;
-  int t_end = t_begin + tiles_per_split;
-  if (t_end > ntiles) t_end = ntiles;
-  if (t_begin >= t_end) {
-    if (partials) {
-      const size_t wg = ((size_t)bz * gy + by) * gx + bx;
-      for (int e = 0; e < 36; ++e) partials[(wg * 36 + e) * NT + tid] = f32x4_t{0.f, 0.f, 0.f, 0.f};
-    }
-    return;
-  }
-  const char* xg = reinterpret_cast<const char*>(a.x);
-  const char* dyg = reinterpret_cast<const char*>(a.dy);
-
-  int rel_y[YL], rel_h[HL];
-  static_assert(HL <= 16, "edge mask holds 16 halo entries");
-  unsigned long long edge = 0;
-  unsigned hvalid = 0;
-#pragma unroll
-  for (int i = 0; i < YL; ++i) {
-    const int p = prowy + YROWS * i;
-    const int ni = p / (TH * TW), rem = p - ni * (TH * TW);
-    const int ph = rem / TW, pw = rem - ph * TW;
-    rel_y[i] = (ni * a.H + ph) * a.W + pw;
-  }
-#pragma unroll
-  for (int i = 0; i < HL; ++i) {
-    const int hp = prow + HROWS * i;
-    rel_h[i] = 0;
-    if (hp < HP) {
-      const int ni = hp / (HH * HWD), rem = hp - ni * (HH * HWD);
-      const int hr = rem / HWD, hc = rem - hr * HWD;
-      rel_h[i] = (ni * a.H + hr - 1) * a.W + hc - 1;
-      hvalid |= 1u << i;
-      edge |= (unsigned long long)((hr == 0) | ((hr == HH - 1) << 1) | ((hc == 0) << 2) | ((hc == HWD - 1) << 3)) << (4 * i);
-    }
-  }
-  const size_t ybase = ((size_t)k0 + chunky * EPC) * sizeof(T), xbase = ((size_t)c0 + chunk * EPC) * sizeof(T);
-
-  u32x4_t yreg[YL], hreg[HL];
-  unsigned hin = 0;
-  int seg_ld = 0;
-  auto load_regs = [&](int tile) {
-    int t = tile;
-    const int tw_i = t % tiles_w; t /= tiles_w;
-    const int th_i = t % tiles_h;
-    const int n0 = (t / tiles_h) * NI;
-    const int h0 = th_i * TH, w0 = tw_i * TW;
-    seg_ld = a.seg_images > 0 ? n0 / a.seg_images : 0;
-    const int origin = (n0 * a.H + h0) * a.W + w0;
-    const unsigned long long out =
-        (unsigned long long)((h0 == 0) | ((h0 + TH >= a.H) << 1) | ((w0 == 0) << 2) | ((w0 + TW >= a.W) << 3)) * 0x1111111111111111ull;
-#pragma unroll
-    for (int i = 0; i < YL; ++i)
-      yreg[i] = ld16(dyg + (size_t)(origin + rel_y[i]) * a.K * sizeof(T) + ybase);
-    hin = hvalid;
-    const unsigned long long bad = edge & out;
-#pragma unroll
-    for (int i = 0; i < HL; ++i) {
-      const bool ok = ((hvalid >> i) & 1u) && !((bad >> (4 * i)) & 0xfull);
-      hreg[i] = ld16(xg + (size_t)(origin + (ok ? rel_h[i] : 0)) * a.C * sizeof(T) + xbase);
-      if (!ok) hin &= ~(1u << i);
-    }
-  };
-  auto swz = [](int row) { return (row >> 1) & 3; };
-  auto chunk_off_of = [&](int row, int ch) {
-    if (!BF) return ch * 16;
-    return (((ch >> 1) ^ swz(row)) << 5) | ((ch & 1) << 4);
-  };
-  auto chunk_off = [&](int row) { return chunk_off_of(row, chunk); };
-  auto store_lds = [&](int buf) {
-    char* yb = smem + buf * BUF;
-    char* hb = yb + YBUF;
-    float r_scale[EPC], r_shift[EPC];
-    if (xform) {
-#pragma unroll
-      for (int e = 0; e < EPC; ++e) { r_scale[e] = s_aff[seg_ld * 128 + chunk * EPC + e]; r_shift[e] = s_aff[seg_ld * 128 + 64 + chunk * EPC + e]; }
-    }
-#pragma unroll
-    for (int i = 0; i < YL; ++i) {
-      const int p = prowy + YROWS * i;
-      st16(yb + (chunky / CPR) * YH + p * RB + chunk_off_of(p, chunky % CPR), yreg[i]);
-    }
-#pragma unroll
-    for (int i = 0; i < HL; ++i) {
-      const int hp = prow + HROWS * i;
-      if (hp >= HP) continue;
-      const int hni = hp / (HH * HWD), hrem = hp - hni * (HH * HWD);
-      const int hpl = (hni * HH + hrem / HWD) * PITCH + hrem % HWD;
-      u32x4_t v = hreg[i];
-      if (!((hin >> i) & 1u)) {
-        v = u32x4_t{0u, 0u, 0u, 0u};
-      } else if (xform) {
-        float f[EPC];
-        Elem<T>::unpack(v, f);
-#pragma unroll
-        for (int e = 0; e < EPC; ++e) {
-          float q = fmaf(f[e], r_scale[e], r_shift[e]);
-          f[e] = a.in_relu ? fmaxf(q, 0.f) : q;
-        }
-        v = Elem<T>::pack(f);
-      }
-      st16(hb + hpl * RB + chunk_off(hpl), v);
-    }
-  };
-
-  f32x4_t acc[9][4];
-#pragma unroll
-  for (int t = 0; t < 9; ++t)
-#pragma unroll
-    for (int c = 0; c < 4; ++c) acc[t][c] = f32x4_t{0.f, 0.f, 0.f, 0.f};
-
-  auto hpix = [&](int p) {
-    if (TW == 16) return (p >> 4) * PITCH + (p & 15);
-    return (p >> 6) * (HH * PITCH) + ((p >> 3) & 7) * PITCH + (p & 7);
-  };
-
-  load_regs(t_begin);
-  __syncthreads();
-  store_lds(0);
-  __syncthreads();
-  int buf = 0;
-  for (int tile = t_begin; tile < t_end; ++tile) {
-    const bool more = tile + 1 < t_end;
-    if (more) load_regs(tile + 1);
-    const char* yb = smem + buf * BUF;
-    const char* hb = yb + YBUF;
-    if constexpr (BF) {
-      const int pl = 16 * (g >> 1) + 4 * (g & 1) + (li >> 2);
-      constexpr int HI = (TW == 16 ? 8 : PITCH) * RB;
-      int Aoff[4], Boff[3];
-#pragma unroll
-      for (int t4 = 0; t4 < 4; ++t4) Aoff[t4] = pl * RB + ((t4 ^ swz(pl)) << 5) + (li & 3) * 8;
-#pragma unroll
-      for (int sx = 0; sx < 3; ++sx) {
-        const int hp = hpix(pl) + sx;
-        Boff[sx] = hp * RB + ((wave ^ swz(hp)) << 5) + (li & 3) * 8;
-      }
-      bf16x8_t bfr[2];
-      auto bfrag_of = [&](int q, int t) {
-        const int qoff = (hpix(q * 32) + (t / 3) * PITCH) * RB;
-        return tr_pair(hb + Boff[t % 3] + qoff, hb + Boff[t % 3] + qoff + HI);
-      };
-      auto qstep = [&](const int q, const int par) {
-        bf16x8_t af[4];
-#pragma unroll
-        for (int t4 = 0; t4 < 4; ++t4) {
-          const char* pa = yb + kh * YH + q * 32 * RB + Aoff[t4];
-          af[t4] = tr_pair(pa, pa + 8 * RB);
-        }
-#pragma unroll
-        for (int t = 0; t < 9; ++t) {
-          bfr[(t + 1 + par) & 1] = t < 8 ? bfrag_of(q, t + 1) : bfrag_of(q < 3 ? q + 1 : 3, 0);
-          __builtin_amdgcn_sched_barrier(0);
-#pragma unroll
-          for (int t4 = 0; t4 < 4; ++t4)
-            acc[t][t4] = __builtin_amdgcn_mfma_f32_16x16x32_bf16(af[t4], bfr[(t + par) & 1], acc[t][t4], 0, 0, 0);
-          __builtin_amdgcn_sched_barrier(0);
-        }
-      };
-      bfr[0] = bfrag_of(0, 0);
-#pragma unroll 1
-      for (int q2 = 0; q2 < 2; ++q2) {
-        qstep(2 * q2, 0);
-        qstep(2 * q2 + 1, 1);
-      }
-    } else {
-#pragma unroll 2
-      for (int q = 0; q < 32; ++q) {
-        const int p = 4 * q + g;
-        float av[4];
-#pragma unroll
-        for (int t4 = 0; t4 < 4; ++t4) av[t4] = *reinterpret_cast<const float*>(yb + p * RB + (16 * t4 + li) * 4);
-        const int hp0 = hpix(p);
-#pragma unroll
-        for (int t = 0; t < 9; ++t) {
-          const int toff = (t / 3) * PITCH + (t % 3);
-          const float bv = *reinterpret_cast<const float*>(hb + (hp0 + toff) * RB + (16 * wave + li) * 4);
-#pragma unroll
-          for (int t4 = 0; t4 < 4; ++t4) acc[t][t4] = __builtin_amdgcn_mfma_f32_16x16x4f32(av[t4], bv, acc[t][t4], 0, 0, 0);
-        }
-      }
-    }
-    if (NBUF == 1) {
-      __syncthreads();
-      if (more) store_lds(0);
-    } else if (more) {
-      store_lds(buf ^ 1);
-    }
-    __syncthreads();
-    if (NBUF == 2) buf ^= 1;
-  }
-
-  if (partials) {
-    const size_t wg = ((size_t)bz * gy + by) * gx + bx;
-    f32x4_t* sp = partials + wg * 36 * NT + tid;
-#pragma unroll
-    for (int t = 0; t < 9; ++t)
-#pragma unroll
-      for (int t4 = 0; t4 < 4; ++t4) sp[(size_t)(t * 4 + t4) * NT] = acc[t][t4];
-    return;
-  }
-#pragma unroll
-  for (int t = 0; t < 9; ++t)
-#pragma unroll
-    for (int t4 = 0; t4 < 4; ++t4)
-#pragma unroll
-      for (int j = 0; j < 4; ++j) {
-        const int k = k0 + 64 * kh + 16 * t4 + 4 * g + j;
-        a.dw[((size_t)k * 9 + t) * a.C + c0 + 16 * wave + li] += acc[t][t4][j];
-      }
+  constexpr bool BN = false;
+  constexpr int nt_store = 0;
+  const BnBwdArgs b{};
+#include "wgrad_halo_body.hpp"
+}
+template <typename T, int TW>
+__global__ __launch_bounds__(256, 2) void wgrad3x3_halo_bn_kernel(const WgradArgs a, const BnBwdArgs b, int tiles_per_split, int ntiles,
+                                                                  f32x4_t* partials, int nt_store) {
+  constexpr bool BN = true;
+  constexpr int KH = 1;
+#include "wgrad_halo_body.hpp"
 }
 
 __global__ __launch_bounds__(1024) void wgrad_fold_kernel(const f32x4_t* __restrict__ partials, float* dw, int C, int gx, int gy, int splits,
@@ -371,6 +136,33 @@
   }
   return tw == 16 ? f(WgradHaloInst<float, 16, 1>{}) : f(WgradHaloInst<float, 8, 1>{});
 }
+
+bool wgrad_halo_bn_ok(int dtype, const WgradArgs& a, const BnBwdArgs& b) {
+  if (dtype != DT_BF16 || wgrad_halo_tw(a) != 16 || a.K != 64 || a.C != 64 || a.seg_images > 0) return false;
+  if (b.pool_dy || b.nseg > 1 || b.relu_from_x || b.C != a.K || b.pixels != (size_t)a.N * a.H * a.W) return false;
+  if (b.pixels * 64 * sizeof(bf16_t) >= ((size_t)1 << 32)) return false;
+  if (!b.g_in_reduce && (b.yact || b.yact_bits)) return false;
+  const void* g = b.g_in_reduce ? b.gout : b.dy;
+  return g && b.x && b.dx && b.sums && b.mean && b.invstd && b.scale && a.x && a.dw && !(b.count <= 0.0);
+}
+struct WgradHaloBnInst { static std::string spell() { return kname("wgrad3x3_halo_bn_kernel", ktype<bf16_t>(), 16); } };
+const char* wgrad_halo_bn_name() { return InstName{}(WgradHaloBnInst{}); }
+hipError_t launch_wgrad_halo_bn(const WgradArgs& a, const BnBwdArgs& b0, hipStream_t st) {
+  if (!wgrad_halo_bn_ok(DT_BF16, a, b0)) return hipErrorInvalidValue;
+  static const int nt = [] { const char* e = getenv("SSLCR_WGRAD_BN_NT"); return (e && atoi(e) != 0) ? 1 : 0; }();
+  BnBwdArgs b = b0;
+  if (b.g_in_reduce) { b.dy = b.gout; b.gout = nullptr; b.g_in_reduce = 0; }
+  int tps, ntiles;
+  const int splits = wh_splits(a, 16, 1, &tps, &ntiles);
+  const size_t slab_bytes = splits > 1 ? (size_t)splits * 36 * 256 * sizeof(f32x4_t) : 0;
+  return with_slabs(st, slab_bytes,
+    [&](f32x4_t* slabs) {
+      const size_t lds = (size_t)(128 + 10 * 24) * 64 * sizeof(bf16_t) + 512 + 768;
+      return launch_lds<wgrad3x3_halo_bn_kernel<bf16_t, 16>>(dim3(splits), dim3(256), lds, 96 * 1024, st, a, b, tps, ntiles, slabs, nt);
+    },
+    [&](f32x4_t* slabs) { return launch_wgrad_fold(slabs, a.dw, a.C, 1, 1, splits, 9, 1, st); });
+}
+
 hipError_t launch_wgrad_halo(int dtype, const WgradArgs& a, const WgradPlan& p, hipStream_t st) {
   return wh_pick(dtype, p.tw, p.KH, [&](auto inst) { return launch_wh(inst, a, p.route == WgradRoute::HALO_DMA, st); });
 }
diff --git a/ssl_cr_histo_amd/csrc/wgrad_halo_body.hpp b/ssl_cr_histo_amd/csrc/wgrad_halo_body.hpp
--- /dev/null
+++ b/ssl_cr_histo_amd/csrc/wgrad_halo_body.hpp
@@ -0,0 +1,327 @@
+  constexpr int EPC = Elem<T>::EPC;
+  constexpr bool BF = Elem<T>::DT == DT_BF16;
+  constexpr int RB = 64 * sizeof(T);
+  constexpr int CPR = RB / 16;
+  constexpr int TH = 8;
+  constexpr int NI = 128 / (TH * TW);
+  constexpr int HH = TH + 2, HWD = TW + 2;
+  constexpr int HP = NI * HH * HWD;
+  constexpr int NT = 256 * KH;
+  constexpr int YL = 128 * CPR / 256;
+  constexpr int HL = (HP * CPR + NT - 1) / NT;
+  constexpr int YROWS = 256 / CPR, HROWS = NT / CPR;
+  constexpr int PITCH = BF ? (TW == 16 ? 24 : 16) : HWD;
+  constexpr int YH = 128 * RB;
+  constexpr int YBUF = KH * YH, HBUF = NI * HH * PITCH * RB;
+  constexpr int BUF = YBUF + HBUF;
+  constexpr int NBUF = KH;
+  extern __shared__ __attribute__((aligned(16))) char smem[];
+
+  const int tid = threadIdx.x, lane = tid & 63;
+  const int wave = (tid >> 6) & 3, kh = tid >> 8;
+  const int li = lane & 15, g = lane >> 4;
+  const int gx = a.K / (64 * KH), gy = a.C / 64, GT = gx * gy, splits = (int)gridDim.x / GT;
+  const OuterInner oi = xcd_outer_inner(blockIdx.x, splits, GT, false);
+  const int bz = oi.outer, bt = oi.inner;
+  const int by = bt / gx, bx = bt - by * gx;
+  const int k0 = bx * (64 * KH), c0 = by * 64;
+  const int chunk = tid % CPR, prow = tid / CPR;
+  const int chunky = tid % (CPR * KH), prowy = tid / (CPR * KH);
+  const bool xform = a.in_scale != nullptr;
+  float* s_aff = reinterpret_cast<float*>(smem + NBUF * BUF);
+  const int nseg = a.seg_images > 0 ? a.N / a.seg_images : 1;
+  for (int i = tid; i < nseg * 64; i += NT) {
+    const int sg = i >> 6, ch = i & 63;
+    s_aff[sg * 128 + ch] = xform ? a.in_scale[(size_t)sg * a.seg_stride + c0 + ch] : 1.f;
+    s_aff[sg * 128 + 64 + ch] = xform ? a.in_shift[(size_t)sg * a.seg_stride + c0 + ch] : 0.f;
+  }
+  float* s_bn = s_aff + 128;
+  if constexpr (BN) {
+    if (tid < 64) {
+      const int c = tid;
+      const float invM = (float)(1.0 / b.count);
+      const float is = b.invstd[c], sc = b.scale[c];
+      const float m0 = (float)b.sums[c] * invM, m1 = (float)b.sums[64 + c] * invM;
+      const float cB = -sc * is * is * m1;
+      s_bn[c] = sc;
+      s_bn[64 + c] = cB;
+      s_bn[128 + c] = -sc * m0 - cB * b.mean[c];
+      if (blockIdx.x == 0 && b.dgamma && b.dbeta) {
+        b.dgamma[c] += (float)(b.sums[64 + c] * (double)b.invstd[c] * (double)b.pg_scale);
+        b.dbeta[c] += (float)(b.sums[c] * (double)b.pg_scale);
+      }
+    }
+  }
+  const int tiles_w = a.W / TW, tiles_h = a.H / TH;
+  const int t_begin = bz * tiles_per_split;
+  int t_end = t_begin + tiles_per_split;
+  if (t_end > ntiles) t_end = ntiles;
+  if (t_begin >= t_end) {
+    if (partials) {
+      const size_t wg = ((size_t)bz * gy + by) * gx + bx;
+      for (int e = 0; e < 36; ++e) partials[(wg * 36 + e) * NT + tid] = f32x4_t{0.f, 0.f, 0.f, 0.f};
+    }
+    return;
+  }
+  const char* xg = reinterpret_cast<const char*>(a.x);
+  const char* dyg = reinterpret_cast<const char*>(BN ? b.dy : a.dy);
+  const char* rawg = BN ? reinterpret_cast<const char*>(b.x) : nullptr;
+  char* drawg = BN ? reinterpret_cast<char*>(b.dx) : nullptr;
+
+  int rel_y[YL], rel_h[HL];
+  static_assert(HL <= 16, "edge mask holds 16 halo entries");
+  unsigned long long edge = 0;
+  unsigned hvalid = 0;
+#pragma unroll
+  for (int i = 0; i < YL; ++i) {
+    const int p = prowy + YROWS * i;
+    const int ni = p / (TH * TW), rem = p - ni * (TH * TW);
+    const int ph = rem / TW, pw = rem - ph * TW;
+    rel_y[i] = (ni * a.H + ph) * a.W + pw;
+  }
+#pragma unroll
+  for (int i = 0; i < HL; ++i) {
+    const int hp = prow + HROWS * i;
+    rel_h[i] = 0;
+    if (hp < HP) {
+      const int ni = hp / (HH * HWD), rem = hp - ni * (HH * HWD);
+      const int hr = rem / HWD, hc = rem - hr * HWD;
+      rel_h[i] = (ni * a.H + hr - 1) * a.W + hc - 1;
+      hvalid |= 1u << i;
+      edge |= (unsigned long long)((hr == 0) | ((hr == HH - 1) << 1) | ((hc == 0) << 2) | ((hc == HWD - 1) << 3)) << (4 * i);
+    }
+  }
+  const size_t ybase = ((size_t)k0 + chunky * EPC) * sizeof(T), xbase = ((size_t)c0 + chunk * EPC) * sizeof(T);
+
+  u32x4_t yreg[YL], hreg[HL];
+  unsigned hin = 0;
+  int seg_ld = 0;
+  int org_ld = 0, org_nxt = 0;
+  auto yoff = [&](int i) { return (unsigned)(rel_y[i] * 64 + chunky * EPC) * (unsigned)sizeof(T); };
+  auto load_half = [&](int half) {
+#pragma unroll
+    for (int j = 0; j < 2; ++j) {
+      const unsigned off = (unsigned)org_ld * (unsigned)(64 * sizeof(T)) + yoff(2 * half + j);
+      yreg[j] = ld16(dyg + off);
+      yreg[2 + j] = ld16(rawg + off);
+    }
+  };
+  auto load_regs = [&](int tile) {
+    int t = tile;
+    const int tw_i = t % tiles_w; t /= tiles_w;
+    const int th_i = t % tiles_h;
+    const int n0 = (t / tiles_h) * NI;
+    const int h0 = th_i * TH, w0 = tw_i * TW;
+    seg_ld = a.seg_images > 0 ? n0 / a.seg_images : 0;
+    const int origin = (n0 * a.H + h0) * a.W + w0;
+    const unsigned long long out =
+        (unsigned long long)((h0 == 0) | ((h0 + TH >= a.H) << 1) | ((w0 == 0) << 2) | ((w0 + TW >= a.W) << 3)) * 0x1111111111111111ull;
+    if constexpr (BN) {
+      org_nxt = origin;
+    } else {
+#pragma unroll
+      for (int i = 0; i < YL; ++i)
+        yreg[i] = ld16(dyg + (size_t)(origin + rel_y[i]) * a.K * sizeof(T) + ybase);
+    }
+    hin = hvalid;
+    const unsigned long long bad = edge & out;
+#pragma unroll
+    for (int i = 0; i < HL; ++i) {
+      const bool ok = ((hvalid >> i) & 1u) && !((bad >> (4 * i)) & 0xfull);
+      if constexpr (BN) hreg[i] = ld16(xg + ((unsigned)(origin + (ok ? rel_h[i] : 0)) * (unsigned)(64 * sizeof(T)) + (unsigned)xbase));
+      else hreg[i] = ld16(xg + (size_t)(origin + (ok ? rel_h[i] : 0)) * a.C * sizeof(T) + xbase);
+      if (!ok) hin &= ~(1u << i);
+    }
+  };
+  auto swz = [](int row) { return (row >> 1) & 3; };
+  auto chunk_off_of = [&](int row, int ch) {
+    if (!BF) return ch * 16;
+    return (((ch >> 1) ^ swz(row)) << 5) | ((ch & 1) << 4);
+  };
+  auto chunk_off = [&](int row) { return chunk_off_of(row, chunk); };
+  auto stage_half = [&](int half) {
+    if constexpr (BN) {
+#pragma unroll
+      for (int q = 0; q < 2; ++q) {
+        const f32x4_t cA = *reinterpret_cast<const f32x4_t*>(s_bn + chunky * EPC + 4 * q);
+        const f32x4_t cB = *reinterpret_cast<const f32x4_t*>(s_bn + 64 + chunky * EPC + 4 * q);
+        const f32x4_t cC = *reinterpret_cast<const f32x4_t*>(s_bn + 128 + chunky * EPC + 4 * q);
+#pragma unroll
+        for (int j = 0; j < 2; ++j)
+#pragma unroll
+          for (int w = 0; w < 2; ++w) {
+            const uint32_t gw = yreg[j][2 * q + w], xw = yreg[2 + j][2 * q + w];
+            const float d0 = fmaf(cA[2 * w], bf_lo(gw), fmaf(cB[2 * w], bf_lo(xw), cC[2 * w]));
+            const float d1 = fmaf(cA[2 * w + 1], bf_hi(gw), fmaf(cB[2 * w + 1], bf_hi(xw), cC[2 * w + 1]));
+            yreg[j][2 * q + w] = PackH<T>::pair(d0, d1);
+          }
+        __builtin_amdgcn_sched_barrier(0);
+      }
+#pragma unroll
+      for (int j = 0; j < 2; ++j) {
+        const int p = prowy + YROWS * (2 * half + j);
+        st16(smem + p * RB + chunk_off_of(p, chunky), yreg[j]);
+        char* dst = drawg + ((unsigned)org_ld * (unsigned)(64 * sizeof(T)) + yoff(2 * half + j));
+        if (nt_store) st16_nt(dst, yreg[j]);
+        else st16(dst, yreg[j]);
+      }
+    }
+  };
+  auto store_lds = [&](int buf) {
+    char* yb = smem + buf * BUF;
+    char* hb = yb + YBUF;
+    float r_scale[EPC], r_shift[EPC];
+    auto read_aff = [&] {
+#pragma unroll
+      for (int e = 0; e < EPC; ++e) { r_scale[e] = s_aff[seg_ld * 128 + chunk * EPC + e]; r_shift[e] = s_aff[seg_ld * 128 + 64 + chunk * EPC + e]; }
+    };
+    if constexpr (!BN) {
+      if (xform) read_aff();
+    }
+    if constexpr (BN) {
+      stage_half(0);
+      load_half(1);
+      if (xform) read_aff();
+    } else {
+#pragma unroll
+      for (int i = 0; i < YL; ++i) {
+        const int p = prowy + YROWS * i;
+        st16(yb + (chunky / CPR) * YH + p * RB + chunk_off_of(p, chunky % CPR), yreg[i]);
+      }
+    }
+#pragma unroll
+    for (int i = 0; i < HL; ++i) {
+      const int hp = prow + HROWS * i;
+      if (hp >= HP) continue;
+      const int hni = hp / (HH * HWD), hrem = hp - hni * (HH * HWD);
+      const int hpl = (hni * HH + hrem / HWD) * PITCH + hrem % HWD;
+      u32x4_t v = hreg[i];
+      if (!((hin >> i) & 1u)) {
+        v = u32x4_t{0u, 0u, 0u, 0u};
+      } else if (xform) {
+        float f[EPC];
+        Elem<T>::unpack(v, f);
+#pragma unroll
+        for (int e = 0; e < EPC; ++e) {
+          float q = fmaf(f[e], r_scale[e], r_shift[e]);
+          f[e] = a.in_relu ? fmaxf(q, 0.f) : q;
+        }
+        v = Elem<T>::pack(f);
+      }
+      st16(hb + hpl * RB + chunk_off(hpl), v);
+    }
+  };
+
+  f32x4_t acc[9][4];
+#pragma unroll
+  for (int t = 0; t < 9; ++t)
+#pragma unroll
+    for (int c = 0; c < 4; ++c) acc[t][c] = f32x4_t{0.f, 0.f, 0.f, 0.f};
+
+  auto hpix = [&](int p) {
+    if (TW == 16) return (p >> 4) * PITCH + (p & 15);
+    return (p >> 6) * (HH * PITCH) + ((p >> 3) & 7) * PITCH + (p & 7);
+  };
+
+  load_regs(t_begin);
+  if constexpr (BN) { org_ld = org_nxt; load_half(0); }
+  __syncthreads();
+  store_lds(0);
+  __syncthreads();
+  int buf = 0;
+  for (int tile = t_begin; tile < t_end; ++tile) {
+    const bool more = tile + 1 < t_end;
+    if (more) load_regs(tile + 1);
+    const char* yb = smem + buf * BUF;
+    const char* hb = yb + YBUF;
+    if constexpr (BF) {
+      const int pl = 16 * (g >> 1) + 4 * (g & 1) + (li >> 2);
+      constexpr int HI = (TW == 16 ? 8 : PITCH) * RB;
+      int Aoff[4], Boff[3];
+#pragma unroll
+      for (int t4 = 0; t4 < 4; ++t4) Aoff[t4] = pl * RB + ((t4 ^ swz(pl)) << 5) + (li & 3) * 8;
+#pragma unroll
+      for (int sx = 0; sx < 3; ++sx) {
+        const int hp = hpix(pl) + sx;
+        Boff[sx] = hp * RB + ((wave ^ swz(hp)) << 5) + (li & 3) * 8;
+      }
+      bf16x8_t bfr[2];
+      auto bfrag_of = [&](int q, int t) {
+        const int qoff = (hpix(q * 32) + (t / 3) * PITCH) * RB;
+        return tr_pair(hb + Boff[t % 3] + qoff, hb + Boff[t % 3] + qoff + HI);
+      };
+      auto qstep = [&](const int q, const int par) {
+        bf16x8_t af[4];
+#pragma unroll
+        for (int t4 = 0; t4 < 4; ++t4) {
+          const char* pa = yb + kh * YH + q * 32 * RB + Aoff[t4];
+          af[t4] = tr_pair(pa, pa + 8 * RB);
+        }
+#pragma unroll
+        for (int t = 0; t < 9; ++t) {
+          bfr[(t + 1 + par) & 1] = t < 8 ? bfrag_of(q, t + 1) : bfrag_of(q < 3 ? q + 1 : 3, 0);
+          __builtin_amdgcn_sched_barrier(0);
+#pragma unroll
+          for (int t4 = 0; t4 < 4; ++t4)
+            acc[t][t4] = __builtin_amdgcn_mfma_f32_16x16x32_bf16(af[t4], bfr[(t + par) & 1], acc[t][t4], 0, 0, 0);
+          __builtin_amdgcn_sched_barrier(0);
+        }
+      };
+      bfr[0] = bfrag_of(0, 0);
+#pragma unroll 1
+      for (int q2 = 0; q2 < 2; ++q2) {
+        if constexpr (BN) {
+          if (q2 == 1) {
+            stage_half(1);
+            if (more) { org_ld = org_nxt; load_half(0); }
+            __syncthreads();
+          }
+        }
+        qstep(2 * q2, 0);
+        qstep(2 * q2 + 1, 1);
+      }
+    } else {
+#pragma unroll 2
+      for (int q = 0; q < 32; ++q) {
+        const int p = 4 * q + g;
+        float av[4];
+#pragma unroll
+        for (int t4 = 0; t4 < 4; ++t4) av[t4] = *reinterpret_cast<const float*>(yb + p * RB + (16 * t4 + li) * 4);
+        const int hp0 = hpix(p);
+#pragma unroll
+        for (int t = 0; t < 9; ++t) {
+          const int toff = (t / 3) * PITCH + (t % 3);
+          const float bv = *reinterpret_cast<const float*>(hb + (hp0 + toff) * RB + (16 * wave + li) * 4);
+#pragma unroll
+          for (int t4 = 0; t4 < 4; ++t4) acc[t][t4] = __builtin_amdgcn_mfma_f32_16x16x4f32(av[t4], bv, acc[t][t4], 0, 0, 0);
+        }
+      }
+    }
+    if (NBUF == 1) {
+      __syncthreads();
+      if (more) store_lds(0);
+    } else if (more) {
+      store_lds(buf ^ 1);
+    }
+    __syncthreads();
+    if (NBUF == 2) buf ^= 1;
+  }
+
+  if (partials) {
+    const size_t wg = ((size_t)bz * gy + by) * gx + bx;
+    f32x4_t* sp = partials + wg * 36 * NT + tid;
+#pragma unroll
+    for (int t = 0; t < 9; ++t)
+#pragma unroll
+      for (int t4 = 0; t4 < 4; ++t4) sp[(size_t)(t * 4 + t4) * NT] = acc[t][t4];
+    return;
+  }
+#pragma unroll
+  for (int t = 0; t < 9; ++t)
+#pragma unroll
+    for (int t4 = 0; t4 < 4; ++t4)
+#pragma unroll
+      for (int j = 0; j < 4; ++j) {
+        const int k = k0 + 64 * kh + 16 * t4 + 4 * g + j;
+        a.dw[((size_t)k * 9 + t) * a.C + c0 + 16 * wave + li] += acc[t][t4][j];
+      }
```

Measured after the change: 70220, median of 6. Within noise of the previous version (+0.9%).
